# weleen/AGRL.pytorch

Hardware: AMD Instinct MI355X
Metric: frames/sec (fwd+GCN+distmat), MARS seq_len=8 (higher is better)
Workload: dtype fp16; 1 GPU; MARS seq_len=8 bs=32/GPU fp16 fwd+distmat (BASELINE configs[1]): 256x128 frames, VMGN ResNet50x2-branch + 2 graph layers, cosine distmat vs resident 12180 x 4096 gallery; global_batch=32, seq_len=8, gallery_rows_per_gpu=12180, parallelism=dp1, hip_graph=False, ranks=1, devices_visible=1, library=libagrl_hip.so, clip_batches_rotated=3, clip_bytes_rotated=301989888

## Files before the change

### agrl.pytorch_amd/csrc/bottleneck_block.hip

```cpp
#include "igemm_dev.h"

namespace {

struct BlockParams {
    const void* z;
    const void* w2;
    const float* b2;
    const void* w3;
    const float* b3;
    const void* res;
    const void* xs;
    const void* ws;
    const float* bs;
    void* out;
    const void* w1n;
    const float* b1n;
    void* zn;
    int F, H, W;
};

template <bool CAT, int CN>
__global__ __launch_bounds__(512) void bottleneck_block_kernel(const BlockParams p, int ntiles) {
    static_assert(CN == 64 || (CN == 128 && !CAT), "next conv1: 64 channels, or 128 with the identity shortcut");
    constexpr int NW = 8, PW = 10, PPIX = 100, PPIECES = 13, PATCH_BYTES = PPIECES * 1024, PJ = 2;
    constexpr int W_TAP = 64 * 128, W2_BYTES = 9 * W_TAP;
    constexpr int Y_BYTES = 64 * 128;
    constexpr int X_BYTES = CAT ? 64 * 128 : 0;
    constexpr int R_BYTES = 64 * 512;
    constexpr int NST = CN == 64 ? 5 : 6;
    constexpr int NA2 = CN / 64;
    __shared__ __attribute__((aligned(16))) unsigned char smem[W2_BYTES + 2 * PATCH_BYTES + Y_BYTES + X_BYTES + R_BYTES + 1024];
    unsigned char* s_w2 = smem;
    unsigned char* s_p = s_w2 + W2_BYTES;
    unsigned char* s_y = s_p + 2 * PATCH_BYTES;
    unsigned char* s_x = s_y + Y_BYTES;
    unsigned char* s_r = s_x + X_BYTES;
    unsigned char* s_dummy = s_r + R_BYTES;

    const int tid = threadIdx.x, lane = tid & 63;
    const int wave = __builtin_amdgcn_readfirstlane(tid >> 6);
    const int frow = lane & 15, fchunk = lane >> 4;
    const int lrow = lane >> 3, lchk = lane & 7;
    const int G = gridDim.x;
    const int tw = p.W >> 3, th = p.H >> 3;
    const unsigned char* zsrc = reinterpret_cast<const unsigned char*>(&g_zero16);
    const unsigned char* zg = reinterpret_cast<const unsigned char*>(p.z);
    const unsigned char* resg = reinterpret_cast<const unsigned char*>(p.res);
    const unsigned char* xsg = reinterpret_cast<const unsigned char*>(p.xs);

    {
        const int row = wave * 8 + lrow;
#pragma unroll
        for (int t = 0; t < 9; ++t)
            dma16(reinterpret_cast<const unsigned char*>(p.w2) + ((size_t)row * 576 + t * 64) * 2 + ((lchk ^ ((row >> 1) & 7)) << 4),
                  s_w2 + t * W_TAP + wave * 8 * 128);
    }
    const int wm2 = wave & 1, wn4 = wave >> 1;
    uint4 w3f[4][2], wsf[CAT ? 4 : 1][2], w1f[NA2][8];
#pragma unroll
    for (int a = 0; a < 4; ++a)
#pragma unroll
        for (int kk = 0; kk < 2; ++kk) {
            const size_t o = ((size_t)(wn4 * 64 + a * 16 + frow) * 64 + kk * 32 + fchunk * 8) * 2;
            w3f[a][kk] = *reinterpret_cast<const uint4*>(reinterpret_cast<const unsigned char*>(p.w3) + o);
            if constexpr (CAT) wsf[a][kk] = *reinterpret_cast<const uint4*>(reinterpret_cast<const unsigned char*>(p.ws) + o);
        }
#pragma unroll
    for (int a = 0; a < NA2; ++a)
#pragma unroll
        for (int ks = 0; ks < 8; ++ks)
            w1f[a][ks] = *reinterpret_cast<const uint4*>(reinterpret_cast<const unsigned char*>(p.w1n) +
                                                         ((size_t)(wn4 * (CN / 4) + a * 16 + frow) * 256 + ks * 32 + fchunk * 8) * 2);
    const int wm = wave & 3, wn = wave >> 2;
    float4 b2v[2], b3v[4], b1v[NA2];
#pragma unroll
    for (int a = 0; a < 2; ++a) b2v[a] = *reinterpret_cast<const float4*>(p.b2 + wn * 32 + a * 16 + fchunk * 4);
#pragma unroll
    for (int a = 0; a < 4; ++a) {
        b3v[a] = *reinterpret_cast<const float4*>(p.b3 + wn4 * 64 + a * 16 + fchunk * 4);
        if constexpr (CAT) {
            const float4 t = *reinterpret_cast<const float4*>(p.bs + wn4 * 64 + a * 16 + fchunk * 4);
            b3v[a].x += t.x; b3v[a].y += t.y; b3v[a].z += t.z; b3v[a].w += t.w;
        }
    }
#pragma unroll
    for (int a = 0; a < NA2; ++a) b1v[a] = *reinterpret_cast<const float4*>(p.b1n + wn4 * (CN / 4) + a * 16 + fchunk * 4);
#pragma unroll
    for (int a = 0; a < 4; ++a)
#pragma unroll
        for (int kk = 0; kk < 2; ++kk) {
            asm volatile("" : "+v"(w3f[a][kk].x), "+v"(w3f[a][kk].y), "+v"(w3f[a][kk].z), "+v"(w3f[a][kk].w));
            if constexpr (CAT) asm volatile("" : "+v"(wsf[a][kk].x), "+v"(wsf[a][kk].y), "+v"(wsf[a][kk].z), "+v"(wsf[a][kk].w));
        }
#pragma unroll
    for (int a = 0; a < NA2; ++a)
#pragma unroll
        for (int ks = 0; ks < 8; ++ks) asm volatile("" : "+v"(w1f[a][ks].x), "+v"(w1f[a][ks].y), "+v"(w1f[a][ks].z), "+v"(w1f[a][ks].w));
#pragma unroll
    for (int a = 0; a < 4; ++a) asm volatile("" : "+v"(b3v[a].x), "+v"(b3v[a].y), "+v"(b3v[a].z), "+v"(b3v[a].w));
#pragma unroll
    for (int a = 0; a < 2; ++a) asm volatile("" : "+v"(b2v[a].x), "+v"(b2v[a].y), "+v"(b2v[a].z), "+v"(b2v[a].w));
#pragma unroll
    for (int a = 0; a < NA2; ++a) asm volatile("" : "+v"(b1v[a].x), "+v"(b1v[a].y), "+v"(b1v[a].z), "+v"(b1v[a].w));

    unsigned res_lane[4], out_lane[CN == 64 ? 4 : 1];
#pragma unroll
    for (int j = 0; j < 4; ++j) {
        const int rrow = (wave * 4 + j) * 2 + (lane >> 5);
        res_lane[j] = (unsigned)(((rrow >> 3) * p.W + (rrow & 7)) * 512 + (((lane & 31) ^ (rrow & 31)) << 4));
        const int orow = (tid >> 5) + 16 * j;
        if constexpr (CN == 64) out_lane[j] = (unsigned)(((orow >> 3) * p.W + (orow & 7)) * 512 + (((tid & 31) ^ (orow & 31)) << 4));
    }

    auto tile_origin = [&](int T, int& img, int& oy0, int& ox0) {
        img = T / (tw * th);
        const int trem = T - img * (tw * th);
        oy0 = (trem / tw) << 3;
        ox0 = (trem % tw) << 3;
    };
    auto gpix = [&](int img, int oy0, int ox0, int q) { return ((size_t)img * p.H + oy0 + (q >> 3)) * p.W + ox0 + (q & 7); };

    auto stage_patch = [&](int T, int buf) {
        int img, oy0, ox0;
        tile_origin(T, img, oy0, ox0);
        int ln = lane;
        asm volatile("" : "+v"(ln));
#pragma unroll
        for (int i = 0; i < PJ; ++i) {
            const int piece = wave + NW * i;
            const int row = piece * 8 + (ln >> 3);
            const int py = row / PW, px = row - py * PW;
            const int iy = oy0 + py - 1, ix = ox0 + px - 1;
            const bool ok = piece < PPIECES && row < PPIX && (unsigned)iy < (unsigned)p.H && (unsigned)ix < (unsigned)p.W;
            dma16(ok ? zg + (((size_t)img * p.H + iy) * p.W + ix) * 128 + (((ln & 7) ^ patch_g(py, px)) << 4) : zsrc,
                  piece < PPIECES ? s_p + buf * PATCH_BYTES + piece * 1024 : s_dummy);
        }
    };
    auto stage_shortcut = [&](int T) {
        int img, oy0, ox0;
        tile_origin(T, img, oy0, ox0);
        int ln = lane;
        asm volatile("" : "+v"(ln));
        if constexpr (CAT) {
            const int row = wave * 8 + (ln >> 3);
            dma16(xsg + gpix(img, oy0, ox0, row) * 128 + (((ln & 7) ^ ((row >> 1) & 7)) << 4), s_x + wave * 1024);
        } else {
            const unsigned char* tbase = resg + gpix(img, oy0, ox0, 0) * 512;
#pragma unroll
            for (int j = 0; j < 4; ++j) dma16(tbase + res_lane[j], s_r + (wave * 4 + j) * 1024);
        }
    };

    int xoff[18], woff[2][2];
    {
        const int q = frag_px(frow);
        const int py0 = 2 * wm + (q >> 3), px0 = q & 7;
#pragma unroll
        for (int st = 0; st < 18; ++st) {
            const int t = st >> 1, kk = st & 1;
            xoff[st] = patch_off<PW>(py0 + t / 3, px0 + t % 3, kk * 4 + fchunk);
        }
#pragma unroll
        for (int kk = 0; kk < 2; ++kk)
#pragma unroll
            for (int a = 0; a < 2; ++a) woff[kk][a] = lds_off(wn * 32 + a * 16 + frow, kk * 4 + fchunk);
    }

    const int xcd = blockIdx.x & 7;
    const int xq = ntiles >> 3, xr = ntiles & 7;
    const int xbase = xcd < xr ? xcd * (xq + 1) : xr * (xq + 1) + (xcd - xr) * xq;
    const int tend = xbase + xq + (xcd < xr ? 1 : 0);
    const int tstep = (G >> 3) + (xcd < (G & 7) ? 1 : 0);
    int T = xbase + (int)(blockIdx.x >> 3);
    if (T < tend) stage_patch(T, 0);
    int buf = 0;
    bool first = true;
    for (; T < tend; T += tstep, buf ^= 1) {
        int img, oy0, ox0;
        tile_origin(T, img, oy0, ox0);
        const bool has_next = T + tstep < tend;
        if (first) wait_vmcnt<0>();
        else wait_vmcnt<NST>();
        first = false;
        wg_barrier();
        stage_shortcut(T);
        if (has_next) stage_patch(T + tstep, buf ^ 1);
        int fr = frow, fc = fchunk, td = tid;
        asm volatile("" : "+v"(fr), "+v"(fc), "+v"(td));

        {
            const unsigned char* sp = s_p + buf * PATCH_BYTES;
            const int q = frag_px(fr);
            f32x4_t acc0[2] = {f32x4_t{0.f, 0.f, 0.f, 0.f}, f32x4_t{0.f, 0.f, 0.f, 0.f}};
            uint4 xq[3], wq[3][2];
            auto ld0 = [&](int st, int slot) {
                const int t = st >> 1, kk = st & 1;
                xq[slot] = *reinterpret_cast<const uint4*>(sp + xoff[st]);
#pragma unroll
                for (int a = 0; a < 2; ++a) wq[slot][a] = *reinterpret_cast<const uint4*>(s_w2 + t * W_TAP + woff[kk][a]);
            };
            ld0(0, 0);
            ld0(1, 1);
#pragma unroll
            for (int st = 0; st < 18; ++st) {
                if (st + 2 < 18) ld0(st + 2, (st + 2) % 3);
#pragma unroll
                for (int a = 0; a < 2; ++a) acc0[a] = Frag<lp16_t>::mma(wq[st % 3][a], xq[st % 3], acc0[a]);
                __builtin_amdgcn_sched_barrier(0);
            }
            const int prow = wm * 16 + q;
#pragma unroll
            for (int a = 0; a < 2; ++a) {
                const int c = wn * 32 + a * 16 + fc * 4;
                float v[4] = {relu_nan(acc0[a][0] + b2v[a].x), relu_nan(acc0[a][1] + b2v[a].y),
                              relu_nan(acc0[a][2] + b2v[a].z), relu_nan(acc0[a][3] + b2v[a].w)};
                store4<lp16_t>(reinterpret_cast<lp16_t*>(s_y + prow * 128 + (((c >> 3) ^ ((prow >> 1) & 7)) << 4) + ((c & 4) << 1)), v);
            }
        }
        if constexpr (CAT) {
            if (has_next) wait_vmcnt<PJ>();
            else wait_vmcnt<0>();
        }
        wg_barrier();

        f32x4_t acc[4][2];
#pragma unroll
        for (int a = 0; a < 4; ++a)
#pragma unroll
            for (int b = 0; b < 2; ++b) acc[a][b] = f32x4_t{0.f, 0.f, 0.f, 0.f};
#pragma unroll
        for (int kk = 0; kk < 2; ++kk) {
            uint4 xf[2];
#pragma unroll
            for (int b = 0; b < 2; ++b) xf[b] = *reinterpret_cast<const uint4*>(s_y + lds_off(wm2 * 32 + b * 16 + fr, kk * 4 + fc));
#pragma unroll
            for (int a = 0; a < 4; ++a)
#pragma unroll
                for (int b = 0; b < 2; ++b) acc[a][b] = Frag<lp16_t>::mma(w3f[a][kk], xf[b], acc[a][b]);
        }
        if constexpr (CAT) {
#pragma unroll
            for (int kk = 0; kk < 2; ++kk) {
                uint4 xf[2];
#pragma unroll
                for (int b = 0; b < 2; ++b) xf[b] = *reinterpret_cast<const uint4*>(s_x + lds_off(wm2 * 32 + b * 16 + fr, kk * 4 + fc));
#pragma unroll
                for (int a = 0; a < 4; ++a)
#pragma unroll
                    for (int b = 0; b < 2; ++b) acc[a][b] = Frag<lp16_t>::mma(wsf[a][kk], xf[b], acc[a][b]);
            }
        } else {
            if (has_next) wait_vmcnt<PJ>();
            else wait_vmcnt<0>();
            wg_barrier();
        }
        uint2 rcell[2][4];
        if constexpr (!CAT) {
#pragma unroll
            for (int b = 0; b < 2; ++b) {
                const int px = wm2 * 32 + b * 16 + fr;
#pragma unroll
                for (int a = 0; a < 4; ++a) {
                    const int c = wn4 * 64 + a * 16 + fc * 4;
                    rcell[b][a] = *reinterpret_cast<const uint2*>(s_r + px * 512 + (((c >> 3) ^ (px & 31)) << 4) + ((c & 4) << 1));
                }
            }
        }
#pragma unroll
        for (int b = 0; b < 2; ++b) {
            const int px = wm2 * 32 + b * 16 + fr;
#pragma unroll
            for (int a = 0; a < 4; ++a) {
                const int c = wn4 * 64 + a * 16 + fc * 4;
                unsigned char* cell = s_r + px * 512 + (((c >> 3) ^ (px & 31)) << 4) + ((c & 4) << 1);
                float rr[4] = {0.f, 0.f, 0.f, 0.f};
                if constexpr (!CAT) {
                    unpack_lp16x2(rcell[b][a].x, rr[0], rr[1]);
                    unpack_lp16x2(rcell[b][a].y, rr[2], rr[3]);
                }
                float v[4];
                v[0] = relu_nan(acc[a][b][0] + b3v[a].x + rr[0]);
                v[1] = relu_nan(acc[a][b][1] + b3v[a].y + rr[1]);
                v[2] = relu_nan(acc[a][b][2] + b3v[a].z + rr[2]);
                v[3] = relu_nan(acc[a][b][3] + b3v[a].w + rr[3]);
                store4<lp16_t>(reinterpret_cast<lp16_t*>(cell), v);
            }
        }
        wg_barrier();
        {
            unsigned char* obase = reinterpret_cast<unsigned char*>(p.out) + gpix(img, oy0, ox0, 0) * 512;
#pragma unroll
            for (int i = 0; i < 4; ++i) {
                const int row = (td >> 5) + 16 * i;
                const int pch = td & 31;
                const uint4 v = *reinterpret_cast<const uint4*>(s_r + row * 512 + (pch << 4));
                if constexpr (CN == 64) *reinterpret_cast<uint4*>(obase + out_lane[i]) = v;
                else *reinterpret_cast<uint4*>(reinterpret_cast<unsigned char*>(p.out) + (gpix(img, oy0, ox0, row) * 256 + (pch ^ (row & 31)) * 8) * 2) = v;
            }
        }
        f32x4_t acc2[NA2][2];
#pragma unroll
        for (int a = 0; a < NA2; ++a)
#pragma unroll
            for (int b = 0; b < 2; ++b) acc2[a][b] = f32x4_t{0.f, 0.f, 0.f, 0.f};
        {
            uint4 x2[3][2];
            auto ld2 = [&](int ks, int slot) {
#pragma unroll
                for (int b = 0; b < 2; ++b) {
                    const int px = wm2 * 32 + b * 16 + fr;
                    x2[slot][b] = *reinterpret_cast<const uint4*>(s_r + px * 512 + (((ks * 4 + fc) ^ (px & 31)) << 4));
                }
            };
            ld2(0, 0);
            ld2(1, 1);
#pragma unroll
            for (int ks = 0; ks < 8; ++ks) {
                if (ks + 2 < 8) ld2(ks + 2, (ks + 2) % 3);
#pragma unroll
                for (int a = 0; a < NA2; ++a)
#pragma unroll
                    for (int b = 0; b < 2; ++b) acc2[a][b] = Frag<lp16_t>::mma(w1f[a][ks], x2[ks % 3][b], acc2[a][b]);
                __builtin_amdgcn_sched_barrier(0);
            }
        }
        unsigned char* sz = CN == 64 ? s_y : s_r;
        if constexpr (CN == 128) wg_barrier();
#pragma unroll
        for (int b = 0; b < 2; ++b) {
            const int px = wm2 * 32 + b * 16 + fr;
#pragma unroll
            for (int a = 0; a < NA2; ++a) {
                const int c = wn4 * (CN / 4) + a * 16 + fc * 4;
                float v[4];
                v[0] = relu_nan(acc2[a][b][0] + b1v[a].x);
                v[1] = relu_nan(acc2[a][b][1] + b1v[a].y);
                v[2] = relu_nan(acc2[a][b][2] + b1v[a].z);
                v[3] = relu_nan(acc2[a][b][3] + b1v[a].w);
                store4<lp16_t>(reinterpret_cast<lp16_t*>(sz + px * (CN * 2) + (((c >> 3) ^ (px & (CN / 8 - 1))) << 4) + ((c & 4) << 1)), v);
            }
        }
        wg_barrier();
#pragma unroll
        for (int i = 0; i < CN / 64; ++i) {
            const int row = td >> 3, pch = (td & 7) * (CN / 64) + i;
            const uint4 v = *reinterpret_cast<const uint4*>(sz + row * (CN * 2) + (pch << 4));
            *reinterpret_cast<uint4*>(reinterpret_cast<unsigned char*>(p.zn) + (gpix(img, oy0, ox0, row) * CN + (pch ^ (row & (CN / 8 - 1))) * 8) * 2) = v;
        }
    }
}

}

extern "C" int agrl_bottleneck_block(const void* z, const void* w2, const float* b2, const void* w3, const float* b3,
                                     const void* residual, const void* x_short, const void* w_short, const float* b_short,
                                     void* out, const void* w1_next, const float* b1_next, void* z_next, int F, int H, int W,
                                     int Cmid, int Cout, int Cnext, agrl_stream_t stream) {
    AGRL_CHECK_ARG(z && w2 && b2 && w3 && b3 && out && w1_next && b1_next && z_next, "agrl_bottleneck_block: null pointer");
    AGRL_CHECK_ARG((residual != nullptr) != (x_short != nullptr),
                   "agrl_bottleneck_block: pass either the residual map or the downsample conv's input, not both");
    AGRL_CHECK_ARG(!x_short || (w_short && b_short), "agrl_bottleneck_block: the downsample form needs its weights and bias");
    AGRL_CHECK_ARG(F > 0 && H > 0 && W > 0 && (H % 8) == 0 && (W % 8) == 0, "agrl_bottleneck_block: maps must be multiples of 8 x 8 (got %d x %d)", H, W);
    AGRL_CHECK_ARG(Cmid == 64 && Cout == 256 && (Cnext == 64 || (Cnext == 128 && !x_short)),
                   "agrl_bottleneck_block: built for Cmid=64, Cout=256, Cnext=64 (128 without downsample), got %d/%d/%d", Cmid, Cout, Cnext);
    AGRL_CHECK_ARG((size_t)F * H * W * 256 * 2 < (1ull << 40), "agrl_bottleneck_block: problem too large");
    const uintptr_t al = (uintptr_t)z | (uintptr_t)w2 | (uintptr_t)b2 | (uintptr_t)w3 | (uintptr_t)b3 | (uintptr_t)residual |
                         (uintptr_t)x_short | (uintptr_t)w_short | (uintptr_t)b_short | (uintptr_t)out | (uintptr_t)w1_next |
                         (uintptr_t)b1_next | (uintptr_t)z_next;
    AGRL_CHECK_ARG((al & 15) == 0, "agrl_bottleneck_block: pointers must be 16-byte aligned");
    BlockParams p;
    p.z = z; p.w2 = w2; p.b2 = b2; p.w3 = w3; p.b3 = b3; p.res = residual; p.xs = x_short; p.ws = w_short; p.bs = b_short;
    p.out = out; p.w1n = w1_next; p.b1n = b1_next; p.zn = z_next; p.F = F; p.H = H; p.W = W;
    const int ntiles = F * (H / 8) * (W / 8);
    const int grid = ntiles < 256 ? ntiles : 256;
    if (x_short) hipLaunchKernelGGL((bottleneck_block_kernel<true, 64>), dim3(grid), dim3(512), 0, (hipStream_t)stream, p, ntiles);
    else if (Cnext == 128) hipLaunchKernelGGL((bottleneck_block_kernel<false, 128>), dim3(grid), dim3(512), 0, (hipStream_t)stream, p, ntiles);
    else hipLaunchKernelGGL((bottleneck_block_kernel<false, 64>), dim3(grid), dim3(512), 0, (hipStream_t)stream, p, ntiles);
    AGRL_CHECK_LAUNCH("agrl_bottleneck_block");
    return 0;
}
```

### agrl.pytorch_amd/csrc/bottleneck_tail.hip

```cpp
#include "igemm_dev.h"

namespace {

struct TailParams {
    const void* y2;
    const void* w3;
    const float* b3;
    const void* res;
    void* out;
    const void* w1n;
    const float* b1n;
    void* z;
    const void* xs;
    const void* ws;
    const float* bs;
    int M;
};

constexpr int TBM = 64, TK1 = 64, TN1 = 256, TK2 = 256, TN2 = 64;

template <bool CAT>
__global__ __launch_bounds__(512) void bottleneck_tail_kernel(const TailParams p, int ntiles) {
    constexpr int NKT1 = CAT ? 2 : 1;
    constexpr int W3_BYTES = NKT1 * TN1 * 128;
// ... 207 lines not shown
            const int gch = (lane & 31) ^ (row & 31);
            dma16(gm < p.M ? resg + ((size_t)gm * TN1 + gch * 8) * 2 : zsrc, sr + piece * 1024);
        }
    };
    float4 b3v[4], b1v[2];
#pragma unroll
    for (int a = 0; a < 4; ++a) b3v[a] = *reinterpret_cast<const float4*>(p.b3 + wn4 * 64 + a * 16 + fchunk * 4);
#pragma unroll
    for (int a = 0; a < 2; ++a) b1v[a] = *reinterpret_cast<const float4*>(p.b1n + wn4 * 32 + a * 16 + fchunk * 4);

    int T = blockIdx.x;
    if (T < ntiles) stage_y2(T, 0);
    wait_vmcnt<0>();
    wg_barrier();
    int slot = 0;
    for (; T < ntiles; T += G, slot ^= 1) {
        const int m0 = T * TBM;
        const bool has_next = T + G < ntiles;
        stage_res(T);
        if (has_next) stage_y2(T + G, slot ^ 1);
        const unsigned char* sa = s_a + slot * A_BYTES;
        f32x4_t acc[4][2];
#pragma unroll
        for (int a = 0; a < 4; ++a)
#pragma unroll
            for (int b = 0; b < 2; ++b) acc[a][b] = f32x4_t{0.f, 0.f, 0.f, 0.f};
#pragma unroll
        for (int kk = 0; kk < 2; ++kk) {
            uint4 xf[2], wf[4];
#pragma unroll
            for (int b = 0; b < 2; ++b) xf[b] = *reinterpret_cast<const uint4*>(sa + lds_off(wm2 * 32 + b * 16 + frow, kk * 4 + fchunk));
#pragma unroll
            for (int a = 0; a < 4; ++a) wf[a] = *reinterpret_cast<const uint4*>(s_w3 + lds_off(wn4 * 64 + a * 16 + frow, kk * 4 + fchunk));
#pragma unroll
            for (int a = 0; a < 4; ++a)
#pragma unroll
                for (int b = 0; b < 2; ++b) acc[a][b] = Frag<lp16_t>::mma(wf[a], xf[b], acc[a][b]);
        }
        if (has_next) wait_vmcnt<1>();
        else wait_vmcnt<0>();
        wg_barrier();
#pragma unroll
        for (int b = 0; b < 2; ++b) {
            const int px = wm2 * 32 + b * 16 + frow;
#pragma unroll
            for (int a = 0; a < 4; ++a) {
                const int c = wn4 * 64 + a * 16 + fchunk * 4;
                unsigned char* cell = sr + px * 512 + (((c >> 3) ^ (px & 31)) << 4) + ((c & 4) << 1);
                float rr[4];
                load4<lp16_t>(reinterpret_cast<const lp16_t*>(cell), rr);
                float v[4];
                v[0] = relu_nan(acc[a][b][0] + b3v[a].x + rr[0]);
                v[1] = relu_nan(acc[a][b][1] + b3v[a].y + rr[1]);
                v[2] = relu_nan(acc[a][b][2] + b3v[a].z + rr[2]);
                v[3] = relu_nan(acc[a][b][3] + b3v[a].w + rr[3]);
                store4<lp16_t>(reinterpret_cast<lp16_t*>(cell), v);
            }
        }
        wg_barrier();
#pragma unroll
        for (int i = 0; i < 4; ++i) {
            const int row = (tid >> 5) + 16 * i;
            const int pch = tid & 31;
            const int gm = m0 + row;
            if (gm < p.M) {
                const uint4 v = *reinterpret_cast<const uint4*>(sr + row * 512 + (pch << 4));
                *reinterpret_cast<uint4*>(reinterpret_cast<unsigned char*>(p.out) + ((size_t)gm * TN1 + (pch ^ (row & 31)) * 8) * 2) = v;
            }
        }
        f32x4_t acc2[2][2];
#pragma unroll
        for (int a = 0; a < 2; ++a)
#pragma unroll
            for (int b = 0; b < 2; ++b) acc2[a][b] = f32x4_t{0.f, 0.f, 0.f, 0.f};
#pragma unroll
        for (int ks = 0; ks < TK2 / 32; ++ks) {
            uint4 wf[2], xf[2];
#pragma unroll
            for (int a = 0; a < 2; ++a)
                wf[a] = *reinterpret_cast<const uint4*>(s_w1 + (ks >> 1) * W1_KT + lds_off(wn4 * 32 + a * 16 + frow, (ks & 1) * 4 + fchunk));
#pragma unroll
            for (int b = 0; b < 2; ++b) {
                const int px = wm2 * 32 + b * 16 + frow;
                xf[b] = *reinterpret_cast<const uint4*>(sr + px * 512 + (((ks * 4 + fchunk) ^ (px & 31)) << 4));
            }
#pragma unroll
            for (int a = 0; a < 2; ++a)
#pragma unroll
                for (int b = 0; b < 2; ++b) acc2[a][b] = Frag<lp16_t>::mma(wf[a], xf[b], acc2[a][b]);
        }
        wg_barrier();
#pragma unroll
        for (int b = 0; b < 2; ++b) {
            const int px = wm2 * 32 + b * 16 + frow;
#pragma unroll
            for (int a = 0; a < 2; ++a) {
                const int c = wn4 * 32 + a * 16 + fchunk * 4;
                float v[4];
                v[0] = relu_nan(acc2[a][b][0] + b1v[a].x);
                v[1] = relu_nan(acc2[a][b][1] + b1v[a].y);
                v[2] = relu_nan(acc2[a][b][2] + b1v[a].z);
                v[3] = relu_nan(acc2[a][b][3] + b1v[a].w);
                store4<lp16_t>(reinterpret_cast<lp16_t*>(sr + px * 256 + (((c >> 3) ^ (px & 15)) << 4) + ((c & 4) << 1)), v);
            }
        }
        wg_barrier();
#pragma unroll
        for (int i = 0; i < 2; ++i) {
            const int row = tid >> 3, pch = (tid & 7) * 2 + i;
            const int gm = m0 + row;
            if (gm < p.M) {
                const uint4 v = *reinterpret_cast<const uint4*>(sr + row * 256 + (pch << 4));
                *reinterpret_cast<uint4*>(reinterpret_cast<unsigned char*>(p.z) + ((size_t)gm * CN + (pch ^ (row & 15)) * 8) * 2) = v;
            }
        }
        wait_vmcnt<6>();
        wg_barrier();
    }
}


constexpr int L2K1 = 128, L2N1 = 512, L2K2 = 512, L2N2 = 128;

__global__ __launch_bounds__(512) void bottleneck_tail_l2_kernel(const TailParams p, int ntiles) {
    constexpr int A_BYTES = 2 * TBM * 128;
    constexpr int R_BYTES = TBM * L2N1 * 2;
    __shared__ __attribute__((aligned(16))) unsigned char smem[2 * A_BYTES + 2 * R_BYTES];
    unsigned char* s_a = smem;
    unsigned char* s_r = smem + 2 * A_BYTES;

    const int tid = threadIdx.x, lane = tid & 63;
    const int wave = __builtin_amdgcn_readfirstlane(tid >> 6);
    const int frow = lane & 15, fchunk = lane >> 4;
    const int G = gridDim.x;
    const unsigned char* zsrc = reinterpret_cast<const unsigned char*>(&g_zero16);
    const unsigned char* y2g = reinterpret_cast<const unsigned char*>(p.y2);
    const unsigned char* resg = reinterpret_cast<const unsigned char*>(p.res);

    uint4 w3f[4][4], w1f[16];
#pragma unroll
    for (int a = 0; a < 4; ++a)
#pragma unroll
        for (int kk = 0; kk < 4; ++kk)
            w3f[a][kk] = *reinterpret_cast<const uint4*>(reinterpret_cast<const unsigned char*>(p.w3) +
                                                         ((size_t)(wave * 64 + a * 16 + frow) * L2K1 + kk * 32 + fchunk * 8) * 2);
#pragma unroll
    for (int ks = 0; ks < 16; ++ks)
        w1f[ks] = *reinterpret_cast<const uint4*>(reinterpret_cast<const unsigned char*>(p.w1n) +
                                                  ((size_t)(wave * 16 + frow) * L2K2 + ks * 32 + fchunk * 8) * 2);
    float b3l = p.b3[wave * 64 + lane];
    float b1l = p.b1n[wave * 16 + (lane & 15)];
    asm volatile("" : "+v"(b3l), "+v"(b1l));
    auto lane_bias = [&](float held, int src_lane) {
        return __int_as_float(__builtin_amdgcn_ds_bpermute(src_lane << 2, __float_as_int(held)));
    };
#pragma unroll
    for (int a = 0; a < 4; ++a)
#pragma unroll
        for (int kk = 0; kk < 4; ++kk)
            asm volatile("" : "+v"(w3f[a][kk].x), "+v"(w3f[a][kk].y), "+v"(w3f[a][kk].z), "+v"(w3f[a][kk].w));
#pragma unroll
    for (int ks = 0; ks < 16; ++ks) asm volatile("" : "+v"(w1f[ks].x), "+v"(w1f[ks].y), "+v"(w1f[ks].z), "+v"(w1f[ks].w));

    auto stage_tile = [&](int T, int slot) {
        const int m0 = T * TBM;
        int ln = lane;
        asm volatile("" : "+v"(ln));
        {
            const int row = wave * 8 + (ln >> 3);
            const int gm = m0 + row;
#pragma unroll
            for (int kt = 0; kt < 2; ++kt)
                dma16(gm < p.M ? y2g + (size_t)gm * (L2K1 * 2) + kt * 128 + (((ln & 7) ^ ((row >> 1) & 7)) << 4) : zsrc,
                      s_a + slot * A_BYTES + kt * (TBM * 128) + wave * 1024);
        }
#pragma unroll
        for (int j = 0; j < 8; ++j) {
            const int row = wave * 8 + j;
            const int gm = m0 + row;
            dma16(gm < p.M ? resg + (size_t)gm * (L2N1 * 2) + ((ln ^ (row & 31)) << 4) : zsrc, s_r + slot * R_BYTES + row * 1024);
        }
    };

    int T = blockIdx.x;
    if (T < ntiles) stage_tile(T, 0);
    wait_vmcnt<0>();
    wg_barrier();
    int slot = 0;
    for (; T < ntiles; T += G, slot ^= 1) {
        const int m0 = T * TBM;
        if (T + G < ntiles) stage_tile(T + G, slot ^ 1);
        const unsigned char* sa = s_a + slot * A_BYTES;
        unsigned char* sr = s_r + slot * R_BYTES;
#pragma unroll
        for (int ah = 0; ah < 2; ++ah) {
            f32x4_t acc[2][4];
#pragma unroll
            for (int a = 0; a < 2; ++a)
#pragma unroll
                for (int b = 0; b < 4; ++b) acc[a][b] = f32x4_t{0.f, 0.f, 0.f, 0.f};
            uint4 xp[2][4];
            auto ld1 = [&](int kk, int b) {
                return *reinterpret_cast<const uint4*>(sa + (kk >> 1) * (TBM * 128) + lds_off(b * 16 + frow, (kk & 1) * 4 + fchunk));
            };
#pragma unroll
            for (int b = 0; b < 4; ++b) xp[0][b] = ld1(0, b);
#pragma unroll
            for (int kk = 0; kk < 4; ++kk) {
                if (kk + 1 < 4) {
#pragma unroll
                    for (int b = 0; b < 4; ++b) xp[(kk + 1) & 1][b] = ld1(kk + 1, b);
                }
#pragma unroll
                for (int a = 0; a < 2; ++a)
#pragma unroll
                    for (int b = 0; b < 4; ++b) acc[a][b] = Frag<lp16_t>::mma(w3f[2 * ah + a][kk], xp[kk & 1][b], acc[a][b]);
                __builtin_amdgcn_sched_barrier(0);
            }
            float bv[2][4];
#pragma unroll
            for (int a = 0; a < 2; ++a)
#pragma unroll
                for (int r = 0; r < 4; ++r) bv[a][r] = lane_bias(b3l, (2 * ah + a) * 16 + fchunk * 4 + r);
            uint2 rcell[4][2];
#pragma unroll
            for (int b = 0; b < 4; ++b) {
                const int px = b * 16 + frow;
#pragma unroll
                for (int a = 0; a < 2; ++a) {
                    const int c = wave * 64 + (2 * ah + a) * 16 + fchunk * 4;
                    rcell[b][a] = *reinterpret_cast<const uint2*>(sr + px * 1024 + (((c >> 3) ^ (px & 31)) << 4) + ((c & 4) << 1));
                }
            }
#pragma unroll
            for (int b = 0; b < 4; ++b) {
                const int px = b * 16 + frow;
#pragma unroll
                for (int a = 0; a < 2; ++a) {
                    const int c = wave * 64 + (2 * ah + a) * 16 + fchunk * 4;
                    unsigned char* cell = sr + px * 1024 + (((c >> 3) ^ (px & 31)) << 4) + ((c & 4) << 1);
                    float rr[4];
                    unpack_lp16x2(rcell[b][a].x, rr[0], rr[1]);
                    unpack_lp16x2(rcell[b][a].y, rr[2], rr[3]);
                    float v[4];
#pragma unroll
                    for (int r = 0; r < 4; ++r) v[r] = relu_nan(acc[a][b][r] + bv[a][r] + rr[r]);
                    store4<lp16_t>(reinterpret_cast<lp16_t*>(cell), v);
                }
            }
        }
        wg_barrier();
        int ld = lane, td = tid;
        asm volatile("" : "+v"(ld), "+v"(td));
#pragma unroll
        for (int i = 0; i < 8; ++i) {
            const int row = wave + 8 * i;
            const int gm = m0 + row;
            if (gm < p.M) {
                const uint4 v = *reinterpret_cast<const uint4*>(sr + row * 1024 + (ld << 4));
                *reinterpret_cast<uint4*>(reinterpret_cast<unsigned char*>(p.out) + ((size_t)gm * L2N1 + (ld ^ (row & 31)) * 8) * 2) = v;
            }
        }
        f32x4_t acc2[4];
#pragma unroll
        for (int b = 0; b < 4; ++b) acc2[b] = f32x4_t{0.f, 0.f, 0.f, 0.f};
        uint4 xq[2][4];
        auto ld2 = [&](int ks, int b) {
            const int px = b * 16 + frow;
            return *reinterpret_cast<const uint4*>(sr + px * 1024 + (((ks * 4 + fchunk) ^ (px & 31)) << 4));
        };
#pragma unroll
        for (int b = 0; b < 4; ++b) xq[0][b] = ld2(0, b);
#pragma unroll
        for (int ks = 0; ks < 16; ++ks) {
            if (ks + 1 < 16) {
#pragma unroll
                for (int b = 0; b < 4; ++b) xq[(ks + 1) & 1][b] = ld2(ks + 1, b);
            }
#pragma unroll
            for (int b = 0; b < 4; ++b) acc2[b] = Frag<lp16_t>::mma(w1f[ks], xq[ks & 1][b], acc2[b]);
            __builtin_amdgcn_sched_barrier(0);
        }
        unsigned char* sz = s_a + slot * A_BYTES;
#pragma unroll
        for (int b = 0; b < 4; ++b) {
            const int px = b * 16 + frow;
            const int c = wave * 16 + fchunk * 4;
            float v[4];
#pragma unroll
            for (int r = 0; r < 4; ++r) v[r] = relu_nan(acc2[b][r] + lane_bias(b1l, fchunk * 4 + r));
            store4<lp16_t>(reinterpret_cast<lp16_t*>(sz + px * 256 + (((c >> 3) ^ (px & 15)) << 4) + ((c & 4) << 1)), v);
        }
        wg_barrier();
#pragma unroll
        for (int i = 0; i < 2; ++i) {
            const int row = (td >> 4) + 32 * i, pch = td & 15;
            const int gm = m0 + row;
            if (gm < p.M) {
                const uint4 v = *reinterpret_cast<const uint4*>(sz + row * 256 + (pch << 4));
                *reinterpret_cast<uint4*>(reinterpret_cast<unsigned char*>(p.z) + ((size_t)gm * L2N2 + (pch ^ (row & 15)) * 8) * 2) = v;
            }
        }
        wait_vmcnt<10>();
        wg_barrier();
    }
}

}

extern "C" int agrl_bottleneck_tail(const void* y2, const void* w3, const float* b3, const void* residual,
                                    const void* x_short, const void* w_short, const float* b_short, void* out,
                                    const void* w1_next, const float* b1_next, void* z, int M, int Cmid, int Cout,
                                    int Cnext, int Cshort, agrl_stream_t stream) {
    AGRL_CHECK_ARG(y2 && w3 && b3 && out && w1_next && b1_next && z, "agrl_bottleneck_tail: null pointer");
    AGRL_CHECK_ARG((residual != nullptr) != (x_short != nullptr),
                   "agrl_bottleneck_tail: pass either the residual map or the downsample conv's input, not both");
    AGRL_CHECK_ARG(!x_short || (w_short && b_short), "agrl_bottleneck_tail: the downsample form needs its weights and bias");
    AGRL_CHECK_ARG(M > 0, "agrl_bottleneck_tail: empty problem");
    const bool layer2 = Cmid == L2K1 && Cout == L2N1 && Cnext == L2N2 && !x_short;
    AGRL_CHECK_ARG(layer2 || (Cmid == TK1 && Cout == TN1 && (Cnext == TN2 || (Cnext == 128 && !x_short)) && (!x_short || Cshort == TK1)),
                   "agrl_bottleneck_tail: built for Cmid=64, Cout=256, Cnext=64 (128 without downsample), Cshort=64 "
                   "(layer 1) and Cmid=128, Cout=512, Cnext=128 without downsample (layer 2), got %d/%d/%d/%d", Cmid, Cout, Cnext, Cshort);
    const uintptr_t al = (uintptr_t)y2 | (uintptr_t)w3 | (uintptr_t)b3 | (uintptr_t)residual | (uintptr_t)out |
                         (uintptr_t)w1_next | (uintptr_t)b1_next | (uintptr_t)z | (uintptr_t)x_short | (uintptr_t)w_short |
                         (uintptr_t)b_short;
    AGRL_CHECK_ARG((al & 15) == 0, "agrl_bottleneck_tail: pointers must be 16-byte aligned");
    TailParams p;
    p.y2 = y2; p.w3 = w3; p.b3 = b3; p.res = residual; p.out = out; p.w1n = w1_next; p.b1n = b1_next; p.z = z; p.M = M;
    p.xs = x_short; p.ws = w_short; p.bs = b_short;
    const int ntiles = cdiv(M, TBM);
    const int grid = ntiles < 256 ? ntiles : 256;
    if (layer2) hipLaunchKernelGGL(bottleneck_tail_l2_kernel, dim3(grid), dim3(512), 0, (hipStream_t)stream, p, ntiles);
    else if (Cnext == 128) hipLaunchKernelGGL(bottleneck_tail128_kernel, dim3(grid), dim3(512), 0, (hipStream_t)stream, p, ntiles);
    else if (x_short) hipLaunchKernelGGL(bottleneck_tail_kernel<true>, dim3(grid), dim3(512), 0, (hipStream_t)stream, p, ntiles);
    else hipLaunchKernelGGL(bottleneck_tail_kernel<false>, dim3(grid), dim3(512), 0, (hipStream_t)stream, p, ntiles);
    AGRL_CHECK_LAUNCH("agrl_bottleneck_tail");
    return 0;
}
```

### agrl.pytorch_amd/torchreid/_hip.py

```python
from __future__ import annotations

import ctypes as C
import os
import threading

import torch

F32 = 0
LP16 = 1
F32X3 = 2
F32H3P = 4
F32H3 = 3
FRAMES_NCHW = 0
FRAMES_NHWC = 1
METRIC_EUCLIDEAN = 0
METRIC_COSINE = 1

LP_NAME = os.environ.get("AGRL_HIP_LP16")
if LP_NAME is None:
    LP_NAME = os.environ.get("AGRL_HIP_PRECISION") if os.environ.get("AGRL_HIP_PRECISION") in ("fp16", "bf16") else "fp16"
if LP_NAME not in ("fp16", "bf16"):
    raise ValueError("AGRL_HIP_LP16 must be fp16 or bf16, not %r" % LP_NAME)
LP_DTYPE = torch.float16 if LP_NAME == "fp16" else torch.bfloat16

_HERE = os.path.dirname(os.path.abspath(__file__))
LIB_PATH = os.environ.get(
    "AGRL_HIP_LIB", os.path.normpath(os.path.join(_HERE, "..", "lib", "libagrl_hip.so" if LP_NAME == "fp16" else "libagrl_hip_bf16.so"))
)


class HipLibraryError(RuntimeError):
    """libagrl_hip.so is missing or incomplete."""


class HipKernelError(RuntimeError):
    """An entry point of libagrl_hip.so returned a non-zero status."""


_p = C.c_void_p
_i = C.c_int
_f = C.c_float

SIGNATURES = {
    "agrl_stem_conv_bn_relu_maxpool": [_p, _p, _p, _p, _i, _i, _i, _i, _p],
    "agrl_stem_conv_bn_relu_maxpool_lp16": [_p, _p, _p, _p, _i, _i, _i, _p],
    "agrl_conv2d_bn_act": [_p, _p, _p, _p, _p, _i, _i, _i, _i, _i, _i, _i, _i, _i, _i, _i, _p],
    "agrl_conv1x1_dual_split16": [_p, _p, _p, _p, _p] + [_i] * 8 + [_f, _i, _i, _p],
    "agrl_stem_split16": [_p, _p, _p, _p, _p, _i, _i, _i, _f, _p],
    "agrl_stem_conv_bn_relu_maxpool_u8": [_p, _p, _i, _p, _p, _p, _i, _i, _i, _i, _p],
    "agrl_stem_conv_bn_relu_maxpool_lp16_u8": [_p, _p, _i, _p, _p, _p, _i, _i, _i, _p],
    "agrl_stem_split16_u8": [_p, _p, _i, _p, _p, _p, _p, _i, _i, _i, _f, _p],
    "agrl_frames_normalize_u8": [_p, _p, _i, _p, _i, _i, _i, _p],
    "agrl_split16_planes": [_p, _p, C.c_longlong, _i, _i, _p],
    "agrl_split16_weight_planes": [_p, _p, C.c_longlong, _i, _f, _p],
    "agrl_split16_weights_inloop": [_p, _p, C.c_longlong, _i, _p],
    "agrl_conv1x1_split16": [_p, _p, _p, _p, _p, _i, _i, _i, _i, _f, _i, _p],
    "agrl_conv1x1_split16_dual": [_p, _p, _p, _p, _p, _i, _i, _i, _i, _i, _f, _i, _p],
    "agrl_conv1x1_split16_pool": [_p, _p, _p, _p, _p, _i, _i, _i, _i, _i, _i, C.POINTER(_i), _i, _i, _f, _i, _p],
    "agrl_conv3x3_packed_split16": [_p, _p, _p, _p, _i, _i, _i, _i, _i, _i, _f, _p],
    "agrl_conv2d_bn_act_split16": [_p, _p, _p, _p, _p] + [_i] * 10 + [_f, _i, _i, _p],
    "agrl_bottleneck_tail": [_p, _p, _p, _p, _p, _p, _p, _p, _p, _p, _p, _i, _i, _i, _i, _i, _p],
    "agrl_bottleneck_seam_packed_bytes": [_i, _i, _i],
    "agrl_bottleneck_seam_pack": [_p, _p, _p, _i, _i, _i, _p],
    "agrl_bottleneck_seam": [_p, _p, _p, _p, _p, _p, _p, _i, _i, _i, _i, _p],
    "agrl_conv3x3_packed_bytes": [_i, _i],
    "agrl_conv1x1_packed_bytes": [_i, _i],
    "agrl_conv1x1_pack": [_p, _p, _i, _i, _p],
    "agrl_conv1x1_packed_bn_act": [_p, _p, _p, _p, _p, _i, _i, _i, _i, _i, _p],
    "agrl_conv1x1_packed_res_bn_act": [_p, _p, _p, _p, _p, _i, _i, _i, _i, _p],
    "agrl_conv1x1_packed_res_pool": [_p, _p, _p, _p, _p, _p, _i, _i, _i, _i, _i, _i, C.POINTER(_i), _i, _i, _p],
    "agrl_conv1x1_packed_dual_duo": [_p, _p, _p, _p, _p, _i, _i, _i, _i, _i, _p],
    "agrl_conv1x1_packed_dual_strided": [_p, _p, _p, _p, _p, _i, _i, _i, _i, _i, _i, _i, _i, _p],
    "agrl_conv3x3_pack": [_p, _p, _i, _i, _p],
    "agrl_conv3x3_packed_bn_act": [_p, _p, _p, _p, _i, _i, _i, _i, _i, _i, _p],
    "agrl_bottleneck_block": [_p, _p, _p, _p, _p, _p, _p, _p, _p, _p, _p, _p, _p, _i, _i, _i, _i, _i, _i, _p],
    "agrl_conv1x1_dual_bn_act": [_p, _p, _p, _p, _p, _i, _i, _i, _i, _i, _p],
    "agrl_conv1x1_bn_act_pool": [_p, _p, _p, _p, _p, _p, _p, _i, _i, _i, _i, _i, _i, C.POINTER(_i), _i, _i, _p],
    "agrl_linear_nobias": [_p, _p, _p, _i, _i, _i, _i, _p],
    "agrl_part_pool": [_p, _p, _p, _p, _p, _i, _i, _i, _i, C.POINTER(_i), _i, _i, _p],
    "agrl_clip_pool": [_p, _p, _i, _i, _i, _i, _p],
    "agrl_graph_gram": [_p, _p, _i, _i, _i, _i, _p],
    "agrl_graph_pair_product": [_p, _p, _p, _p, _i, _i, _i, _p],
    "agrl_graph_finalize": [_p, _i, _p, _p, _i, _i, _i, _i, _i, _p],
    "agrl_graph_propagate": [_p, _p, _p, _p, _p, _f, _f, _f, _p, _p, _i, _i, _i, _p],
    "agrl_pam_pool": [_p, _p, _p, _p, _i, _i, _i, _i, _i, C.POINTER(_i), _i, _i, _p],
    "agrl_pam_combine": [_p, _p, _p, _f, _p, _p, _i, _i, _p],
    "agrl_graph_apply": [_p, _p, _p, _i, _i, _i, _i, _p],
    "agrl_graph_tracklet_operand": [_p, _p, _i, _p, _p, _i, _i, _i, _i, _i, _i, _i, _p],
    "agrl_graph_finalize_bits": [_p, _i, _p, _p, _i, _i, _i, _i, _i, _p],
    "agrl_pose_adjacency_bits": [_p, _p, _p, _i, _i, _i, _i, C.c_float, C.c_float, _p],
    "agrl_adjacency_pack": [_p, _p, _i, _i, _p],
    "agrl_graph_linear_mix": [_p, _p, _p, _p, _p, _f, _f, _f, _p, _i, _i, _i, _i, _p],
    "agrl_row_sqnorm": [_p, _p, _i, _i, _i, _p],
    "agrl_attn_pool_bnneck": [_p, _p, _p, _p, _p, _p, _p, _p, _p, _p, _i, _i, _i, _i, _i, _p],
    "agrl_attn_tail": [_p, _p, _p, _p, _p, _p, _p, _p, _p, _p, _p, _p, _p, _i, _i, _i, _i, _i, _p],
    "agrl_row_l2_normalize": [_p, _p, _i, _i, _i, _i, _i, _p],
    "agrl_distmat_split16": [_p, _p, _p, _p, _p, _i, _i, _i, _i, _i, _f, _p, C.c_size_t, _p],
    "agrl_distmat": [_p, _p, _p, _p, _p, _i, _i, _i, _i, _i, _i, _p, C.c_size_t, _p],
    "agrl_pose_adjacency": [_p, _p, _p, _i, _i, _i, _i, C.c_float, C.c_float, _p],
    "agrl_re_ranking_workspace": [_i, _i, _i],
    "agrl_re_ranking": [_p, _p, _p, _i, _i, _i, _i, C.c_double, _p, _i, _p, C.c_size_t, _p],
    "agrl_rank_topk": [_p, _i, _i, _i, _i, _i, _p, _p, _p],
    "agrl_distmat_topk_workspace": [_i, _i],
    "agrl_distmat_topk": [_p, _p, _p, _p, _i, _i, _i, _i, _i, _i, _i, _p, _p, _p, C.c_size_t, _p, C.c_size_t, _p],
    "agrl_rank_argsort": [_p, _i, _i, _i, _p, _p],
    "agrl_rank_mars": [_p, _p, _p, _p, _p, _i, _i, _i, _p, _p, _p],
    "agrl_rank_market1501": [_p, _i, _i, _i, _p, _p, _p, _p, _i, _p, _p, _p, _p],
    "agrl_triplet_hard_mine": [_p, _p, _i, _i, _p, _p, _p, _p, _p],
    "agrl_axpby": [_p, _p, _f, _f, _p, C.c_size_t, _p],
    "agrl_part_pool_backward": [_p, _p, _p, _p, _i, _i, _i, _i, _i, C.POINTER(_i), _i, _p],
    "agrl_attn_pool_backward": [_p, _p, _p, _i, _i, _i, _i, _p],
    "agrl_graph_matrix_backward": [_p, _i, _p, _p, _i, _i, _i, _i, _p],
    "agrl_xent_label_smooth": [_p, _p, _i, _i, _f, _p, _p, _p, _p],
    "agrl_triplet_loss": [_p, _p, _i, _i, _f, _i, _p, _p, _p, _p, _p, _p, _p, _p],
    "agrl_bn_workspace": [_i, _i],
    "agrl_bn_stats": [_p, _p, _p, _i, _i, _p, C.c_size_t, _p],
    "agrl_conv2d_stats": [_p, _p, _p, _p, C.c_size_t] + [_i] * 10 + [_p],
    "agrl_bn_stats_from_partials": [_p, _i, _i, _i, _p, _p, _p, C.c_size_t, _p],
    "agrl_bn_fold_train": [_p, _p, _p, _p, _f, _f, C.c_longlong, _p, _p, _p, _p, _p, _p, _i, _p],
    "agrl_bn_apply": [_p, _p, _p, _p, _p, _p, _i, _i, _i, _f, _p],
    "agrl_bn_backward": [_p, _p, _p, _p, _p, _p, _p, _i, _f, _p, _p, _p, _p, _i, _i, _p, C.c_size_t, _p],
    "agrl_im2col_t": [_p, _p, _i, _i, _i, _i, _i, _i, _i, _i, _i, _p],
    "agrl_gemm_nt_splitk": [_p, _p, _p, _i, _i, _i, _i, _p, C.c_size_t, _p],
    "agrl_im2col_rows": [_p, _p] + [_i] * 10 + [_p],
    "agrl_conv_wgrad_workspace": [_i] * 9,
    "agrl_conv_wgrad_plan": [_i] * 10 + [C.POINTER(_i)],
    "agrl_conv_wgrad": [_p, _p, _p] + [_i] * 10 + [_p, C.c_size_t, _p],
    "agrl_maxpool3x3s2": [_p, _p, _p, _i, _i, _i, _i, _p],
    "agrl_maxpool3x3s2_backward": [_p, _p, _p, _i, _i, _i, _i, _p],
    "agrl_diag_read_stream": [_p, C.c_size_t, _p, _i, _p],
    "agrl_optim_geometry": [C.POINTER(_i), C.POINTER(_i), C.POINTER(_i)],
    "agrl_adam_step": [_p, _i, _p, _i] + [_f] * 7 + [_i, _i, _p],
    "agrl_sgd_step": [_p, _i, _p, _i, _f, _f, _f, _i, _i, _i, _i, _p],
}

_lock = threading.Lock()
_lib = None


def lib():
    global _lib
    if _lib is not None:
        return _lib
    with _lock:
        if _lib is not None:
            return _lib
        if not os.path.exists(LIB_PATH):
            raise HipLibraryError(
                "libagrl_hip.so not found at %s -- build it with `python __graft_entry__.py` "
                "(or `make -C agrl.pytorch_amd/csrc`); the HIP path has no fallback" % LIB_PATH
            )
        try:
            h = C.CDLL(LIB_PATH)
        except OSError as e:
            raise HipLibraryError("cannot load %s: %s" % (LIB_PATH, e))
        for name, argtypes in SIGNATURES.items():
            try:
                fn = getattr(h, name)
            except AttributeError:
                raise HipLibraryError("%s does not export %s" % (LIB_PATH, name))
            fn.argtypes = argtypes
            fn.restype = _i
        h.agrl_re_ranking_workspace.restype = C.c_size_t
        h.agrl_bn_workspace.restype = C.c_size_t
        h.agrl_conv_wgrad_workspace.restype = C.c_size_t
        h.agrl_distmat_topk_workspace.restype = C.c_size_t
        h.agrl_bottleneck_seam_packed_bytes.restype = C.c_longlong
        h.agrl_conv3x3_packed_bytes.restype = C.c_longlong
        h.agrl_conv1x1_packed_bytes.restype = C.c_longlong
        for name in ("agrl_reload_options", "agrl_built_with_ablation", "agrl_lp16_is_f16"):
            getattr(h, name).argtypes = []
            getattr(h, name).restype = _i
        h.agrl_version.restype = _i
        h.agrl_last_error.restype = C.c_char_p
        if bool(h.agrl_lp16_is_f16()) != (LP_NAME == "fp16"):
            raise HipLibraryError("%s stores 16-bit data as %s but AGRL_HIP_LP16 asks for %s" % (
                LIB_PATH, "fp16" if h.agrl_lp16_is_f16() else "bf16", LP_NAME))
        _lib = h
    return _lib


RELOAD_HOOKS = []


def reload_options():
    lib().agrl_reload_options()
    for hook in RELOAD_HOOKS:
        hook()


def available() -> bool:
    try:
        lib()
        return True
    except HipLibraryError:
        return False


def _check(name, status):
    if status != 0:
        msg = lib().agrl_last_error()
        raise HipKernelError("%s failed (%d): %s" % (name, status, msg.decode() if msg else "?"))


def stream_ptr(device=None):
    return torch.cuda.current_stream(device).cuda_stream


def ptr(t):
    if t is None:
        return None
    assert t.is_cuda, "HIP entry points take device tensors"
    assert t.is_contiguous(), "HIP entry points take contiguous tensors"
    return t.data_ptr()


def dtype_code(dt):
    if dt == torch.float32:
        return F32
    if dt == LP_DTYPE:
        return LP16
    raise TypeError("unsupported dtype %s (float32 / %s only: the loaded library's 16-bit type is %s)" % (dt, LP_DTYPE, LP_NAME))


PROFILE = None
PROFILE_TAG = None


def call(name, *args):
    fn = getattr(lib(), name)
    if PROFILE is None:
        _check(name, fn(*args))
        return
    stream = torch.cuda.ExternalStream(args[-1]) if args[-1] else torch.cuda.current_stream()
    start, end = torch.cuda.Event(enable_timing=True), torch.cuda.Event(enable_timing=True)
    start.record(stream)
    _check(name, fn(*args))
    end.record(stream)
    global PROFILE_TAG
    PROFILE.append((name, start, end, PROFILE_TAG))
    PROFILE_TAG = None
```

### agrl.pytorch_amd/torchreid/hip_ops.py

```python
from __future__ import annotations

import ctypes as C
import os

import torch

from . import _hip
from ._hip import F32, LP16, LP_DTYPE, LP_NAME, METRIC_COSINE, METRIC_EUCLIDEAN, call, dtype_code, ptr


import contextlib
import threading
import weakref

_MODE = threading.local()


@contextlib.contextmanager
def f32_split(on=True):
    prev = getattr(_MODE, 'split', False)
    _MODE.split = bool(on)
    try:
        yield
    finally:
# ... 308 lines not shown
    Cc = x.shape[-1]
    out = torch.empty(tuple(x.shape[:-1]) + (nplanes * Cc,), dtype=torch.float16, device=x.device)
    with _dev(x):
        call("agrl_split16_planes", ptr(x), ptr(out), x.numel() // Cc, Cc, nplanes, _stream(x))
    return out


def to_split16_weight_planes(x, scale):
    assert x.dtype == torch.float32 and x.is_contiguous() and x.dim() == 2 and x.shape[1] % 4 == 0
    out = torch.empty((x.shape[0], 3 * x.shape[1]), dtype=torch.float16, device=x.device)
    with _dev(x):
        call("agrl_split16_weight_planes", ptr(x), ptr(out), x.shape[0], x.shape[1], float(scale), _stream(x))
    return out


def distmat_split16(q3, g3, metric, g_unscale, qn=None, gn=None, out=None):
    m, D3 = q3.shape
    n = g3.shape[0]
    assert g3.shape[1] == D3 and q3.dtype == torch.float16 and g3.dtype == torch.float16
    if out is None:
        out = torch.empty((m, n), dtype=torch.float32, device=q3.device)
    code = METRIC_EUCLIDEAN if metric == "euclidean" else METRIC_COSINE
    if _hip.PROFILE is not None:
        _hip.PROFILE_TAG = {"flops": 2.0 * m * n * D3 / 3, "mfma_flops": 2.0 * m * n * D3, "bytes": 2.0 * (m + n) * D3 + 4.0 * m * n}
    ws = None
    if (-(-m // 64)) * (-(-n // 128)) < 256:
        ws = torch.empty((8 * m * n,), dtype=torch.float32, device=q3.device)
    with _dev(q3):
        call("agrl_distmat_split16", ptr(q3), ptr(g3), ptr(qn), ptr(gn), out.data_ptr(), m, n, D3, out.stride(0), code, float(g_unscale),
             ptr(ws), 0 if ws is None else ws.numel() * 4, _stream(q3))
    return out


def from_split16_planes(x3, nplanes=3):
    Cc = x3.shape[-1] // nplanes
    return x3[..., :Cc].float() + x3[..., Cc:2 * Cc].float() * (2.0 ** -11)


def conv1x1_split16(x3, packed, unscale, bias, Cout, residual3=None, relu=True, x2=None, layout=0):
    N, H, W, Kx = x3.shape
    K3 = Kx // 2 * 3 if layout & 1 else Kx
    K23 = 0 if x2 is None else x2.shape[3]
    M = N * H * W
    no = 2 if layout & 2 else 3
    assert x3.dtype == torch.float16 and x3.is_contiguous() and packed.numel() == 2 * (K3 + K23) * Cout
    assert residual3 is None or (residual3.dtype == torch.float16 and residual3.is_contiguous() and tuple(residual3.shape) == (N, H, W, no * Cout))
    out = torch.empty((N, H, W, no * Cout), dtype=torch.float16, device=x3.device)
    if _hip.PROFILE is not None:
        _hip.PROFILE_TAG = {"flops": 2.0 * M * Cout * (K3 + K23) / 3, "mfma_flops": 2.0 * M * Cout * (K3 + K23),
                            "bytes": 2.0 * (x3.numel() + (0 if x2 is None else x2.numel()) + out.numel() + (0 if residual3 is None else residual3.numel() * 2 // no)) + packed.numel()}
    with _dev(x3):
        if x2 is None:
            call("agrl_conv1x1_split16", ptr(x3), ptr(packed), ptr(bias), ptr(residual3), ptr(out), M, K3, Cout, 1 if relu else 0,
                 float(unscale), int(layout), _stream(x3))
        else:
            assert residual3 is None and x2.dtype == torch.float16 and x2.is_contiguous() and tuple(x2.shape[:3]) == (N, H, W)
            call("agrl_conv1x1_split16_dual", ptr(x3), ptr(x2), ptr(packed), ptr(bias), ptr(out), M, K3, K23, Cout, 1 if relu else 0,
                 float(unscale), int(layout), _stream(x3))
    return out


def conv1x1_split16_pool(x3, packed, unscale, bias, Cout, residual3, splits, mean, relu=True, layout=0):
    N, H, W, K3 = x3.shape
    assert x3.dtype == torch.float16 and x3.is_contiguous() and (H, W) == (16, 8) and packed.numel() == 2 * K3 * Cout
    assert not (layout & 1), "the pooled conv's input is conv2's output: a triple"
    assert residual3 is None or (residual3.dtype == torch.float16 and residual3.is_contiguous()
                                 and tuple(residual3.shape) == (N, H, W, (2 if layout & 2 else 3) * Cout))
    P = int(sum(splits))
    pooled = torch.empty((N, P, Cout), dtype=torch.float32, device=x3.device)
    arr = (C.c_int * len(splits))(*[int(s_) for s_ in splits])
    if _hip.PROFILE is not None:
        _hip.PROFILE_TAG = {"flops": 2.0 * N * H * W * Cout * K3 / 3, "mfma_flops": 2.0 * N * H * W * Cout * K3,
                            "bytes": 2.0 * (x3.numel() + (residual3.numel() if residual3 is not None else 0)) + packed.numel() + 4.0 * pooled.numel()}
    with _dev(x3):
        call("agrl_conv1x1_split16_pool", ptr(x3), ptr(packed), ptr(bias), ptr(residual3), ptr(pooled), N, H, W, K3, Cout,
             1 if relu else 0, arr, len(splits), 1 if mean else 0, float(unscale), int(layout), _stream(x3))
    return pooled


def conv3x3_split16(x3, packed, unscale, bias, Cout, relu=True):
    N, H, W, Cin3 = x3.shape
    assert x3.dtype == torch.float16 and x3.is_contiguous() and packed.numel() == 2 * 9 * Cin3 * Cout
    out = torch.empty((N, H, W, 3 * Cout), dtype=torch.float16, device=x3.device)
    if _hip.PROFILE is not None:
        _hip.PROFILE_TAG = {"flops": 2.0 * N * H * W * Cout * 9 * Cin3 / 3, "mfma_flops": 2.0 * N * H * W * Cout * 9 * Cin3,
                            "bytes": 2.0 * (x3.numel() + out.numel()) + packed.numel()}
    with _dev(x3):
        call("agrl_conv3x3_packed_split16", ptr(x3), ptr(packed), ptr(bias), ptr(out), N, H, W, Cin3, Cout, 1 if relu else 0,
             float(unscale), _stream(x3))
    return out


def conv1x1_dual_supported(x1, x2, w_cat):
    K1, K2 = x1.shape[-1], x2.shape[-1]
    return (x1.dtype == LP_DTYPE and x2.dtype == LP_DTYPE and K1 == 2 * K2 and K1 % 64 == 0
            and w_cat.shape[0] % 256 == 0 and x1.shape[:-1] == x2.shape[:-1])


def conv1x1_dual(x1, x2, w_cat, bias, relu=True):
    N, H, W, K1 = x1.shape
    K2 = x2.shape[-1]
    Cout = w_cat.shape[0]
    assert tuple(w_cat.shape) == (Cout, K1 + K2) and w_cat.dtype == x1.dtype
    out = torch.empty((N, H, W, Cout), dtype=x1.dtype, device=x1.device)
    M = N * H * W
    if _hip.PROFILE is not None:
        _hip.PROFILE_TAG = {"flops": 2.0 * M * Cout * (K1 + K2), "bytes": 2.0 * (x1.numel() + x2.numel() + w_cat.numel() + out.numel()),
                            "conv": (1, 1, K1 + K2, Cout, H, W)}
    with _dev(x1):
        call("agrl_conv1x1_dual_bn_act", ptr(x1), ptr(x2), ptr(w_cat), ptr(bias), ptr(out), M, K1, K2, Cout, 1 if relu else 0,
             _stream(x1))
    return out


def conv1x1_bn_act_pool(x, w_ohwi, bias, residual, splits, mean, want_lp, relu=True):
    N, H, W, Cin = x.shape
    Cout = w_ohwi.shape[0]
    assert x.dtype == LP_DTYPE and tuple(w_ohwi.shape[1:3]) == (1, 1) and H * W == 128
    P = int(sum(splits))
    pooled = torch.empty((N, P, Cout), dtype=torch.float32, device=x.device)
    pooled_lp = torch.empty((N, P, Cout), dtype=LP_DTYPE, device=x.device) if want_lp else None
    arr = (C.c_int * len(splits))(*[int(s) for s in splits])
    if _hip.PROFILE is not None:
        _hip.PROFILE_TAG = {"flops": 2.0 * N * H * W * Cout * Cin,
                            "bytes": 2.0 * (x.numel() + w_ohwi.numel() + (residual.numel() if residual is not None else 0)) + 4.0 * pooled.numel()}
    with _dev(x):
        call("agrl_conv1x1_bn_act_pool", ptr(x), ptr(w_ohwi), ptr(bias), ptr(residual), None, ptr(pooled), ptr(pooled_lp),
             N, H, W, Cin, Cout, 1 if relu else 0, arr, len(splits), 1 if mean else 0, _stream(x))
    return pooled, pooled_lp


SEAM_SHAPES = ((256, 1024, 256), (512, 2048, 512), (256, 1024, 512))


def bottleneck_seam_supported(w3, w1_next, pixels=None):
    return (w3.dtype == LP_DTYPE and w1_next.dtype == LP_DTYPE and w3.dim() == 4 and tuple(w3.shape[1:3]) == (1, 1)
            and (w3.shape[3], w3.shape[0], w1_next.shape[0]) in SEAM_SHAPES and tuple(w1_next.shape[1:]) == (1, 1, w3.shape[0])
            and (pixels is None or pixels % 128 == 0))


def bottleneck_seam_pack(w3, w1_next):
    assert bottleneck_seam_supported(w3, w1_next)
    Cout, Cmid, Cnext = w3.shape[0], w3.shape[3], w1_next.shape[0]
    w3, w1_next = w3.contiguous(), w1_next.contiguous()
    nbytes = int(_hip.lib().agrl_bottleneck_seam_packed_bytes(Cmid, Cout, Cnext))
    assert nbytes == 2 * (w3.numel() + w1_next.numel())
    packed = torch.empty((nbytes,), dtype=torch.uint8, device=w3.device)
    with _dev(w3):
        call("agrl_bottleneck_seam_pack", ptr(w3), ptr(w1_next), ptr(packed), Cmid, Cout, Cnext, _stream(w3))
    return packed


def bottleneck_seam(y2, packed, b3, residual, b1_next, dims):
    Cmid, Cout, Cnext = dims
    N, H, W, C = y2.shape
    M = N * H * W
    assert y2.dtype == LP_DTYPE and C == Cmid and residual.shape == (N, H, W, Cout) and residual.dtype == y2.dtype and M % 128 == 0
    assert y2.is_contiguous() and residual.is_contiguous()
    out = torch.empty((N, H, W, Cout), dtype=y2.dtype, device=y2.device)
    z = torch.empty((N, H, W, Cnext), dtype=y2.dtype, device=y2.device)
    if _hip.PROFILE is not None:
        _hip.PROFILE_TAG = {"flops": 2.0 * M * (Cmid * Cout + Cout * Cnext),
                            "bytes": 2.0 * (y2.numel() + residual.numel() + out.numel() + z.numel()) + packed.numel(),
                            "conv": (1, 1, Cmid, Cout, H, W)}
    with _dev(y2):
        call("agrl_bottleneck_seam", ptr(y2), ptr(packed), ptr(b3), ptr(residual), ptr(out), ptr(b1_next), ptr(z), M, Cmid, Cout,
             Cnext, _stream(y2))
    return out, z


def conv3x3_packed_enabled():
    return True


def conv3x3_packed_supported(w_ohwi, H=None, W=None):
    return (w_ohwi.dtype == LP_DTYPE and w_ohwi.dim() == 4 and tuple(w_ohwi.shape[1:3]) == (3, 3) and w_ohwi.shape[3] % 64 == 0
            and w_ohwi.shape[3] >= 128 and (w_ohwi.shape[0] % 256 == 0 or w_ohwi.shape[0] == 128) and (H is None or (H % 16 == 0 and W % 8 == 0)))


def conv3x3_pack(w_ohwi):
    assert conv3x3_packed_supported(w_ohwi)
    Cout, Cin = w_ohwi.shape[0], w_ohwi.shape[3]
    if Cout == 128:
        w_ohwi = torch.cat([w_ohwi, torch.zeros_like(w_ohwi)], dim=0)
        Cout = 256
    w_ohwi = w_ohwi.contiguous()
    nbytes = int(_hip.lib().agrl_conv3x3_packed_bytes(Cin, Cout))
    assert nbytes == 2 * w_ohwi.numel()
    packed = torch.empty((nbytes,), dtype=torch.uint8, device=w_ohwi.device)
    with _dev(w_ohwi):
        call("agrl_conv3x3_pack", ptr(w_ohwi), ptr(packed), Cin, Cout, _stream(w_ohwi))
    return packed


def conv3x3_packed(x, packed, bias, Cout, relu=True):
    N, H, W, Cin = x.shape
    assert x.dtype == LP_DTYPE and x.is_contiguous() and packed.numel() == 2 * 9 * Cin * max(Cout, 256)
    out = torch.empty((N, H, W, Cout), dtype=x.dtype, device=x.device)
    if _hip.PROFILE is not None:
        _hip.PROFILE_TAG = {"flops": 2.0 * N * H * W * 9 * Cin * Cout, "bytes": 2.0 * (x.numel() + out.numel()) + 2.0 * 9 * Cin * Cout,
                            "conv": (3, 1, Cin, Cout, H, W)}
    with _dev(x):
        call("agrl_conv3x3_packed_bn_act", ptr(x), ptr(packed), ptr(bias), ptr(out), N, H, W, Cin, Cout, 1 if relu else 0, _stream(x))
    return out


def conv1x1_packed_supported(w):
    w2 = w.reshape(w.shape[0], -1) if w.dim() == 4 and tuple(w.shape[1:3]) == (1, 1) else w
    return w2.dtype == LP_DTYPE and w2.dim() == 2 and w2.shape[1] % 128 == 0 and w2.shape[0] % 256 == 0


def conv1x1_pack(w):
    assert conv1x1_packed_supported(w)
    w = w.reshape(w.shape[0], -1).contiguous()
    Cout, K = w.shape
    nbytes = int(_hip.lib().agrl_conv1x1_packed_bytes(K, Cout))
    assert nbytes == 2 * w.numel()
    packed = torch.empty((nbytes,), dtype=torch.uint8, device=w.device)
    with _dev(w):
        call("agrl_conv1x1_pack", ptr(w), ptr(packed), K, Cout, _stream(w))
    return packed


def conv1x1_packed(x, packed, bias, Cout, relu=True, x2=None, duo=False):
    N, H, W, K1 = x.shape
    K2 = 0 if x2 is None else x2.shape[3]
    M = N * H * W
    assert x.dtype == LP_DTYPE and x.is_contiguous() and packed.numel() == 2 * (K1 + K2) * Cout
    assert x2 is None or (x2.dtype == x.dtype and x2.is_contiguous() and tuple(x2.shape[:3]) == (N, H, W))
    out = torch.empty((N, H, W, Cout), dtype=x.dtype, device=x.device)
    if _hip.PROFILE is not None:
        _hip.PROFILE_TAG = {"flops": 2.0 * M * (K1 + K2) * Cout,
                            "bytes": 2.0 * (x.numel() + (0 if x2 is None else x2.numel()) + out.numel()) + packed.numel(),
                            "conv": (1, 1, K1 + K2, Cout, H, W)}
    with _dev(x):
        if duo and x2 is not None:
            call("agrl_conv1x1_packed_dual_duo", ptr(x), ptr(x2), ptr(packed), ptr(bias), ptr(out), M, K1, K2, Cout, 1 if relu else 0, _stream(x))
        else:
            call("agrl_conv1x1_packed_bn_act", ptr(x), ptr(x2), ptr(packed), ptr(bias), ptr(out), M, K1, K2, Cout, 1 if relu else 0, _stream(x))
    return out


def conv1x1_packed_dual_strided(x, x2, packed, bias, Cout, stride, relu=True):
    N, Hi, Wi, K1 = x.shape
    Ho, Wo = (Hi - 1) // stride + 1, (Wi - 1) // stride + 1
    K2 = x2.shape[3]
    assert x.dtype == LP_DTYPE and x2.dtype == LP_DTYPE and x.is_contiguous() and x2.is_contiguous()
    assert tuple(x2.shape[:3]) == (N, Ho, Wo) and packed.numel() == 2 * (K1 + K2) * Cout
    out = torch.empty((N, Ho, Wo, Cout), dtype=x.dtype, device=x.device)
    M = N * Ho * Wo
    if _hip.PROFILE is not None:
        _hip.PROFILE_TAG = {"flops": 2.0 * M * (K1 + K2) * Cout, "bytes": 2.0 * (M * K1 + x2.numel() + out.numel()) + packed.numel(),
                            "conv": (1, 1, K1 + K2, Cout, Ho, Wo)}
    with _dev(x):
        call("agrl_conv1x1_packed_dual_strided", ptr(x), ptr(x2), ptr(packed), ptr(bias), ptr(out), N, Hi, Wi, stride, K1, K2, Cout,
             1 if relu else 0, _stream(x))
    return out


def conv1x1_packed_res(x, packed, bias, Cout, residual, relu=True):
    N, H, W, K = x.shape
    M = N * H * W
    assert x.dtype == LP_DTYPE and x.is_contiguous() and packed.numel() == 2 * K * Cout
    assert residual is None or (residual.dtype == x.dtype and residual.is_contiguous() and tuple(residual.shape) == (N, H, W, Cout))
    out = torch.empty((N, H, W, Cout), dtype=x.dtype, device=x.device)
    if _hip.PROFILE is not None:
        _hip.PROFILE_TAG = {"flops": 2.0 * M * K * Cout,
                            "bytes": 2.0 * (x.numel() + out.numel() * (2 if residual is not None else 1)) + packed.numel(),
                            "conv": (1, 1, K, Cout, H, W)}
    with _dev(x):
        call("agrl_conv1x1_packed_res_bn_act", ptr(x), ptr(packed), ptr(bias), ptr(residual), ptr(out), M, K, Cout, 1 if relu else 0,
             _stream(x))
    return out


def conv1x1_packed_res_pool(x, packed, bias, Cout, residual, splits, mean, want_lp, relu=True):
    N, H, W, K = x.shape
    assert x.dtype == LP_DTYPE and x.is_contiguous() and (H, W) == (16, 8) and packed.numel() == 2 * K * Cout
    assert residual is None or (residual.dtype == x.dtype and residual.is_contiguous() and tuple(residual.shape) == (N, H, W, Cout))
    P = int(sum(splits))
    pooled = torch.empty((N, P, Cout), dtype=torch.float32, device=x.device)
    pooled_lp = torch.empty((N, P, Cout), dtype=LP_DTYPE, device=x.device) if want_lp else None
    arr = (C.c_int * len(splits))(*[int(s) for s in splits])
    if _hip.PROFILE is not None:
        _hip.PROFILE_TAG = {"flops": 2.0 * N * H * W * Cout * K,
                            "bytes": 2.0 * (x.numel() + (residual.numel() if residual is not None else 0)) + packed.numel() + 4.0 * pooled.numel()}
    with _dev(x):
        call("agrl_conv1x1_packed_res_pool", ptr(x), ptr(packed), ptr(bias), ptr(residual), ptr(pooled), ptr(pooled_lp),
             N, H, W, K, Cout, 1 if relu else 0, arr, len(splits), 1 if mean else 0, _stream(x))
    return pooled, pooled_lp


def bottleneck_tail_supported(y2, w3, w1_next, shortcut_conv=None):
    if (y2.dtype == LP_DTYPE and tuple(w3.shape) == (512, 1, 1, 128) and tuple(w1_next.shape) == (128, 1, 1, 512)
            and shortcut_conv is None):
        return True
    ok = (y2.dtype == LP_DTYPE and tuple(w3.shape) == (256, 1, 1, 64)
          and tuple(w1_next.shape) in ((64, 1, 1, 256), (128, 1, 1, 256)))
    if shortcut_conv is not None:
        ok = ok and tuple(shortcut_conv[0].shape) == (256, 1, 1, 64) and shortcut_conv[1] == 1 and w1_next.shape[0] == 64
    return ok


def bottleneck_tail(y2, w3, b3, residual, w1_next, b1_next, shortcut=None):
    N, H, W, Cmid = y2.shape
    Cout, Cnext = w3.shape[0], w1_next.shape[0]
    assert y2.dtype == LP_DTYPE and (residual is None) != (shortcut is None)
    xs = ws = bs = None
    Cshort = 0
    if shortcut is not None:
        xs, ws, bs = shortcut
        assert xs.shape[:3] == y2.shape[:3] and xs.dtype == y2.dtype
        Cshort = xs.shape[3]
    else:
        assert residual.shape == (N, H, W, Cout) and residual.dtype == y2.dtype
    out = torch.empty((N, H, W, Cout), dtype=y2.dtype, device=y2.device)
    z = torch.empty((N, H, W, Cnext), dtype=y2.dtype, device=y2.device)
    M = N * H * W
    if _hip.PROFILE is not None:
        rd = (residual.numel() if residual is not None else xs.numel() + ws.numel())
        _hip.PROFILE_TAG = {"flops": 2.0 * M * ((Cmid + Cshort) * Cout + Cout * Cnext),
                            "bytes": 2.0 * (y2.numel() + rd + out.numel() + z.numel() + w3.numel() + w1_next.numel())}
    with _dev(y2):
        call("agrl_bottleneck_tail", ptr(y2), ptr(w3), ptr(b3), ptr(residual), ptr(xs), ptr(ws), ptr(bs), ptr(out),
             ptr(w1_next), ptr(b1_next), ptr(z), M, Cmid, Cout, Cnext, Cshort, _stream(y2))
    return out, z


def bottleneck_block_supported(z, w2, stride, w3, w1_next, shortcut_conv=None):
    ok = (z.dtype == LP_DTYPE and stride == 1 and tuple(w2.shape) == (64, 3, 3, 64) and tuple(w3.shape) == (256, 1, 1, 64)
          and tuple(w1_next.shape) in ((64, 1, 1, 256), (128, 1, 1, 256)) and z.shape[1] % 8 == 0 and z.shape[2] % 8 == 0)
    if shortcut_conv is not None:
        ok = ok and tuple(shortcut_conv[0].shape) == (256, 1, 1, 64) and shortcut_conv[1] == 1 and w1_next.shape[0] == 64
    return ok


def bottleneck_block(z, w2, b2, w3, b3, residual, w1_next, b1_next, shortcut=None):
    N, H, W, Cmid = z.shape
    Cout, Cnext = w3.shape[0], w1_next.shape[0]
    assert z.dtype == LP_DTYPE and (residual is None) != (shortcut is None)
    xs = ws = bs = None
    if shortcut is not None:
        xs, ws, bs = shortcut
        assert tuple(xs.shape) == (N, H, W, 64) and xs.dtype == z.dtype
    else:
        assert tuple(residual.shape) == (N, H, W, Cout) and residual.dtype == z.dtype
    out = torch.empty((N, H, W, Cout), dtype=z.dtype, device=z.device)
    zn = torch.empty((N, H, W, Cnext), dtype=z.dtype, device=z.device)
    M = N * H * W
    if _hip.PROFILE is not None:
        rd = residual.numel() if residual is not None else xs.numel() + ws.numel()
        _hip.PROFILE_TAG = {"flops": 2.0 * M * (9 * Cmid * Cmid + (Cmid + (64 if shortcut is not None else 0)) * Cout + Cout * Cnext),
                            "bytes": 2.0 * (z.numel() + rd + out.numel() + zn.numel() + w2.numel() + w3.numel() + w1_next.numel())}
    with _dev(z):
        call("agrl_bottleneck_block", ptr(z), ptr(w2), ptr(b2), ptr(w3), ptr(b3), ptr(residual), ptr(xs), ptr(ws), ptr(bs),
             ptr(out), ptr(w1_next), ptr(b1_next), ptr(zn), N, H, W, Cmid, Cout, Cnext, _stream(z))
    return out, zn


def linear_nobias(x, w):
    M, K = x.shape
    Nout, K2 = w.shape
    assert K == K2 and x.dtype == w.dtype
    y = torch.empty((M, Nout), dtype=torch.float32, device=x.device)
    if _hip.PROFILE is not None:
        _hip.PROFILE_TAG = {"flops": 2.0 * M * K * Nout, "bytes": x.element_size() * (x.numel() + w.numel()) + 4 * y.numel()}
    with _dev(x):
        call("agrl_linear_nobias", ptr(x), ptr(w), ptr(y), M, K, Nout, _gemm_code(x.dtype), _stream(x))
    return y


def part_pool(x4_1, x4_2, splits, want_lp):
    F_, h, w, Cc = x4_1.shape
    assert x4_2.shape == x4_1.shape and x4_1.dtype == x4_2.dtype
    P = int(sum(splits))
    gsum = torch.empty((F_, Cc), dtype=torch.float32, device=x4_1.device)
    nodes = torch.empty((F_, P, Cc), dtype=torch.float32, device=x4_1.device)
    nodes_lp = torch.empty((F_, P, Cc), dtype=LP_DTYPE, device=x4_1.device) if want_lp else None
    arr = (C.c_int * len(splits))(*[int(s) for s in splits])
    with _dev(x4_1):
        call("agrl_part_pool", ptr(x4_1), ptr(x4_2), ptr(gsum), ptr(nodes), ptr(nodes_lp), F_, h, w, Cc, arr,
             len(splits), dtype_code(x4_1.dtype), _stream(x4_1))
    return gsum, nodes, nodes_lp


GRAM_CSLICE = 128


def graph_matrix(f, adj, use_pose, learn_graph, mask_diag=False):
    B, V, Cc = f.shape
    G = torch.empty((B, V, V), dtype=torch.float32, device=f.device)
    gram = None
    nz = 0
    with _dev(f):
        if learn_graph:
            nz = Cc // GRAM_CSLICE
            gram = torch.empty((B, nz, V, V), dtype=torch.float32, device=f.device)
            call("agrl_graph_gram", ptr(f), ptr(gram), B, V, Cc, GRAM_CSLICE, _stream(f))
        if use_pose and adjacency_is_packed(adj):
            assert tuple(adj.shape) == (B, V, (V + 31) // 32)
            call("agrl_graph_finalize_bits", ptr(gram), nz, ptr(adj.contiguous()), ptr(G), B, V, 1, 1 if learn_graph else 0,
                 1 if mask_diag else 0, _stream(f))
            return G
        if use_pose:
            assert adj is not None and tuple(adj.shape) == (B, V, V) and adj.dtype == torch.float32
            adj = adj.contiguous()
        call("agrl_graph_finalize", ptr(gram), nz, ptr(adj) if use_pose else None, ptr(G), B, V,
             1 if use_pose else 0, 1 if learn_graph else 0, 1 if mask_diag else 0, _stream(f))
    return G


def adjacency_is_packed(adj):
    return adj is not None and adj.dtype == torch.int32


def adjacency_pack(adj):
    B, V, V2 = adj.shape
    assert V == V2 and adj.dtype == torch.float32
    bits = torch.empty((B, V, (V + 31) // 32), dtype=torch.int32, device=adj.device)
    with _dev(adj):
        call("agrl_adjacency_pack", ptr(adj.contiguous()), ptr(bits), B, V, _stream(adj))
    return bits


def adjacency_pack_host(adj):
    import numpy as np
    a = np.asarray(adj.detach().cpu() if hasattr(adj, "detach") else adj) != 0
    B, V, _ = a.shape
    W = (V + 31) // 32
    pad = np.zeros((B, V, W * 32), dtype=bool)
    pad[:, :, :V] = a
    words = (pad.reshape(B, V, W, 32).astype(np.uint64) << np.arange(32, dtype=np.uint64)).sum(axis=3).astype(np.uint32)
    return torch.from_numpy(words.view(np.int32).copy())


def graph_propagate(f, h, G, bn_scale, bn_shift, gamma, slope, want_lp, keep=None):
    if keep is None:
        keep = 1.0 - float(gamma)
    B, V, Cc = f.shape
    out = torch.empty_like(f)
    out_lp = torch.empty((B, V, Cc), dtype=LP_DTYPE, device=f.device) if want_lp else None
    if _hip.PROFILE is not None:
        _hip.PROFILE_TAG = {"flops": 2.0 * B * V * V * Cc, "bytes": 4.0 * (3 * B * V * Cc + B * V * V)}
    with _dev(f):
        call("agrl_graph_propagate", ptr(f), ptr(h), ptr(G), ptr(bn_scale), ptr(bn_shift), float(keep), float(gamma),
             float(slope), ptr(out), ptr(out_lp), B, V, Cc, _stream(f))
    return out, out_lp


def graph_apply_presplit_supported(f):
    B, V, Cc = f.shape
    return V <= 64 and V % 4 == 0 and Cc % 128 == 0


def graph_apply_operand(G, f, out_dtype, presplit=False):
    B, V, Cc = f.shape
    assert f.dtype == torch.float32 and G.dtype == torch.float32 and tuple(G.shape) == (B, V, V)
    assert not presplit or (out_dtype == torch.float32 and graph_apply_presplit_supported(f))
    if V <= 64 and V % 4 == 0 and Cc % 128 == 0:
        out = torch.empty((B, V, Cc), dtype=out_dtype, device=f.device)
        if _hip.PROFILE is not None:
            _hip.PROFILE_TAG = {"flops": 2.0 * B * V * V * Cc, "bytes": 4.0 * (B * V * Cc + B * V * V) + out.element_size() * B * V * Cc}
        with _dev(f):
            call("agrl_graph_apply", ptr(G.contiguous()), ptr(f.contiguous()), ptr(out), _hip.F32H3P if presplit else dtype_code(out_dtype), B, V, Cc,
                 _stream(f))
        return out
    key = (f.device, Cc)
    if key not in _UNIT:
        _UNIT[key] = (torch.ones((Cc,), dtype=torch.float32, device=f.device), torch.zeros((Cc,), dtype=torch.float32, device=f.device))
    one, zero = _UNIT[key]
    out, out_lp = graph_propagate(f, f, G, one, zero, 1.0, 1.0, want_lp=out_dtype == LP_DTYPE, keep=0.0)
    return out_lp if out_dtype == LP_DTYPE else out


TRACKLET_FORM_MIN_B = 224


def graph_tracklet_operand_supported(f):
    B, V, Cc = f.shape
    return B >= TRACKLET_FORM_MIN_B and V <= 64 and V % 4 == 0 and Cc % 512 == 0


def graph_tracklet_operand(f, adj, use_pose, learn_graph, out_dtype, want_graph=False, mask_diag=False):
    B, V, Cc = f.shape
    assert f.dtype == torch.float32
    P = torch.empty((B, V, Cc), dtype=out_dtype, device=f.device)
    G = torch.empty((B, V, V), dtype=torch.float32, device=f.device) if want_graph else None
    packed = use_pose and adjacency_is_packed(adj)
    if use_pose:
        assert adj is not None and (tuple(adj.shape) == (B, V, (V + 31) // 32) if packed else (tuple(adj.shape) == (B, V, V) and adj.dtype == torch.float32))
        adj = adj.contiguous()
    if _hip.PROFILE is not None:
        _hip.PROFILE_TAG = {"flops": 4.0 * B * V * V * Cc, "bytes": 4.0 * (B * V * Cc + B * V * V) + P.element_size() * B * V * Cc}
    with _dev(f):
        call("agrl_graph_tracklet_operand", ptr(f.contiguous()), ptr(adj) if use_pose else None, 1 if packed else 0, ptr(G), ptr(P),
             dtype_code(out_dtype), B, V, Cc, 1 if use_pose else 0, 1 if learn_graph else 0, 1 if mask_diag else 0, _stream(f))
    return P, G


def graph_linear_mix(p_op, w, f, bn_scale, bn_shift, gamma, slope, keep=None, p_presplit=False):
    if keep is None:
        keep = 1.0 - float(gamma)
    B, V, K = p_op.shape
    Nout = w.shape[0]
    assert w.shape[1] == K and p_op.dtype == w.dtype and f.dtype == torch.float32 and tuple(f.shape) == (B, V, Nout)
    out = torch.empty_like(f)
    if _hip.PROFILE is not None:
        _hip.PROFILE_TAG = {"flops": 2.0 * B * V * K * Nout, "bytes": p_op.element_size() * (p_op.numel() + w.numel()) + 8.0 * f.numel()}
    code = _gemm_code(p_op.dtype)
    unscale = getattr(w, 'agrl_unscale', None)
    if unscale is not None:
        assert p_op.dtype == torch.float32 and getattr(bn_scale, 'agrl_folded_unscale', None) == unscale and getattr(w, 'agrl_presplit', False)
        code = _hip.F32H3P if p_presplit else _hip.F32H3
    else:
        assert not p_presplit
    with _dev(f):
        call("agrl_graph_linear_mix", ptr(p_op.contiguous()), ptr(w), ptr(f.contiguous()), ptr(bn_scale), ptr(bn_shift), float(keep), float(gamma),
             float(slope), ptr(out), B * V, K, Nout, code, _stream(f))
    return out


def pam_pool(x, qk, splits):
    F_, h, w, Cc = x.shape
    P = int(sum(splits))
    xmean = torch.empty((F_, P, Cc), dtype=torch.float32, device=x.device)
    xbar = None
    Cq = 0
    if qk is not None:
        assert qk.dtype == x.dtype and tuple(qk.shape[:3]) == (F_, h, w) and qk.shape[3] % 2 == 0
        Cq = qk.shape[3] // 2
        xbar = torch.empty((F_, P, Cc), dtype=torch.float32, device=x.device)
    arr = (C.c_int * len(splits))(*[int(s) for s in splits])
    with _dev(x):
        call("agrl_pam_pool", ptr(x), ptr(qk), ptr(xbar), ptr(xmean), F_, h, w, Cc, Cq, arr, len(splits), dtype_code(x.dtype),
             _stream(x))
    return xbar, xmean


def pam_combine(y, bv, xmean, gamma, want_lp):
    nodes = torch.empty_like(xmean)
    nodes_lp = torch.empty(xmean.shape, dtype=LP_DTYPE, device=xmean.device) if want_lp else None
    rows, Cc = xmean.numel() // xmean.shape[-1], xmean.shape[-1]
    with _dev(xmean):
        call("agrl_pam_combine", ptr(y), ptr(bv), ptr(xmean), float(gamma), ptr(nodes), ptr(nodes_lp), rows, Cc, _stream(xmean))
    return nodes, nodes_lp


def clip_pool(feats, num_clips, mode="avg"):
    assert feats.dtype == torch.float32 and feats.dim() == 2 and feats.size(0) % num_clips == 0 and mode in ("avg", "max")
    feats = feats.contiguous()
    T, D = feats.size(0) // num_clips, feats.size(1)
    out = torch.empty((T, D), dtype=torch.float32, device=feats.device)
    with _dev(feats):
        call("agrl_clip_pool", ptr(feats), ptr(out), T, num_clips, D, 0 if mode == "avg" else 1, _stream(feats))
    return out


def row_sqnorm(x):
    R, Cc = x.shape
    out = torch.empty((R,), dtype=torch.float32, device=x.device)
    with _dev(x):
        call("agrl_row_sqnorm", ptr(x), ptr(out), R, Cc, dtype_code(x.dtype), _stream(x))
    return out


def attn_pool_bnneck(nodes, sqn, gsum, g_scale, g_shift, a_scale, a_shift, B, S, P, hw, want_feats=False):
    Cc = nodes.shape[-1]
    out = torch.empty((B, 2 * Cc), dtype=torch.float32, device=nodes.device)
    g_f = torch.empty((B, Cc), dtype=torch.float32, device=nodes.device) if want_feats else None
    att_f = torch.empty((B, Cc), dtype=torch.float32, device=nodes.device) if want_feats else None
    with _dev(nodes):
        call("agrl_attn_pool_bnneck", ptr(nodes), ptr(sqn), ptr(gsum), ptr(g_scale), ptr(g_shift), ptr(a_scale),
             ptr(a_shift), ptr(out), ptr(g_f), ptr(att_f), B, S, P, Cc, hw, _stream(nodes))
    if want_feats:
        return out, g_f, att_f
    return out


def attn_tail_supported(S, P, Cc, B=None):
    ok = Cc % 4 == 0 and (((S * P + 3) & ~3) + 2 * Cc + 4) * 4 <= 64 * 1024
    if B is None or not ok:
        return ok
    force = switch('AGRL_HIP_FUSE_ATTN_TAIL', '')
    if force != '':
        return force != '0'
    return B >= int(switch('AGRL_HIP_ATTN_TAIL_MIN_B', '224'))


def attn_tail(nodes, gsum, g_scale, g_shift, a_scale, a_shift, B, S, P, hw, want_feats=False, query_dtype=None, want_node_sqn=False):
    Cc = nodes.shape[-1]
    dev = nodes.device
    out = torch.empty((B, 2 * Cc), dtype=torch.float32, device=dev)
    g_f = torch.empty((B, Cc), dtype=torch.float32, device=dev) if want_feats else None
    att_f = torch.empty((B, Cc), dtype=torch.float32, device=dev) if want_feats else None
    node_sqn = torch.empty((B * S * P,), dtype=torch.float32, device=dev) if want_node_sqn else None
    q_lp = q_f32 = out_sqn = None
    if query_dtype is not None:
        out_sqn = torch.empty((B,), dtype=torch.float32, device=dev)
        if query_dtype == LP_DTYPE:
            q_lp = torch.empty((B, 2 * Cc), dtype=LP_DTYPE, device=dev)
        else:
            q_f32 = torch.empty((B, 2 * Cc), dtype=torch.float32, device=dev)
    with _dev(nodes):
        call("agrl_attn_tail", ptr(nodes), ptr(gsum), ptr(g_scale), ptr(g_shift), ptr(a_scale), ptr(a_shift), ptr(out), ptr(g_f),
             ptr(att_f), ptr(node_sqn), ptr(out_sqn), ptr(q_lp), ptr(q_f32), B, S, P, Cc, hw, _stream(nodes))
    query = None if query_dtype is None else {'sqn': out_sqn, 'normalized': q_lp if q_lp is not None else q_f32}
    return out, ((g_f, att_f) if want_feats else None), query, node_sqn


class QueryOperandCache:

    def __init__(self, emb, query):
        self.ref = weakref.ref(emb)
        self.version = emb._version
        self.query = query

    def lookup(self, emb, dtype):
        if self.ref() is not emb or self.version != emb._version or self.query['normalized'].dtype != dtype:
            return None
        return self.query


def query_operands(model, emb, metric, dtype):
    cache = getattr(model, '_hip_query', None)
    q = cache.lookup(emb, dtype) if cache is not None else None
    if metric == 'cosine':
        return (q['normalized'] if q is not None else row_l2_normalize(emb, True, dtype)), None
    qn = q['sqn'] if q is not None else row_sqnorm(emb)
    return (row_l2_normalize(emb, False, dtype) if dtype != torch.float32 else emb), qn


def k_multiple(dtype):
    return 64 if dtype == LP_DTYPE else 32


def row_l2_normalize(x, normalize, out_dtype, pad_to=1):
    R, Cc = x.shape
    assert x.dtype == torch.float32
    ld = -(-Cc // pad_to) * pad_to
    y = torch.empty((R, ld), dtype=out_dtype, device=x.device)
    with _dev(x):
        call("agrl_row_l2_normalize", ptr(x), ptr(y), R, Cc, ld, 1 if normalize else 0, dtype_code(out_dtype),
             _stream(x))
    return y


def distmat(q, g, metric, qn=None, gn=None, out=None):
    m, D = q.shape
    n, D2 = g.shape
    assert D == D2 and q.dtype == g.dtype
    if out is None:
        out = torch.empty((m, n), dtype=torch.float32, device=q.device)
    assert out.stride(1) == 1 and out.dtype == torch.float32
    code = METRIC_EUCLIDEAN if metric == "euclidean" else METRIC_COSINE
    if _hip.PROFILE is not None:
        _hip.PROFILE_TAG = {"flops": 2.0 * m * n * D, "bytes": q.element_size() * (m + n) * D + 4.0 * m * n}
    ws = None
    if (-(-m // 64)) * (-(-n // 128)) < 256:
        ws = torch.empty((8 * m * n,), dtype=torch.float32, device=q.device)
# ... 409 lines not shown
```

### agrl.pytorch_amd/torchreid/models/_ganet_hip.py

```python
from __future__ import annotations

import torch

from torchreid import hip_ops as ops
from torchreid import _hip
from torchreid.models._vmgn_hip import (_PRECISIONS, eval_frames, run_stem, _fingerprint, _fold_bn1d, _fold_conv_bn, _pack_stage, _run_block, _run_trunk,
                                         check_packed_range)


def pack_weights(model, device, precision):
    ops.check_precision(precision)
    key = (device.index if device.index is not None else torch.cuda.current_device(), precision)
    cached = model._hip_packs.get(key)
    if cached is not None and (model.hip_static_weights or cached['fingerprint'] == _fingerprint(model)):
        return cached
    first = next(model.parameters())
    if first.device != device:
        raise RuntimeError('model parameters live on {} but the input is on {}'.format(first.device, device))
    dtype = _PRECISIONS[precision]
    s16 = precision == 'fp16x3'
    pam = model.pam_layer
    with torch.no_grad():
        stem_w, stem_b = _fold_conv_bn(model.conv1, model.bn1, torch.float32)
        cq = pam.query_conv.weight.shape[0]
        pack = {
            'dtype': dtype,
            'stem': (stem_w, stem_b),
            'stem_lp': ops.pack_stem_weights_lp16(stem_w) if dtype == ops.LP_DTYPE else None,
            'stem_s16': ops.pack_stem_weights_split16(stem_w) if s16 else None,
            'trunk': (_pack_stage(model.layer1, dtype, split16=s16) + _pack_stage(model.layer2, dtype, split16=s16)
                      + _pack_stage(model.layer3, dtype, seam=True, split16=s16)),
            'l4': _pack_stage(model.layer4, dtype, split16=s16),
            'qk_w': torch.cat([pam.query_conv.weight, pam.key_conv.weight], 0).detach().float().permute(0, 2, 3, 1).contiguous().to(dtype),
            'qk_b': torch.cat([pam.query_conv.bias, pam.key_conv.bias], 0).detach().float().contiguous(),
            'cq': cq,
            'v_w': pam.value_conv.weight.detach().float().view(pam.value_conv.weight.shape[0], -1).contiguous().to(dtype),
            'v_b': pam.value_conv.bias.detach().float().contiguous(),
            'pam_gamma': float(pam.gamma.detach()),
            'bn': _fold_bn1d(model.bottleneck),
            'graph': [],
        }
        for layer in model.graph_layers:
            scale, shift = _fold_bn1d(layer.bn)
            pack['graph'].append({'w': layer.linear.weight.detach().to(dtype).contiguous(), 'scale': scale, 'shift': shift,
                                  'slope': float(layer.relu.negative_slope), 'use_pose': bool(layer.use_pose),
                                  'learn_graph': bool(layer.learn_graph)})
    if dtype == ops.LP_DTYPE:
        check_packed_range(pack, 'ganet')
    pack['fingerprint'] = _fingerprint(model)
    model._hip_packs[key] = pack
    return pack


def hip_forward_ganet(model, x, adj, stages=None):
    _hip.lib()
    frames, B, S, norm = eval_frames(model, x)
    P = model.total_split
    V = S * P
    if tuple(adj.shape) != (B, V, V):
        raise ValueError('adj must be {} for S={} and {} parts, got {}'.format((B, V, V), S, P, tuple(adj.shape)))
    pack = pack_weights(model, x.device, model.hip_precision)
    lp = pack['dtype'] == ops.LP_DTYPE
    splits = list(model.total_split_list)
    with torch.no_grad(), ops.f32_split(model.hip_precision == 'bf16x3'):
        a = run_stem(frames, pack, norm)
        a = _run_trunk(a, pack['trunk'])
        for blk in pack['l4']:
            a = _run_block(a, blk)
        C = a.shape[-1]
        gamma_p = pack['pam_gamma']
        if gamma_p != 0.0:
            qk = ops.conv_bn_act(a, pack['qk_w'], pack['qk_b'], 1, 0, False)
            xbar, xmean = ops.pam_pool(a, qk, splits)
            operand = xbar.to(pack['dtype']) if lp else xbar
            y = ops.linear_nobias(operand.view(B * V, C), pack['v_w'])
            nodes, nodes_lp = ops.pam_combine(y, pack['v_b'], xmean, gamma_p, want_lp=lp)
        else:
            _, xmean = ops.pam_pool(a, None, splits)
            nodes, nodes_lp = ops.pam_combine(None, None, xmean, 0.0, want_lp=lp)
        del a
        nodes = nodes.view(B, V, C)
        if nodes_lp is not None:
            nodes_lp = nodes_lp.view(B, V, C)
        adj32 = adj.detach().to(torch.float32).contiguous()
        outs = [nodes]
        for g, layer in zip(pack['graph'], model.graph_layers):
            gamma_g = float(layer.gamma)
            cur = outs[-1]
            if gamma_g == 0.0:
                outs.append(cur)
                continue
            operand = nodes_lp if lp else cur
            h = ops.linear_nobias(operand.view(B * V, C), g['w']).view(B, V, C)
            G = ops.graph_matrix(cur, adj32, g['use_pose'], g['learn_graph'], mask_diag=True)
            if stages is not None:
                stages.setdefault('G', []).append(G)
            nxt, nodes_lp = ops.graph_propagate(cur, h, G, g['scale'], g['shift'], gamma_g, g['slope'], want_lp=lp, keep=1.0)
            outs.append(nxt)
        cat = torch.cat(outs, dim=2).contiguous()
        Ct = cat.shape[-1]
        if stages is not None:
            stages.update(nodes=nodes, cat=cat)
        sqn = ops.row_sqnorm(cat.view(B * V, Ct))
        gsum = torch.zeros((B * S, Ct), dtype=torch.float32, device=x.device)
        ident = (torch.ones_like(pack['bn'][0]), torch.zeros_like(pack['bn'][1]))
        out = ops.attn_pool_bnneck(cat, sqn, gsum, ident[0], ident[1], pack['bn'][0], pack['bn'][1], B, S, P, 1)
        return out[:, Ct:].contiguous()
```

### agrl.pytorch_amd/torchreid/models/_vmgn_hip.py

```python
from __future__ import annotations

import os

import torch

from torchreid import hip_ops as ops
from torchreid import _hip

_PRECISIONS = {'fp32': torch.float32, ops.LP_NAME: ops.LP_DTYPE, 'bf16x3': torch.float32, 'fp16x3': torch.float32}


def _fold_conv_bn(conv, bn, dtype, split16=False):
    w = conv.weight.detach().float()
    scale = bn.weight.detach().float() / torch.sqrt(bn.running_var.detach().float() + bn.eps)
    shift = bn.bias.detach().float() - bn.running_mean.detach().float() * scale
    w = (w * scale.view(-1, 1, 1, 1)).permute(0, 2, 3, 1).contiguous()
    if split16:
        assert dtype == torch.float32
        return ops.split16_inloop_weights(w), shift.contiguous()
    return w.to(dtype).contiguous(), shift.contiguous()


def check_packed_range(pack, where="vmgn"):
    def walk(obj, path):
        if torch.is_tensor(obj):
            if obj.dtype == ops.LP_DTYPE and obj.numel() and not bool(torch.isfinite(obj).all()):
                raise FloatingPointError("%s: the BatchNorm-folded weights of %s overflow %s (abs-max of the fp32 fold is beyond its "
                                         "range): load the bf16 build (AGRL_HIP_LP16=bf16) or use hip_precision='fp32'" % (where, path, ops.LP_NAME))
        elif isinstance(obj, dict):
            for k, v in obj.items():
                walk(v, "%s.%s" % (path, k))
        elif isinstance(obj, (list, tuple)):
            for i, v in enumerate(obj):
                walk(v, "%s[%d]" % (path, i))
    walk({k: v for k, v in pack.items() if k != 'fingerprint'}, "pack")


def _fold_bn1d(bn):
    scale = bn.weight.detach().float() / torch.sqrt(bn.running_var.detach().float() + bn.eps)
    shift = bn.bias.detach().float() - bn.running_mean.detach().float() * scale
    return scale.contiguous(), shift.contiguous()


def _pack_stage(stage, dtype, seam=False, split16=False):
    blocks = []
    for unit in stage:
        blk = {
            'c1': _fold_conv_bn(unit.conv1, unit.bn1, dtype, split16),
            'c2': _fold_conv_bn(unit.conv2, unit.bn2, dtype, split16),
            'c3': _fold_conv_bn(unit.conv3, unit.bn3, dtype, split16),
            'stride': unit.conv2.stride[0],
            'ds': None,
        }
        if unit.downsample is not None:
            blk['ds'] = _fold_conv_bn(unit.downsample[0], unit.downsample[1], dtype, split16)
            blk['ds_stride'] = unit.downsample[0].stride[0]
            if split16 and blk['ds_stride'] == blk['stride'] and blk['ds'][0].shape[3] % 32 == 0 and blk['c3'][0].shape[3] % 32 == 0:
                cout = blk['c3'][0].shape[0]
                wd = ops.split16_true_weights(blk['ds'][0])
                w3 = ops.split16_true_weights(blk['c3'][0])
                blk['dual16'] = (ops.split16_inloop_weights(torch.cat([wd.view(cout, -1), w3.view(cout, -1)], dim=1).contiguous()),
                                 (blk['ds'][1] + blk['c3'][1]).contiguous())
            if dtype == ops.LP_DTYPE and blk['ds_stride'] == 1 and blk['stride'] == 1:
                cout = blk['c3'][0].shape[0]
                blk['dual'] = (torch.cat([blk['ds'][0].view(cout, -1), blk['c3'][0].view(cout, -1)], dim=1).contiguous(),
                               (blk['ds'][1] + blk['c3'][1]).contiguous())
                if (ops.conv1x1_packed_supported(blk['dual'][0]) and blk['dual'][0].shape[1] >= 1536
                        and blk['ds'][0].shape[3] % 128 == 0 and blk['c3'][0].shape[3] % 128 == 0):
                    blk['dualp'] = ops.conv1x1_pack(blk['dual'][0])
            if dtype == ops.LP_DTYPE and blk['ds_stride'] > 1 and blk['ds_stride'] == blk['stride']:
                cout = blk['c3'][0].shape[0]
                dual_w = torch.cat([blk['ds'][0].view(cout, -1), blk['c3'][0].view(cout, -1)], dim=1).contiguous()
                if (ops.conv1x1_packed_supported(dual_w) and blk['ds'][0].shape[3] % 128 == 0 and blk['c3'][0].shape[3] % 128 == 0):
                    blk['dualps'] = ops.conv1x1_pack(dual_w)
                    blk['dualps_bias'] = (blk['ds'][1] + blk['c3'][1]).contiguous()
        if dtype == ops.LP_DTYPE and ops.conv1x1_packed_supported(blk['c1'][0]) and blk['c1'][0].shape[3] >= 1024:
            blk['c1p'] = ops.conv1x1_pack(blk['c1'][0])
        if (dtype == ops.LP_DTYPE and blk['ds'] is None and ops.conv1x1_packed_supported(blk['c3'][0])
                and blk['c3'][0].shape[0] >= 2048):
            blk['c3p'] = ops.conv1x1_pack(blk['c3'][0])
        if dtype == ops.LP_DTYPE and blk['stride'] == 1 and ops.conv3x3_packed_supported(blk['c2'][0]):
            blk['c2p'] = ops.conv3x3_pack(blk['c2'][0])
        blocks.append(blk)
    if seam and dtype == ops.LP_DTYPE:
        for blk, nxt in zip(blocks[:-1], blocks[1:]):
            if ops.bottleneck_seam_supported(blk['c3'][0], nxt['c1'][0]):
                blk['seam'] = ops.bottleneck_seam_pack(blk['c3'][0], nxt['c1'][0])
                blk['seam_dims'] = (blk['c3'][0].shape[3], blk['c3'][0].shape[0], nxt['c1'][0].shape[0])
    return blocks


def K_OK(w):
    return w.dim() == 2 and w.shape[1] % 32 == 0


def _fingerprint(model):
    return tuple((t.data_ptr(), t._version) for t in list(model.parameters()) + list(model.buffers()))


def pack_weights(model, device, precision):
    ops.check_precision(precision)
    key = (device.index if device.index is not None else torch.cuda.current_device(), precision)
    cached = model._hip_packs.get(key)
    if cached is not None and (model.hip_static_weights or cached['fingerprint'] == _fingerprint(model)):
        return cached
    first = next(model.parameters())
    if first.device != device:
        raise RuntimeError('model parameters live on {} but the input is on {}'.format(first.device, device))
    dtype = _PRECISIONS[precision]
    s16 = precision == 'fp16x3'
    with torch.no_grad():
        stem_w, stem_b = _fold_conv_bn(model.conv1, model.bn1, torch.float32)
        pack = {
            'dtype': dtype,
            'stem': (stem_w, stem_b),
            'stem_lp': ops.pack_stem_weights_lp16(stem_w) if dtype == ops.LP_DTYPE else None,
            'stem_s16': ops.pack_stem_weights_split16(stem_w) if s16 else None,
            'trunk': _pack_stage(model.layer1, dtype, split16=s16) + _pack_stage(model.layer2, dtype, split16=s16) + _pack_stage(model.layer3, dtype, seam=True, split16=s16),
            'graph': [],
        }
        if hasattr(model, 'layer4_1'):
            pack['l4_1'] = _pack_stage(model.layer4_1, dtype, split16=s16)
            pack['l4_2'] = _pack_stage(model.layer4_2, dtype, split16=s16)
            pack['g_bn'] = _fold_bn1d(model.global_bottleneck)
            pack['a_bn'] = _fold_bn1d(model.att_bottleneck)
        else:
            pack['l4'] = _pack_stage(model.layer4, dtype, split16=s16)
            pack['a_bn'] = _fold_bn1d(model.bottleneck)
            pack['g_bn'] = (torch.ones_like(pack['a_bn'][0]), torch.zeros_like(pack['a_bn'][1]))
        for layer in model.graph_layers:
            scale, shift = _fold_bn1d(layer.bn)
            gw = layer.linear.weight.detach().to(dtype).contiguous()
            if s16 and K_OK(gw):
                gw = ops.split16_inloop_weights(gw)
                scale = (scale * gw.agrl_unscale).contiguous()
                scale.agrl_folded_unscale = gw.agrl_unscale
            pack['graph'].append({
                'w': gw,
                'scale': scale, 'shift': shift,
                'gamma': float(layer.gamma), 'slope': float(layer.relu.negative_slope),
                'use_pose': bool(layer.use_pose), 'learn_graph': bool(layer.learn_graph),
            })
    if s16:
        stages = pack['trunk'] + pack.get('l4_1', []) + pack.get('l4_2', []) + pack.get('l4', [])
        for blk in stages:
            for name in ('c1', 'c2', 'c3', 'ds'):
                if blk.get(name) is not None and not (hasattr(blk[name][0], 'agrl_unscale') and getattr(blk[name][0], 'agrl_presplit', False)):
                    raise RuntimeError("fp16x3 pack: %s lost its pre-scale attributes" % name)
    if s16 and ops.split16_planes_available() and hasattr(model, 'layer4_1'):
        first = len(model.layer1) + len(model.layer2) + 1
        with torch.no_grad():
            ok = all(_pack_planes(blk) for blk in pack['trunk'][first:] + pack['l4_1'] + pack['l4_2'])
        pack['planes_from'] = first if ok else None
    if s16:
        for blk in stages:
            for name in ('c1', 'c2', 'c3', 'ds', 'dual16'):
                if blk.get(name) is not None and hasattr(blk[name][0], 'agrl_scaled'):
                    del blk[name][0].agrl_scaled
    if dtype == ops.LP_DTYPE:
        check_packed_range(pack)
    pack['fingerprint'] = _fingerprint(model)
    model._hip_packs[key] = pack
    return pack


def _pack_planes(blk):
    def true_w(pair):
        return ops.split16_true_weights(pair[0])

    w1, w2, w3 = true_w(blk['c1']), true_w(blk['c2']), true_w(blk['c3'])
    K1, K3c, mid, cout = w1.shape[3], w3.shape[3], w1.shape[0], w3.shape[0]
    if blk['stride'] != 1 or mid % 256 or cout % 256 or K1 % 128 or K3c % 128 or tuple(w2.shape[1:3]) != (3, 3) or w2.shape[3] % 64:
        return False
    p3 = {}
    t, u = ops.split16_plane_weights(w1.view(mid, K1), pair_first=True)
    p3['c1'] = (ops.conv1x1_pack(t), u, blk['c1'][1], mid)
    t, u = ops.split16_plane_weights(w2)
    p3['c2'] = (ops.conv3x3_pack(t), u, blk['c2'][1], w2.shape[0])
    if blk['ds'] is not None:
        if blk['ds_stride'] != 1:
            return False
        wd = true_w(blk['ds'])
        Kd = wd.shape[3]
        if Kd % 128:
            return False
        t, u = ops.split16_plane_weights(torch.cat([wd.view(cout, Kd), w3.view(cout, K3c)], dim=1), segments=[Kd, K3c], pair_first=True)
        p3['dual'] = (ops.conv1x1_pack(t), u, (blk['ds'][1] + blk['c3'][1]).contiguous(), cout)
    else:
        t, u = ops.split16_plane_weights(w3.view(cout, K3c))
        p3['c3'] = (ops.conv1x1_pack(t), u, blk['c3'][1], cout)
    blk['p3'] = p3
    return True


def _run_block_planes(x3, blk, pool=None):
    p3 = blk['p3']
    xp, rop = 1, 2
    y = ops.conv1x1_split16(x3, p3['c1'][0], p3['c1'][1], p3['c1'][2], p3['c1'][3], layout=xp)
    y = ops.conv3x3_split16(y, p3['c2'][0], p3['c2'][1], p3['c2'][2], p3['c2'][3])
    if 'dual' in p3:
        assert pool is None
        d = p3['dual']
        return ops.conv1x1_split16(x3, d[0], d[1], d[2], d[3], x2=y, layout=xp | rop)
    c = p3['c3']
    if pool is not None:
        return ops.conv1x1_split16_pool(y, c[0], c[1], c[2], c[3], x3, pool[0], pool[1], layout=rop)
    return ops.conv1x1_split16(y, c[0], c[1], c[2], c[3], residual3=x3, layout=rop)


def _conv2(y, blk):
    if 'c2p' in blk and y.shape[1] % 16 == 0 and y.shape[2] % 8 == 0:
        return ops.conv3x3_packed(y, blk['c2p'], blk['c2'][1], blk['c2'][0].shape[0], True)
    return ops.conv_bn_act(y, blk['c2'][0], blk['c2'][1], blk['stride'], 1, True)


def _conv1(x, blk):
    if 'c1p' in blk and x.is_contiguous():
        return ops.conv1x1_packed_res(x, blk['c1p'], blk['c1'][1], blk['c1'][0].shape[0], None, True)
    return ops.conv_bn_act(x, blk['c1'][0], blk['c1'][1], 1, 0, True)


def _run_block_inloop(x, blk, out_planes=0):
    y = ops.conv_bn_act(x, blk['c1'][0], blk['c1'][1], 1, 0, True, out_presplit=True)
    y = ops.conv_bn_act(y, blk['c2'][0], blk['c2'][1], blk['stride'], 1, True, x_presplit=True, out_presplit=True)
    if 'dual16' in blk and x.is_contiguous():
        return ops.conv1x1_dual_split16(x, y, blk['dual16'][0], blk['dual16'][1], blk['stride'], True, x2_presplit=True, out_planes=out_planes)
    shortcut = x if blk['ds'] is None else ops.conv_bn_act(x, blk['ds'][0], blk['ds'][1], blk['ds_stride'], 0, False)
    out = ops.conv_bn_act(y, blk['c3'][0], blk['c3'][1], 1, 0, True, residual=shortcut, x_presplit=True)
    return ops.to_split16_planes(out, out_planes) if out_planes else out


def _is_inloop(blk):
    return getattr(blk['c1'][0], 'agrl_presplit', False)


def _run_trunk(a, blocks):
    z = None
    for i, blk in enumerate(blocks):
        if _is_inloop(blk):
            a = _run_block_inloop(a, blk)
            continue
        nxt = blocks[i + 1] if i + 1 < len(blocks) else None
        y = z if z is not None else ops.conv_bn_act(a, blk['c1'][0], blk['c1'][1], 1, 0, True)
        if nxt is not None:
            ds = None if blk['ds'] is None else (blk['ds'][0], blk['ds_stride'])
            if ops.bottleneck_block_supported(y, blk['c2'][0], blk['stride'], blk['c3'][0], nxt['c1'][0], ds) and (
                    ds is None or a.shape[3] == 64):
                if ds is None:
                    a, z = ops.bottleneck_block(y, blk['c2'][0], blk['c2'][1], blk['c3'][0], blk['c3'][1], a,
                                                nxt['c1'][0], nxt['c1'][1])
                else:
                    a, z = ops.bottleneck_block(y, blk['c2'][0], blk['c2'][1], blk['c3'][0], blk['c3'][1], None,
                                                nxt['c1'][0], nxt['c1'][1], shortcut=(a, blk['ds'][0], blk['ds'][1]))
                continue
        y = _conv2(y, blk)
        fusable = nxt is not None and ops.bottleneck_tail_supported(y, blk['c3'][0], nxt['c1'][0])
        if fusable and blk['ds'] is not None and ops.bottleneck_tail_supported(
                y, blk['c3'][0], nxt['c1'][0], (blk['ds'][0], blk['ds_stride'])) and a.shape[3] == 64:
            a, z = ops.bottleneck_tail(y, blk['c3'][0], blk['c3'][1], None, nxt['c1'][0], nxt['c1'][1],
                                       shortcut=(a, blk['ds'][0], blk['ds'][1]))
            continue
        if ('dualps' in blk and a.is_contiguous() and y.is_contiguous() and a.dtype == y.dtype and a.shape[0] == y.shape[0]
                and tuple(y.shape[1:3]) == tuple((d - 1) // blk['stride'] + 1 for d in a.shape[1:3])):
            a = ops.conv1x1_packed_dual_strided(a, y, blk['dualps'], blk['dualps_bias'], blk['c3'][0].shape[0], blk['stride'], True)
            z = None
            continue
        shortcut = a if blk['ds'] is None else ops.conv_bn_act(a, blk['ds'][0], blk['ds'][1], blk['ds_stride'], 0, False)
        if nxt is not None and 'seam' in blk and (y.numel() // y.shape[-1]) % 128 == 0:
            a, z = ops.bottleneck_seam(y, blk['seam'], blk['c3'][1], shortcut, nxt['c1'][1], blk['seam_dims'])
            continue
        if fusable:
            a, z = ops.bottleneck_tail(y, blk['c3'][0], blk['c3'][1], shortcut, nxt['c1'][0], nxt['c1'][1])
        else:
            a = ops.conv_bn_act(y, blk['c3'][0], blk['c3'][1], 1, 0, True, residual=shortcut)
            z = None
    return a


def _run_block(x, blk, pool=None):
    if _is_inloop(blk):
        assert pool is None
        return _run_block_inloop(x, blk)
    y = _conv1(x, blk)
    y = _conv2(y, blk)
    if (pool is None and 'dualp' in blk
            and x.shape[:3] == y.shape[:3] and x.dtype == y.dtype and x.is_contiguous() and y.is_contiguous()):
        return ops.conv1x1_packed(x, blk['dualp'], blk['dual'][1], blk['dual'][0].shape[0], True, x2=y, duo=True)
    if pool is None and 'dual' in blk and ops.conv1x1_dual_supported(x, y, blk['dual'][0]):
        return ops.conv1x1_dual(x, y, blk['dual'][0], blk['dual'][1], True)
    shortcut = x if blk['ds'] is None else ops.conv_bn_act(x, blk['ds'][0], blk['ds'][1], blk['ds_stride'], 0, False)
    duo = 'c3p' in blk and blk['ds'] is None and shortcut.is_contiguous() and y.is_contiguous()
    if pool is not None:
        if duo and tuple(y.shape[1:3]) == (16, 8):
            return ops.conv1x1_packed_res_pool(y, blk['c3p'], blk['c3'][1], blk['c3'][0].shape[0], shortcut, pool[0], pool[1], False)[0]
        return ops.conv1x1_bn_act_pool(y, blk['c3'][0], blk['c3'][1], shortcut, pool[0], pool[1], False)[0]
    if duo:
        return ops.conv1x1_packed_res(y, blk['c3p'], blk['c3'][1], blk['c3'][0].shape[0], shortcut)
    return ops.conv_bn_act(y, blk['c3'][0], blk['c3'][1], 1, 0, True, residual=shortcut)


def run_stem(frames, pack, norm=None):
    mean, std = norm if norm is not None else (ops.PIXEL_MEAN, ops.PIXEL_STD)
    if pack['stem_lp'] is not None:
        return ops.stem_lp16(frames, pack['stem_lp'], pack['stem'][1], mean, std)
    if pack.get('stem_s16') is not None:
        return ops.stem_split16(frames, pack['stem_s16'][0], pack['stem_s16'][1], pack['stem_s16'][2], pack['stem'][1], mean, std)
    return ops.stem(frames, pack['stem'][0], pack['stem'][1], pack['dtype'], mean, std)


def eval_frames(model, x):
    if x.dtype == torch.uint8:
        _, B, S, _, _ = ops.clip_frames(x)
        norm = (getattr(model, 'pixel_mean', ops.PIXEL_MEAN), getattr(model, 'pixel_std', ops.PIXEL_STD))
        return x.reshape((B * S,) + tuple(x.shape[2:])), B, S, norm
    if x.dtype != torch.float32:
        raise TypeError('frames must be float32, got {}'.format(x.dtype))
    B, S, Cc, H, W = x.shape
    return x.reshape(B * S, Cc, H, W), B, S, None


def _frame_size(frames):
    if frames.dtype == torch.uint8 and ops.frames_layout(frames.shape) == 'nhwc':
        return frames.shape[1], frames.shape[2]
    return frames.shape[2], frames.shape[3]


def hip_featuremaps(frames, pack, norm=None):
    a = run_stem(frames, pack, norm)
    a = _run_trunk(a, pack['trunk'])
    x4_1 = a
    for blk in pack['l4_1']:
        x4_1 = _run_block(x4_1, blk)
    x4_2 = a
    for blk in pack['l4_2']:
        x4_2 = _run_block(x4_2, blk)
    return x4_1, x4_2


def hip_features_pooled(frames, pack, splits, norm=None):
    first = pack.get('planes_from')
    if (pack['dtype'] != ops.LP_DTYPE and first is None) or pack['l4_1'][0]['stride'] != 1:
        return None
    H, W = _frame_size(frames)
    h4, w4 = H, W
    for _ in range(4):
        h4, w4 = (h4 + 1) // 2, (w4 + 1) // 2
    if (h4, w4) != (16, 8):
        return None
    a = run_stem(frames, pack, norm)
    if first is None:
        run_block = _run_block
        a = _run_trunk(a, pack['trunk'])
    else:
        run_block = _run_block_planes
        a = _run_trunk(a, pack['trunk'][:first - 1])
        a = _run_block_inloop(a, pack['trunk'][first - 1], out_planes=2)
        for blk in pack['trunk'][first:]:
            a = run_block(a, blk)
    assert a.shape[1] == 16 and a.shape[2] == 8
    splits = list(splits)
    x4_1 = a
    for blk in pack['l4_1'][:-1]:
        x4_1 = run_block(x4_1, blk)
    gsum = run_block(x4_1, pack['l4_1'][-1], pool=([1], False))
    x4_2 = a
    for blk in pack['l4_2'][:-1]:
        x4_2 = run_block(x4_2, blk)
    nodes = run_block(x4_2, pack['l4_2'][-1], pool=(splits, True))
    return gsum.view(gsum.shape[0], gsum.shape[2]), nodes


def gcn_commute_enabled(model=None):
    return True


def hip_graph_layers(nodes, nodes_lp, adj, pack, stages=None, commute=True):
    if not commute:
        raise ValueError("hip_graph_layers runs the commuted GraphLayer only ((G f) W^T): the Linear -> message pass form is retired")
    for i, g in enumerate(pack['graph']):
        pre = False
        if ops.graph_tracklet_operand_supported(nodes):
            P, G = ops.graph_tracklet_operand(nodes, adj, g['use_pose'], g['learn_graph'], pack['dtype'], want_graph=stages is not None)
        else:
            G = ops.graph_matrix(nodes, adj, g['use_pose'], g['learn_graph'])
            pre = getattr(g['w'], 'agrl_presplit', False) and ops.graph_apply_presplit_supported(nodes)
            P = ops.graph_apply_operand(G, nodes, pack['dtype'], presplit=pre)
        if stages is not None:
            stages['G%d' % i] = G
        nodes = ops.graph_linear_mix(P, g['w'], nodes, g['scale'], g['shift'], g['gamma'], g['slope'], p_presplit=pre)
    return nodes


def hip_forward(model, x, adj, return_feats=False, stages=None):
    _hip.lib()
    frames, B, S, norm = eval_frames(model, x)
    P = model.total_split
    V = S * P
    packed_adj = ops.adjacency_is_packed(adj)
    if tuple(adj.shape) != ((B, V, (V + 31) // 32) if packed_adj else (B, V, V)):
        raise ValueError('adj must be {} (fp32) or {} (bit-packed int32) for S={} and {} parts, got {}'.format(
            (B, V, V), (B, V, (V + 31) // 32), S, P, tuple(adj.shape)))
    pack = pack_weights(model, x.device, model.hip_precision)
    lp = pack['dtype'] == ops.LP_DTYPE
    with torch.no_grad(), ops.f32_split(model.hip_precision == 'bf16x3'):
        fused = hip_features_pooled(frames, pack, model.total_split_list, norm)
        if fused is not None:
            gsum, nodes = fused
            hw = 128
        else:
            x4_1, x4_2 = hip_featuremaps(frames, pack, norm)
            hw = x4_1.shape[1] * x4_1.shape[2]
            gsum, nodes, _ = ops.part_pool(x4_1, x4_2, model.total_split_list, want_lp=False)
            del x4_1, x4_2
        C = nodes.shape[-1]
        nodes = nodes.view(B, V, C)
        adj32 = adj.detach().contiguous() if packed_adj else adj.detach().to(torch.float32).contiguous()
        if stages is not None:
            stages.update(gsum=gsum, hw=hw, nodes=nodes)
        nodes = hip_graph_layers(nodes, None, adj32, pack, stages)
        model._hip_query = None
        if ops.attn_tail_supported(S, P, C, B):
            want = return_feats or stages is not None
            out, feats, query, _ = ops.attn_tail(nodes, gsum, pack['g_bn'][0], pack['g_bn'][1], pack['a_bn'][0], pack['a_bn'][1],
                                                 B, S, P, hw, want_feats=want, query_dtype=ops.LP_DTYPE if lp else torch.float32)
            model._hip_query = ops.QueryOperandCache(out, query)
            res = (out, feats[0], feats[1]) if want else out
        else:
            sqn = ops.row_sqnorm(nodes.view(B * V, C))
            res = ops.attn_pool_bnneck(nodes, sqn, gsum, pack['g_bn'][0], pack['g_bn'][1], pack['a_bn'][0],
                                       pack['a_bn'][1], B, S, P, hw, want_feats=return_feats or stages is not None)
        if stages is not None:
            stages.update(nodes_out=nodes, out=res[0], g_f=res[1], att_f=res[2])
            return res if return_feats else res[0]
        return res


def hip_forward_gsta(model, x, adj):
    _hip.lib()
    frames, B, S, norm = eval_frames(model, x)
    P = model.total_split
    V = S * P
    if tuple(adj.shape) != (B, V, V):
        raise ValueError('adj must be {} for S={} and {} parts, got {}'.format((B, V, V), S, P, tuple(adj.shape)))
    pack = pack_weights(model, x.device, model.hip_precision)
    lp = pack['dtype'] == ops.LP_DTYPE
    splits = list(model.total_split_list)
    with torch.no_grad(), ops.f32_split(model.hip_precision == 'bf16x3'):
        a = run_stem(frames, pack, norm)
        a = _run_trunk(a, pack['trunk'])
        if lp and a.shape[1] * a.shape[2] == 128 and pack['l4'][0]['stride'] == 1:
            for blk in pack['l4'][:-1]:
                a = _run_block(a, blk)
            nodes = _run_block(a, pack['l4'][-1], pool=(splits, True))
            hw = 128
        else:
            for blk in pack['l4']:
                a = _run_block(a, blk)
            hw = a.shape[1] * a.shape[2]
            _, nodes, _ = ops.part_pool(a, a, splits, want_lp=False)
        C = nodes.shape[-1]
        nodes = nodes.view(B, V, C)
        nodes = hip_graph_layers(nodes, None, adj.detach().to(torch.float32).contiguous(), pack)
        sqn = ops.row_sqnorm(nodes.view(B * V, C))
        gsum = torch.zeros((B * S, C), dtype=torch.float32, device=x.device)
        out = ops.attn_pool_bnneck(nodes, sqn, gsum, pack['g_bn'][0], pack['g_bn'][1], pack['a_bn'][0], pack['a_bn'][1], B, S, P, hw)
        return out[:, C:].contiguous()
```

### agrl.pytorch_amd/torchreid/models/ganet.py

```python
from __future__ import absolute_import
from __future__ import division

__all__ = ['ganet']

import os

import numpy as np
import torch
from torch import nn
from torch.nn import functional as F

from torchreid.utils.reidtools import calc_splits
from .vmgn import Bottleneck, RESNET50_STAGES, _make_stage


class PAM_Module(nn.Module):

    def __init__(self, in_dim):
        super(PAM_Module, self).__init__()
        self.channel_in = in_dim
        self.query_conv = nn.Conv2d(in_dim, in_dim // 8, kernel_size=1)
        self.key_conv = nn.Conv2d(in_dim, in_dim // 8, kernel_size=1)
        self.value_conv = nn.Conv2d(in_dim, in_dim, kernel_size=1)
        self.gamma = nn.Parameter(torch.zeros(1))
        self.softmax = nn.Softmax(dim=-1)

    def forward(self, x):
        n, c, h, w = x.size()
        query = self.query_conv(x).view(n, -1, h * w).permute(0, 2, 1)
        key = self.key_conv(x).view(n, -1, h * w)
        attention = self.softmax(torch.bmm(query, key))
        value = self.value_conv(x).view(n, -1, h * w)
        attended = torch.bmm(value, attention.permute(0, 2, 1)).view(n, c, h, w)
        return self.gamma * attended + x, attended


class CAM_Module(nn.Module):

    def __init__(self, in_dim):
        super(CAM_Module, self).__init__()
        self.channel_in = in_dim
        self.gamma = nn.Parameter(torch.zeros(1))
        self.softmax = nn.Softmax(dim=-1)

    def forward(self, x):
        n, c, h, w = x.size()
        flat = x.view(n, c, -1)
        energy = torch.bmm(flat, flat.permute(0, 2, 1))
        energy = torch.max(energy, -1, keepdim=True)[0].expand_as(energy) - energy
        out = torch.bmm(self.softmax(energy), flat).view(n, c, h, w)
        return self.gamma * out + x


class MaskedGraphLayer(nn.Module):

    def __init__(self, in_features, out_features, learn_graph=True, use_pose=True, dist_method='l2', gamma=0, k=4, **kwargs):
        super(MaskedGraphLayer, self).__init__()
        assert use_pose or learn_graph
        if dist_method != 'l2':
            raise NotImplementedError("dist_method={!r}: only 'l2' is on the ganet path".format(dist_method))
        self.in_features = in_features
        self.out_features = out_features
        self.learn_graph = learn_graph
        self.use_pose = use_pose
        self.dist_method = dist_method
        self.gamma = gamma
        self.linear = nn.Linear(in_features, out_features, bias=False)
        self.bn = nn.BatchNorm1d(out_features)
        self.relu = nn.LeakyReLU(0.1)
        nn.init.normal_(self.linear.weight, 0, 0.01)
        nn.init.constant_(self.bn.weight, 1)
        nn.init.constant_(self.bn.bias, 0)

    def get_sim_matrix(self, v_feats):
        sq = v_feats.pow(2).sum(dim=2)
        d2 = sq.unsqueeze(1) + sq.unsqueeze(2) - 2 * torch.bmm(v_feats, v_feats.transpose(1, 2))
        return 2 / (d2.clamp(1e-12).sqrt().exp() + 1)

    def forward(self, input, adj):
        h = self.linear(input)
        n, v, _ = h.size()
        mask = 1 - torch.eye(v, dtype=h.dtype, device=h.device).unsqueeze(0)
        graph = None
        if self.use_pose:
            graph = F.normalize(mask * adj, p=1, dim=2)
        if self.learn_graph:
            learned = F.normalize(mask * self.get_sim_matrix(input), p=1, dim=2)
            graph = learned if graph is None else (graph + learned) / 2
        msg = torch.bmm(graph, h)
        msg = self.relu(self.bn(msg.view(n * v, -1)).view(n, v, -1))
        return input + self.gamma * msg


class GANet(nn.Module):

    def __init__(self, num_classes, loss, block, layers, num_split, pyramid_part, num_gb, use_pose, learn_graph,
                 consistent_loss, nonlinear='relu', **kwargs):
        super(GANet, self).__init__()
        assert block is Bottleneck
        self.loss = loss
        self.feature_dim = 512 * block.expansion
        self.conv1 = nn.Conv2d(3, 64, kernel_size=7, stride=2, padding=3, bias=False)
        self.bn1 = nn.BatchNorm2d(64)
        self.relu = nn.ReLU(inplace=True)
        self.maxpool = nn.MaxPool2d(kernel_size=3, stride=2, padding=1)
        ch = 64
        self.layer1, ch = _make_stage(ch, 64, layers[0], 1)
        self.layer2, ch = _make_stage(ch, 128, layers[1], 2)
        self.layer3, ch = _make_stage(ch, 256, layers[2], 2)
        self.layer4, ch = _make_stage(ch, 512, layers[3], 1)

        self.num_split = num_split
        self.total_split_list = calc_splits(num_split) if pyramid_part else [num_split]
        self.total_split = sum(self.total_split_list)
        self.pam_layer = PAM_Module(self.feature_dim)
        self.cam_layer = CAM_Module(self.feature_dim)
        self.avgpool = nn.AdaptiveAvgPool2d(1)
        self.num_gb = num_gb
        self.graph_layers = nn.ModuleList(
            MaskedGraphLayer(in_features=self.feature_dim, out_features=self.feature_dim, use_pose=use_pose, learn_graph=learn_graph)
            for _ in range(num_gb))
        self.consistent_loss = consistent_loss
        self.bottleneck = nn.BatchNorm1d((num_gb + 1) * self.feature_dim)
        self.bottleneck.bias.requires_grad_(False)
        self.classifier = nn.Linear((num_gb + 1) * self.feature_dim, num_classes, bias=False)
        self._init_params()

        self.hip_precision = os.environ.get('AGRL_HIP_PRECISION', 'fp32')
        from torchreid import hip_ops as _ops
        _ops.check_precision(self.hip_precision)
        self.hip_static_weights = False
        self._hip_packs = {}
        self.pixel_mean = (0.485, 0.456, 0.406)
        self.pixel_std = (0.229, 0.224, 0.225)

    def _init_params(self):
        for m in self.modules():
            if isinstance(m, nn.Conv2d):
                nn.init.kaiming_normal_(m.weight, mode='fan_out', nonlinearity='relu')
                if m.bias is not None:
                    nn.init.constant_(m.bias, 0)
            elif isinstance(m, (nn.BatchNorm2d, nn.BatchNorm1d)):
                nn.init.constant_(m.weight, 1)
                nn.init.constant_(m.bias, 0)
            elif isinstance(m, nn.Linear):
                nn.init.normal_(m.weight, 0, 0.01)
                if m.bias is not None:
                    nn.init.constant_(m.bias, 0)

    def featuremaps(self, x):
        x = self.maxpool(self.relu(self.bn1(self.conv1(x))))
        return self.layer4(self.layer3(self.layer2(self.layer1(x))))

    def _attention_op(self, feat):
        att = F.normalize(feat.norm(p=2, dim=3, keepdim=True), p=1, dim=1)
        return (feat * att).sum(dim=1)

    def forward(self, x, adj, *args):
        if x.is_cuda and not self.training:
            from torchreid.models._ganet_hip import hip_forward_ganet
            return hip_forward_ganet(self, x, adj)
        if x.dtype == torch.uint8:
            from torchreid import hip_ops as _ops
            x = _ops.clips_to_float(x, self.pixel_mean, self.pixel_std)
        B, S, C, H, W = x.size()
        fm = self.featuremaps(x.view(B * S, C, H, W))
        _, c, h, w = fm.shape
        nodes = []
        for n in self.total_split_list:
            step = h // n
            for i in range(n):
                piece = fm[:, :, step * i: step * (i + 1)]
                pam_f, _ = self.pam_layer(piece)
                nodes.append(self.avgpool(pam_f + piece).view(B * S, c))
        f = torch.stack(nodes, dim=2).transpose(1, 2).contiguous().view(B, S * self.total_split, c)
        outs = [f]
        for layer in self.graph_layers:
            outs.append(layer(outs[-1], adj))
        f = torch.cat(outs, dim=2).view(B, S, self.total_split, (self.num_gb + 1) * c)
        f_g = self._attention_op(f).mean(dim=1).view(B, -1)
        bn = self.bottleneck(f_g)
        if self.consistent_loss and self.training:
            keep = []
            for _ in range(B):
                idx = list(range(S))
                idx.remove(np.random.randint(S))
                keep.append(idx)
            keep = torch.LongTensor(keep).to(f.device)
            sf = torch.gather(f, dim=1, index=keep.view(B, S - 1, 1, 1).repeat(1, 1, f.size(2), f.size(3)))
            sf_g = self._attention_op(sf).mean(dim=1).view(B, -1)
            sy = self.classifier(self.bottleneck(sf_g))
        if not self.training:
            return bn
        y = self.classifier(bn)
        if self.loss == {'xent'}:
            return [y, sy] if self.consistent_loss else y
        elif self.loss == {'xent', 'htri'}:
            return ([y, sy], [f_g, sf_g]) if self.consistent_loss else (y, f_g)
        raise KeyError('Unsupported loss: {}'.format(self.loss))

    def invalidate_hip_cache(self):
        self._hip_packs.clear()


def ganet(num_classes, loss, last_stride, num_split, num_gb, num_scale, knn, pyramid_part, use_pose, learn_graph,
          pretrained=True, consistent_loss=False, **kwargs):
    model = GANet(num_classes=num_classes, loss=loss, block=Bottleneck, layers=list(RESNET50_STAGES), last_stride=last_stride,
                  num_split=num_split, pyramid_part=pyramid_part, num_gb=num_gb, use_pose=use_pose, learn_graph=learn_graph,
                  consistent_loss=consistent_loss, nonlinear='relu', **kwargs)
    path = os.environ.get('AGRL_PRETRAINED_RESNET50', '')
    if pretrained and path and os.path.isfile(path):
        own = model.state_dict()
        picked = {k: v for k, v in torch.load(path, map_location='cpu').items() if k in own and own[k].size() == v.size()}
        own.update(picked)
        model.load_state_dict(own)
    return model
```

### agrl.pytorch_amd/torchreid/models/gsta.py

```python
from __future__ import absolute_import
from __future__ import division

__all__ = ['gsta']

import os

import numpy as np
import torch
from torch import nn
from torch.nn import functional as F

from torchreid.utils.reidtools import calc_splits
from .vmgn import Bottleneck, GraphLayer, RESNET50_STAGES, _make_stage


class GSTASingle(nn.Module):

    def __init__(self, num_classes, loss, block, layers, num_split, pyramid_part, num_gb, use_pose, learn_graph,
                 consistent_loss, nonlinear='relu', **kwargs):
        super(GSTASingle, self).__init__()
        assert block is Bottleneck
        self.loss = loss
        self.feature_dim = 512 * block.expansion
        self.conv1 = nn.Conv2d(3, 64, kernel_size=7, stride=2, padding=3, bias=False)
        self.bn1 = nn.BatchNorm2d(64)
        self.relu = nn.ReLU(inplace=True)
        self.maxpool = nn.MaxPool2d(kernel_size=3, stride=2, padding=1)
        ch = 64
        self.layer1, ch = _make_stage(ch, 64, layers[0], 1)
        self.layer2, ch = _make_stage(ch, 128, layers[1], 2)
        self.layer3, ch = _make_stage(ch, 256, layers[2], 2)
        self.layer4, ch = _make_stage(ch, 512, layers[3], 1)

        self.num_split = num_split
        self.total_split_list = calc_splits(num_split) if pyramid_part else [num_split]
        self.total_split = sum(self.total_split_list)
        self.parts_avgpool = nn.ModuleList(nn.AdaptiveAvgPool2d((n, 1)) for n in self.total_split_list)
        self.num_gb = num_gb
        self.graph_layers = nn.ModuleList(
            GraphLayer(in_features=self.feature_dim, out_features=self.feature_dim, use_pose=use_pose, learn_graph=learn_graph)
            for _ in range(num_gb))
        self.consistent_loss = consistent_loss
        self.bottleneck = nn.BatchNorm1d(self.feature_dim)
        self.bottleneck.bias.requires_grad_(False)
        self.classifier = nn.Linear(self.feature_dim, num_classes, bias=False)
        self._init_params()

        self.hip_precision = os.environ.get('AGRL_HIP_PRECISION', 'fp32')
        from torchreid import hip_ops as _ops
        _ops.check_precision(self.hip_precision)
        self.hip_static_weights = False
        self.hip_train = os.environ.get('AGRL_HIP_TRAIN', '1') != '0'
        self.hip_train_precision = os.environ.get('AGRL_HIP_TRAIN_PRECISION', 'fp32')
        self._hip_packs = {}
        self.pixel_mean = (0.485, 0.456, 0.406)
        self.pixel_std = (0.229, 0.224, 0.225)

    def _init_params(self):
        for m in self.modules():
            if isinstance(m, nn.Conv2d):
                nn.init.kaiming_normal_(m.weight, mode='fan_out', nonlinearity='relu')
            elif isinstance(m, (nn.BatchNorm2d, nn.BatchNorm1d)):
                nn.init.constant_(m.weight, 1)
                nn.init.constant_(m.bias, 0)
            elif isinstance(m, nn.Linear):
                nn.init.normal_(m.weight, 0, 0.01)

    def featuremaps(self, x):
        x = self.maxpool(self.relu(self.bn1(self.conv1(x))))
        return self.layer4(self.layer3(self.layer2(self.layer1(x))))

    def _attention_op(self, feat):
        att = F.normalize(feat.norm(p=2, dim=3, keepdim=True), p=1, dim=1)
        return (feat * att).sum(dim=1)

    def forward(self, x, adj, *args):
        if x.is_cuda and not self.training:
            from torchreid.models._vmgn_hip import hip_forward_gsta
            return hip_forward_gsta(self, x, adj)
        if x.dtype == torch.uint8:
            from torchreid import hip_ops as _ops
            x = _ops.clips_to_float(x, self.pixel_mean, self.pixel_std)
        if x.is_cuda and self.training and self.hip_train:
            if x.dtype != torch.float32:
                raise TypeError('the native train step takes float32 frames, got {}; set model.hip_train = False for the '
                                'stock-torch module tree'.format(x.dtype))
            from torchreid.models._train_hip import forward_train_gsta
            return forward_train_gsta(self, x, adj)
        B, S, C, H, W = x.size()
        fm = self.featuremaps(x.view(B * S, C, H, W))
        c = fm.size(1)
        parts = [pool(fm).view(B, S, c, n) for pool, n in zip(self.parts_avgpool, self.total_split_list)]
        f = torch.cat(parts, dim=3).transpose(2, 3).contiguous().view(B, S * self.total_split, c)
        for layer in self.graph_layers:
            f = layer(f, adj)
        f = f.view(B, S, self.total_split, c)
        f_g = self._attention_op(f).mean(dim=1).view(B, -1)
        bn = self.bottleneck(f_g)
        if self.consistent_loss and self.training:
            keep = []
            for _ in range(B):
                idx = list(range(S))
                idx.remove(np.random.randint(S))
                keep.append(idx)
            keep = torch.LongTensor(keep).to(f.device)
            sf = torch.gather(f, dim=1, index=keep.view(B, S - 1, 1, 1).repeat(1, 1, f.size(2), f.size(3)))
            sf_g = self._attention_op(sf).mean(dim=1).view(B, -1)
            sy = self.classifier(self.bottleneck(sf_g))
        if not self.training:
            return bn
        y = self.classifier(bn)
        if self.loss == {'xent'}:
            return [y, sy] if self.consistent_loss else y
        elif self.loss == {'xent', 'htri'}:
            return ([y, sy], [f_g, sf_g]) if self.consistent_loss else (y, f_g)
        raise KeyError('Unsupported loss: {}'.format(self.loss))

    def invalidate_hip_cache(self):
        self._hip_packs.clear()


def gsta(num_classes, loss, last_stride, num_split, num_gb, num_scale, pyramid_part, use_pose, learn_graph,
         pretrained=True, consistent_loss=False, **kwargs):
    model = GSTASingle(num_classes=num_classes, loss=loss, block=Bottleneck, layers=list(RESNET50_STAGES), last_stride=last_stride,
                       num_split=num_split, pyramid_part=pyramid_part, num_gb=num_gb, use_pose=use_pose, learn_graph=learn_graph,
                       consistent_loss=consistent_loss, nonlinear='relu', **kwargs)
    path = os.environ.get('AGRL_PRETRAINED_RESNET50', '')
    if pretrained and path and os.path.isfile(path):
        own = model.state_dict()
        picked = {k: v for k, v in torch.load(path, map_location='cpu').items() if k in own and own[k].size() == v.size()}
        own.update(picked)
        model.load_state_dict(own)
    return model
```

### agrl.pytorch_amd/torchreid/models/vmgn.py

```python
from __future__ import absolute_import
from __future__ import division

__all__ = ['vmgn']

import copy
import os

import torch
from torch import nn
from torch.nn import functional as F

from torchreid.utils.reidtools import calc_splits
from torchreid.utils.torchtools import weights_init_kaiming, weights_init_classifier

FEATURE_DIM = 2048
RESNET50_STAGES = (3, 4, 6, 3)


class Bottleneck(nn.Module):
    expansion = 4

    def __init__(self, inplanes, planes, stride=1, downsample=None):
        super(Bottleneck, self).__init__()
        width_out = planes * self.expansion
        self.conv1 = nn.Conv2d(inplanes, planes, kernel_size=1, bias=False)
        self.bn1 = nn.BatchNorm2d(planes)
        self.conv2 = nn.Conv2d(planes, planes, kernel_size=3, stride=stride, padding=1, bias=False)
        self.bn2 = nn.BatchNorm2d(planes)
        self.conv3 = nn.Conv2d(planes, width_out, kernel_size=1, bias=False)
        self.bn3 = nn.BatchNorm2d(width_out)
        self.relu = nn.ReLU(inplace=True)
        self.downsample = downsample
        self.stride = stride

    def forward(self, x):
        shortcut = x if self.downsample is None else self.downsample(x)
        y = self.relu(self.bn1(self.conv1(x)))
        y = self.relu(self.bn2(self.conv2(y)))
        y = self.bn3(self.conv3(y))
        y += shortcut
        return self.relu(y)


def _make_stage(inplanes, planes, blocks, stride):
    out_ch = planes * Bottleneck.expansion
    downsample = None
    if stride != 1 or inplanes != out_ch:
        downsample = nn.Sequential(
            nn.Conv2d(inplanes, out_ch, kernel_size=1, stride=stride, bias=False),
            nn.BatchNorm2d(out_ch),
        )
    units = [Bottleneck(inplanes, planes, stride, downsample)]
    units.extend(Bottleneck(out_ch, planes) for _ in range(1, blocks))
    return nn.Sequential(*units), out_ch


class GraphLayer(nn.Module):

    def __init__(self, in_features, out_features, learn_graph=True, use_pose=True,
                 dist_method='l2', gamma=0.1, k=4, **kwargs):
        super(GraphLayer, self).__init__()
        assert use_pose or learn_graph
        if dist_method != 'l2':
            raise NotImplementedError("dist_method={!r}: only 'l2' is on the vmgn path".format(dist_method))
        self.in_features = in_features
        self.out_features = out_features
        self.learn_graph = learn_graph
        self.use_pose = use_pose
        self.dist_method = dist_method
        self.gamma = gamma
        self.linear = nn.Linear(in_features, out_features, bias=False)
        self.bn = nn.BatchNorm1d(out_features)
        self.relu = nn.LeakyReLU(0.1)
        nn.init.normal_(self.linear.weight, 0, 0.01)
        nn.init.constant_(self.bn.weight, 1)
        nn.init.constant_(self.bn.bias, 0)

    def get_sim_matrix(self, v_feats):
        sq = v_feats.pow(2).sum(dim=2)
        d2 = sq.unsqueeze(1) + sq.unsqueeze(2)
        d2 = d2 - 2 * torch.bmm(v_feats, v_feats.transpose(1, 2))
        dist = d2.clamp(1e-12).sqrt()
        return 2 / (dist.exp() + 1)

    def forward(self, input, adj):
        h = self.linear(input)
        n, v, _ = h.size()
        graph = None
        if self.use_pose:
            graph = F.normalize(adj, p=1, dim=2)
        if self.learn_graph:
            learned = F.normalize(self.get_sim_matrix(input), p=1, dim=2)
            graph = learned if graph is None else (graph + learned) / 2
        msg = torch.bmm(graph, h)
        msg = self.relu(self.bn(msg.view(n * v, -1)).view(n, v, -1))
        return (1 - self.gamma) * input + self.gamma * msg


class GSTA(nn.Module):

    def __init__(self, num_classes, loss, block, layers, num_split, pyramid_part, num_gb, use_pose,
                 learn_graph, consistent_loss, nonlinear='relu', **kwargs):
        super(GSTA, self).__init__()
        assert block is Bottleneck
        self.loss = loss
        self.feature_dim = 512 * block.expansion

        self.conv1 = nn.Conv2d(3, 64, kernel_size=7, stride=2, padding=3, bias=False)
        self.bn1 = nn.BatchNorm2d(64)
        self.relu = nn.ReLU(inplace=True)
        self.maxpool = nn.MaxPool2d(kernel_size=3, stride=2, padding=1)
        ch = 64
        self.layer1, ch = _make_stage(ch, 64, layers[0], 1)
        self.layer2, ch = _make_stage(ch, 128, layers[1], 2)
        self.layer3, ch = _make_stage(ch, 256, layers[2], 2)
        self.layer4_1, ch = _make_stage(ch, 512, layers[3], 1)
        _load_local_pretrained(self)
        self.layer4_2 = copy.deepcopy(self.layer4_1)

        self.global_avg_pool = nn.AdaptiveAvgPool3d(1)
        self.global_bottleneck = nn.BatchNorm1d(self.feature_dim)
        self.global_bottleneck.bias.requires_grad_(False)
        self.global_classifier = nn.Linear(self.feature_dim, num_classes, bias=False)
        weights_init_kaiming(self.global_bottleneck)
        weights_init_classifier(self.global_classifier)

        self.num_split = num_split
        self.total_split_list = calc_splits(num_split) if pyramid_part else [num_split]
        self.total_split = sum(self.total_split_list)
        self.parts_avgpool = nn.ModuleList(nn.AdaptiveAvgPool2d((n, 1)) for n in self.total_split_list)
        self.num_gb = num_gb
        self.graph_layers = nn.ModuleList(
            GraphLayer(in_features=self.feature_dim, out_features=self.feature_dim,
                       use_pose=use_pose, learn_graph=learn_graph)
            for _ in range(num_gb))
        self.consistent_loss = consistent_loss
        self.att_bottleneck = nn.BatchNorm1d(self.feature_dim)
        self.att_bottleneck.bias.requires_grad_(False)
        self.att_classifier = nn.Linear(self.feature_dim, num_classes, bias=False)
        weights_init_kaiming(self.att_bottleneck)
        weights_init_classifier(self.att_classifier)

        self.hip_precision = os.environ.get('AGRL_HIP_PRECISION', 'fp32')
        from torchreid import hip_ops as _ops
        _ops.check_precision(self.hip_precision)
        self.hip_static_weights = False
        self.hip_train = os.environ.get('AGRL_HIP_TRAIN', '1') != '0'
        self.hip_train_precision = os.environ.get('AGRL_HIP_TRAIN_PRECISION', 'fp32')
        self.hip_train_tail = os.environ.get('AGRL_HIP_TRAIN_TAIL', '1') != '0'
        self._hip_packs = {}
        self.pixel_mean = (0.485, 0.456, 0.406)
        self.pixel_std = (0.229, 0.224, 0.225)

    def _attention_op(self, feat):
        att = F.normalize(feat.norm(p=2, dim=3, keepdim=True), p=1, dim=1)
        return (feat * att).sum(dim=1)

    def featuremaps(self, x):
        x = self.maxpool(self.relu(self.bn1(self.conv1(x))))
        x = self.layer3(self.layer2(self.layer1(x)))
        return self.layer4_1(x), self.layer4_2(x)

    def _pooled_nodes(self, x4_1, x4_2, B, S):
        _, c, h, w = x4_1.shape
        g_f = self.global_avg_pool(x4_1.view(B, S, c, h, w).transpose(1, 2).contiguous()).view(B, -1)
        parts = [pool(x4_2).view(B, S, c, n) for pool, n in zip(self.parts_avgpool, self.total_split_list)]
        f = torch.cat(parts, dim=3).transpose(2, 3).contiguous().view(B, S * self.total_split, c)
        return g_f, f

    def forward(self, x, adj, *args):
        if x.is_cuda and not self.training:
            from torchreid.models._vmgn_hip import hip_forward
            return hip_forward(self, x, adj)

        if x.dtype == torch.uint8:
            from torchreid import hip_ops as _ops
            x = _ops.clips_to_float(x, self.pixel_mean, self.pixel_std)
        B, S, C, H, W = x.size()
        if x.is_cuda and self.training and self.hip_train and x.dtype != torch.float32:
            raise TypeError('the native train step takes float32 frames (the reference trains in fp32), got {}; '
                            'set model.hip_train = False for the stock-torch module tree'.format(x.dtype))
        if x.is_cuda and self.training and self.hip_train and self.hip_train_tail:
            from torchreid.models._train_hip import forward_train
            out_list, f_list = forward_train(self, x, adj)
            if self.loss == {'xent'}:
                return out_list
            elif self.loss == {'xent', 'htri'}:
                return out_list, f_list
            raise KeyError('Unsupported loss: {}'.format(self.loss))
        if x.is_cuda and self.training and self.hip_train:
            from torchreid.models._train_hip import featuremaps_train
            x4_1, x4_2 = [t.contiguous() for t in featuremaps_train(self, x.view(B * S, C, H, W))]
        else:
            x4_1, x4_2 = self.featuremaps(x.view(B * S, C, H, W))
        c = x4_1.size(1)
        g_f, f = self._pooled_nodes(x4_1, x4_2, B, S)
        g_bn = self.global_bottleneck(g_f)
        for layer in self.graph_layers:
            f = layer(f, adj)
        f = f.view(B, S, self.total_split, c)
        att_f = self._attention_op(f).mean(dim=1).view(B, -1)
        att_bn = self.att_bottleneck(att_f)

        if not self.training:
            return torch.cat([g_bn, att_bn], dim=1)

        out_list = [self.global_classifier(g_bn), self.att_classifier(att_bn)]
        f_list = [g_f, att_f]
        if self.consistent_loss:
            assert S >= 5
            for num_frame in [S - 3, S - 2, S - 1]:
                pick = torch.sort(torch.randperm(S)[:num_frame])[0].long().to(f.device)
                sub = torch.gather(f, dim=1, index=pick.view(1, num_frame, 1, 1).repeat(B, 1, self.total_split, c))
                satt_f = self._attention_op(sub).mean(dim=1).view(B, -1)
                out_list.append(self.att_classifier(self.att_bottleneck(satt_f)))
                f_list.append(satt_f)

        if self.loss == {'xent'}:
            return out_list
        elif self.loss == {'xent', 'htri'}:
            return out_list, f_list
        raise KeyError('Unsupported loss: {}'.format(self.loss))

    def invalidate_hip_cache(self):
        self._hip_packs.clear()


def _load_local_pretrained(model):
    path = os.environ.get('AGRL_PRETRAINED_RESNET50', '')
    if not path or not os.path.isfile(path):
        return False
    pretrained = torch.load(path, map_location='cpu')
    own = model.state_dict()
    picked = {}
    for key, value in pretrained.items():
        target = key.replace('layer4.', 'layer4_1.', 1) if key.startswith('layer4.') else key
        if target in own and own[target].size() == value.size():
            picked[target] = value
    own.update(picked)
    model.load_state_dict(own)
    print('Initialized model with pretrained weights from {}'.format(path))
    return True


def vmgn(num_classes, loss, last_stride, num_split, num_gb, num_scale,
         pyramid_part, use_pose, learn_graph, consistent_loss=False, **kwargs):
    return GSTA(
        num_classes=num_classes,
        loss=loss,
        block=Bottleneck,
        layers=list(RESNET50_STAGES),
        last_stride=last_stride,
        num_split=num_split,
        pyramid_part=pyramid_part,
        num_gb=num_gb,
        use_pose=use_pose,
        learn_graph=learn_graph,
        consistent_loss=consistent_loss,
        nonlinear='relu',
        **kwargs
    )
```

### include/agrl_hip.h

```cpp
#ifndef AGRL_HIP_H
#define AGRL_HIP_H

#include <stddef.h>
#include <stdint.h>

#ifdef __cplusplus
extern "C" {
#endif

#define AGRL_F32 0
#define AGRL_LP16 1
#define AGRL_BF16 AGRL_LP16
#define AGRL_F32X3 2
#define AGRL_F32H3 3
#define AGRL_F32H3P 4

#define AGRL_METRIC_EUCLIDEAN 0
#define AGRL_METRIC_COSINE 1

typedef void* agrl_stream_t;

int agrl_version(void);
const char* agrl_last_error(void);

int agrl_lp16_is_f16(void);

int agrl_reload_options(void);
int agrl_built_with_ablation(void);


int agrl_stem_conv_bn_relu_maxpool(const float* x, const float* w, const float* bias, void* out,
                                   int N, int H, int W, int out_dtype, agrl_stream_t stream);

int agrl_stem_conv_bn_relu_maxpool_lp16(const float* x, const void* w_packed, const float* bias,
                                        void* out, int N, int H, int W, agrl_stream_t stream);

int agrl_stem_split16(const float* x, const void* wh_packed, const void* wl_packed, const float* bias, float* out, int N, int H,
                      int W, float w_unscale, agrl_stream_t stream);

#define AGRL_FRAMES_NCHW 0
#define AGRL_FRAMES_NHWC 1
int agrl_stem_conv_bn_relu_maxpool_u8(const unsigned char* x, const float* table, int layout, const float* w, const float* bias,
                                      void* out, int N, int H, int W, int out_dtype, agrl_stream_t stream);
int agrl_stem_conv_bn_relu_maxpool_lp16_u8(const unsigned char* x, const float* table, int layout, const void* w_packed,
                                           const float* bias, void* out, int N, int H, int W, agrl_stream_t stream);
int agrl_stem_split16_u8(const unsigned char* x, const float* table, int layout, const void* wh_packed, const void* wl_packed,
                         const float* bias, float* out, int N, int H, int W, float w_unscale, agrl_stream_t stream);

int agrl_frames_normalize_u8(const unsigned char* x, const float* table, int layout, float* out, int N, int H, int W,
                             agrl_stream_t stream);

int agrl_conv2d_bn_act(const void* x, const void* w, const float* bias, const void* residual,
                       void* out, int N, int H, int W, int Cin, int Cout, int R, int S, int stride,
                       int pad, int relu, int dtype, agrl_stream_t stream);

int agrl_conv2d_bn_act_split16(const void* x, const void* w_scaled, const float* bias, const void* residual, void* out, int N,
                               int H, int W, int Cin, int Cout, int R, int S, int stride, int pad, int relu, float w_unscale,
                               int x_presplit, int out_presplit, agrl_stream_t stream);

int agrl_split16_weights_inloop(const float* w_scaled, void* out, long long rows, int K, agrl_stream_t stream);

int agrl_conv1x1_dual_split16(const void* x, const void* x2, const void* w_scaled, const float* bias, void* out, int N, int H, int W,
                              int stride, int K1, int K2, int Cout, int relu, float w_unscale, int x2_presplit, int out_planes,
                              agrl_stream_t stream);

int agrl_split16_planes(const float* x, void* out, long long rows, int C, int nplanes, agrl_stream_t stream);
int agrl_split16_weight_planes(const float* x, void* out, long long rows, int C, float scale, agrl_stream_t stream);
int agrl_conv1x1_split16(const void* x, const void* packed, const float* bias, const void* residual, void* out, int M, int K3,
                         int Cout, int relu, float w_unscale, int layout, agrl_stream_t stream);
int agrl_conv1x1_split16_dual(const void* x, const void* x2, const void* packed, const float* bias, void* out, int M, int K1_3,
                              int K2_3, int Cout, int relu, float w_unscale, int layout, agrl_stream_t stream);
int agrl_conv1x1_split16_pool(const void* x, const void* packed, const float* bias, const void* residual, float* pool_out, int N,
                              int H, int W, int K3, int Cout, int relu, const int* splits, int n_splits, int mean, float w_unscale,
                              int layout, agrl_stream_t stream);
int agrl_conv3x3_packed_split16(const void* x, const void* packed, const float* bias, void* out, int N, int H, int W, int Cin3,
                                int Cout, int relu, float w_unscale, agrl_stream_t stream);

int agrl_conv1x1_dual_bn_act(const void* x1, const void* x2, const void* w, const float* bias, void* out, int M,
                             int K1, int K2, int Cout, int relu, agrl_stream_t stream);

int agrl_conv1x1_bn_act_pool(const void* x, const void* w, const float* bias, const void* residual,
                             void* out, float* pool_out, void* pool_out_lp, int N, int H, int W,
                             int Cin, int Cout, int relu, const int* splits, int n_splits, int mean,
                             agrl_stream_t stream);

int agrl_bottleneck_tail(const void* y2, const void* w3, const float* b3, const void* residual,
                         const void* x_short, const void* w_short, const float* b_short, void* out,
                         const void* w1_next, const float* b1_next, void* z, int M, int Cmid, int Cout,
                         int Cnext, int Cshort, agrl_stream_t stream);

long long agrl_bottleneck_seam_packed_bytes(int Cmid, int Cout, int Cnext);
int agrl_bottleneck_seam_pack(const void* w3, const void* w1_next, void* packed, int Cmid, int Cout, int Cnext,
                              agrl_stream_t stream);
int agrl_bottleneck_seam(const void* y2, const void* packed, const float* b3, const void* residual, void* out,
                         const float* b1_next, void* z, int M, int Cmid, int Cout, int Cnext, agrl_stream_t stream);

long long agrl_conv3x3_packed_bytes(int Cin, int Cout);
int agrl_conv3x3_pack(const void* w_ohwi, void* packed, int Cin, int Cout, agrl_stream_t stream);
int agrl_conv3x3_packed_bn_act(const void* x, const void* packed, const float* bias, void* out, int N, int H, int W, int Cin,
                               int Cout, int relu, agrl_stream_t stream);

long long agrl_conv1x1_packed_bytes(int K, int Cout);
int agrl_conv1x1_pack(const void* w, void* packed, int K, int Cout, agrl_stream_t stream);
int agrl_conv1x1_packed_bn_act(const void* x, const void* x2, const void* packed, const float* bias, void* out, int M, int K1,
                               int K2, int Cout, int relu, agrl_stream_t stream);

int agrl_conv1x1_packed_res_bn_act(const void* x, const void* packed, const float* bias, const void* residual, void* out, int M,
                                   int K, int Cout, int relu, agrl_stream_t stream);
int agrl_conv1x1_packed_res_pool(const void* x, const void* packed, const float* bias, const void* residual, float* pool_out,
                                 void* pool_out_lp, int N, int H, int W, int K, int Cout, int relu, const int* splits,
                                 int n_splits, int mean, agrl_stream_t stream);
int agrl_conv1x1_packed_dual_duo(const void* x, const void* x2, const void* packed, const float* bias, void* out, int M, int K1,
                                 int K2, int Cout, int relu, agrl_stream_t stream);
int agrl_conv1x1_packed_dual_strided(const void* x, const void* x2, const void* packed, const float* bias, void* out, int N, int Hi,
                                     int Wi, int stride, int K1, int K2, int Cout, int relu, agrl_stream_t stream);

int agrl_bottleneck_block(const void* z, const void* w2, const float* b2, const void* w3, const float* b3,
                          const void* residual, const void* x_short, const void* w_short, const float* b_short,
                          void* out, const void* w1_next, const float* b1_next, void* z_next, int F, int H, int W,
                          int Cmid, int Cout, int Cnext, agrl_stream_t stream);

int agrl_linear_nobias(const void* x, const void* w, float* y, int M, int K, int Nout,
                       int in_dtype, agrl_stream_t stream);


int agrl_pose_adjacency(const float* poses, const unsigned char* detected, float* adj, int B, int S,
                        int num_split, int pyramid_part, float height, float threshold, agrl_stream_t stream);
int agrl_pose_adjacency_bits(const float* poses, const unsigned char* detected, uint32_t* adj_bits, int B, int S, int num_split,
                             int pyramid_part, float height, float threshold, agrl_stream_t stream);
int agrl_adjacency_pack(const float* adj, uint32_t* adj_bits, int B, int V, agrl_stream_t stream);


int agrl_part_pool(const void* x4_1, const void* x4_2, float* gsum, float* nodes, void* nodes_lp,
                   int F, int h, int w, int C, const int* splits, int n_splits, int dtype,
                   agrl_stream_t stream);


int agrl_graph_gram(const float* f, float* gram_part, int B, int V, int C, int cslice,
                    agrl_stream_t stream);

int agrl_graph_finalize(const float* gram_part, int nz, const float* adj, float* G, int B, int V,
                        int use_pose, int learn_graph, int mask_diag, agrl_stream_t stream);
int agrl_graph_finalize_bits(const float* gram_part, int nz, const uint32_t* adj_bits, float* G, int B, int V, int use_pose,
                             int learn_graph, int mask_diag, agrl_stream_t stream);

int agrl_graph_apply(const float* G, const float* f, void* out, int out_dtype, int B, int V, int C, agrl_stream_t stream);
int agrl_graph_tracklet_operand(const float* f, const void* adj, int adj_packed, float* G_out, void* out, int out_dtype, int B,
                                int V, int C, int use_pose, int learn_graph, int mask_diag, agrl_stream_t stream);
int agrl_graph_linear_mix(const void* p_op, const void* w, const float* f, const float* bn_scale, const float* bn_shift,
                          float keep, float gamma, float slope, float* out, int M, int K, int Nout, int in_dtype,
                          agrl_stream_t stream);

int agrl_graph_propagate(const float* f, const float* h, const float* G, const float* bn_scale,
                         const float* bn_shift, float keep, float gamma, float slope, float* out, void* out_lp,
                         int B, int V, int C, agrl_stream_t stream);


int agrl_pam_pool(const void* x, const void* qk, float* xbar, float* xmean, int F, int h, int w, int C, int Cq,
                  const int* splits, int n_splits, int dtype, agrl_stream_t stream);

int agrl_pam_combine(const float* y, const float* bv, const float* xmean, float gamma, float* nodes, void* nodes_lp,
                     int rows, int C, agrl_stream_t stream);


int agrl_row_sqnorm(const void* x, float* sqn, int R, int C, int dtype, agrl_stream_t stream);

int agrl_attn_pool_bnneck(const float* nodes, const float* sqn, const float* gsum,
                          const float* g_scale, const float* g_shift, const float* a_scale,
                          const float* a_shift, float* out, float* g_f, float* att_f, int B, int S,
                          int P, int C, int hw, agrl_stream_t stream);

int agrl_attn_tail(const float* nodes, const float* gsum, const float* g_scale, const float* g_shift, const float* a_scale,
                   const float* a_shift, float* out, float* g_f, float* att_f, float* node_sqn, float* out_sqn, void* q_lp,
                   float* q_f32, int B, int S, int P, int C, int hw, agrl_stream_t stream);

int agrl_clip_pool(const float* feats, float* out, int T, int n, int D, int mode, agrl_stream_t stream);


int agrl_row_l2_normalize(const float* x, void* y, int R, int C, int ldy, int normalize, int out_dtype,
                          agrl_stream_t stream);

int agrl_distmat(const void* q, const void* g, const float* qn, const float* gn, float* dist,
                 int m, int n, int D, int ldd, int metric, int dtype, void* workspace,
                 size_t workspace_bytes, agrl_stream_t stream);

int agrl_distmat_split16(const void* q3, const void* g3, const float* qn, const float* gn, float* dist, int m, int n, int D3,
                         int ldd, int metric, float g_unscale, void* workspace, size_t workspace_bytes, agrl_stream_t stream);

int agrl_rank_topk(const float* dist, int m, int n, int ldd, int k, int idx_offset, int32_t* idx,
                   float* val, agrl_stream_t stream);

size_t agrl_distmat_topk_workspace(int m, int n);
int agrl_distmat_topk(const void* q, const void* g, const float* qn, const float* gn, int m, int n, int D, int metric,
                      int dtype, int k, int idx_offset, int32_t* idx, float* val, void* workspace,
                      size_t workspace_bytes, void* gemm_workspace, size_t gemm_workspace_bytes, agrl_stream_t stream);

int agrl_rank_argsort(const float* dist, int m, int n, int ldd, int32_t* idx, agrl_stream_t stream);

int agrl_rank_mars(const int32_t* topk_idx, const int32_t* q_pids, const int32_t* q_camids,
                   const int32_t* g_pids, const int32_t* g_camids, int m, int n, int k, double* ap,
                   float* cmc, agrl_stream_t stream);

int agrl_rank_market1501(const float* dist, int m, int n, int ldd, const int32_t* q_pids,
                         const int32_t* q_camids, const int32_t* g_pids, const int32_t* g_camids,
                         int max_rank, double* ap, float* cmc, int32_t* valid, agrl_stream_t stream);

size_t agrl_re_ranking_workspace(int m, int n, int k1);
int agrl_re_ranking(const float* q_g, const float* q_q, const float* g_g, int m, int n, int k1, int k2,
                    double lambda_value, float* final_dist, int ldf, void* workspace, size_t workspace_bytes,
                    agrl_stream_t stream);


size_t agrl_bn_workspace(int M, int C);

int agrl_bn_stats(const float* y, float* mean, float* var, int M, int C, void* workspace, size_t workspace_bytes,
                  agrl_stream_t stream);

int agrl_conv2d_stats(const float* x, const float* w, float* out, float* partial, size_t partial_bytes, int N, int H, int W, int Cin,
                      int Cout, int R, int S, int stride, int pad, int dtype, agrl_stream_t stream);
int agrl_bn_stats_from_partials(const float* partial, int rows, int C, int M, float* mean, float* var, void* workspace,
                                size_t workspace_bytes , agrl_stream_t stream);

int agrl_bn_fold_train(const float* mean, const float* var, const float* gamma, const float* beta, float eps, float momentum,
                       long long n, float* running_mean, float* running_var, long long* num_batches_tracked, float* scale,
                       float* shift, float* invstd, int C, agrl_stream_t stream);

int agrl_bn_apply(const float* y, const float* scale, const float* shift, const float* residual, float* out, unsigned char* mask,
                  int M, int C, int relu, float slope, agrl_stream_t stream);

int agrl_bn_backward(const float* dout, const float* out, const unsigned char* mask, const float* y, const float* mean,
                     const float* invstd, const float* gamma, int relu, float slope, float* dy, float* dz, float* dgamma,
                     float* dbeta, int M, int C, void* workspace, size_t workspace_bytes, agrl_stream_t stream);

int agrl_im2col_t(const float* x, float* T, int ldT, int F, int H, int W, int C, int R, int S, int stride, int pad,
                  agrl_stream_t stream);

int agrl_im2col_rows(const float* x, float* P, int ldP, int F, int H, int W, int C, int R, int S, int stride, int pad, int nchw,
                     agrl_stream_t stream);

int agrl_gemm_nt_splitk(const void* x, const void* w, float* y, int M, int K, int Nout, int in_dtype, void* workspace,
                        size_t workspace_bytes, agrl_stream_t stream);

size_t agrl_conv_wgrad_workspace(int F, int H, int W, int Cin, int Cout, int R, int S, int stride, int pad);
int agrl_conv_wgrad_plan(int F, int H, int W, int Cin, int Cout, int R, int S, int stride, int pad, int dtype, int* plan);
int agrl_conv_wgrad(const float* x, const float* dy, float* dw, int F, int H, int W, int Cin, int Cout, int R, int S, int stride,
                    int pad, int dtype, void* workspace, size_t workspace_bytes, agrl_stream_t stream);

int agrl_maxpool3x3s2(const float* x, float* out, unsigned char* idx, int F, int H, int W, int C, agrl_stream_t stream);
int agrl_maxpool3x3s2_backward(const float* dout, const unsigned char* idx, float* dx, int F, int H, int W, int C,
                               agrl_stream_t stream);


int agrl_axpby(const float* x, const float* y, float a, float b, float* out, size_t total, agrl_stream_t stream);

int agrl_part_pool_backward(const float* dg, const float* dnodes, float* dx1, float* dx2, int F, int S, int h, int w, int C,
                            const int* splits, int n_splits, agrl_stream_t stream);

int agrl_attn_pool_backward(const float* nodes, const float* datt, float* dnodes, int B, int S, int P, int C,
                            agrl_stream_t stream);

int agrl_graph_matrix_backward(const float* gram_part, int nz, const float* dG, float* M, int B, int V, int use_pose,
                               int mask_diag, agrl_stream_t stream);

int agrl_graph_pair_product(const float* a, const float* b, float* part, float* out, int B, int V, int C, agrl_stream_t stream);

int agrl_xent_label_smooth(const float* logits, const int32_t* targets, int n, int K, float eps, float* loss, float* dlogits,
                           float* row_loss, agrl_stream_t stream);


int agrl_triplet_hard_mine(const float* x, const int32_t* pids, int n, int d, float* dist_ap,
                           float* dist_an, int32_t* idx_ap, int32_t* idx_an, agrl_stream_t stream);


int agrl_diag_read_stream(const void* src, size_t bytes, float* sink, int workgroups, agrl_stream_t stream);

int agrl_triplet_loss(const float* x, const int32_t* pids, int n, int d, float margin, int soft, float* loss, float* grad,
                      float* dist_ap, float* dist_an, int32_t* idx_ap, int32_t* idx_an, float* coeff, agrl_stream_t stream);

int agrl_optim_geometry(int* chunk_elems, int* max_workgroups, int* descriptor_words);

int agrl_adam_step(const void* tensors, int n_tensors, const void* chunks, int n_chunks, float weight_decay,
                   float one_minus_beta1, float beta2, float one_minus_beta2, float step_size, float inv_sqrt_bc2, float eps,
                   int amsgrad, int zero_grad, agrl_stream_t stream);

int agrl_sgd_step(const void* tensors, int n_tensors, const void* chunks, int n_chunks, float weight_decay, float momentum,
                  float lr, int has_momentum, int first_step, int nesterov, int zero_grad, agrl_stream_t stream);

#ifdef __cplusplus
}
#endif
#endif
```

Before: 73940 frames/s.

## Write stride-2 subsampled block outputs at layer exits feeding strided downsample blocks

```diff
diff --git a/agrl.pytorch_amd/csrc/bottleneck_block.hip b/agrl.pytorch_amd/csrc/bottleneck_block.hip
--- a/agrl.pytorch_amd/csrc/bottleneck_block.hip
+++ b/agrl.pytorch_amd/csrc/bottleneck_block.hip
@@ -19,15 +19,16 @@
     int F, H, W;
 };
 
-template <bool CAT, int CN>
+template <bool CAT, int CN, int NST = 4 + CN / 64>
 __global__ __launch_bounds__(512) void bottleneck_block_kernel(const BlockParams p, int ntiles) {
     static_assert(CN == 64 || (CN == 128 && !CAT), "next conv1: 64 channels, or 128 with the identity shortcut");
+    static_assert(NST == 4 + CN / 64 || (NST == 1 + CN / 64 && CN == 128 && !CAT), "4 out stores per thread, or 1 (out at stride 2)");
+    constexpr bool SOUT = NST != 4 + CN / 64;
     constexpr int NW = 8, PW = 10, PPIX = 100, PPIECES = 13, PATCH_BYTES = PPIECES * 1024, PJ = 2;
     constexpr int W_TAP = 64 * 128, W2_BYTES = 9 * W_TAP;
     constexpr int Y_BYTES = 64 * 128;
     constexpr int X_BYTES = CAT ? 64 * 128 : 0;
     constexpr int R_BYTES = 64 * 512;
-    constexpr int NST = CN == 64 ? 5 : 6;
     constexpr int NA2 = CN / 64;
     __shared__ __attribute__((aligned(16))) unsigned char smem[W2_BYTES + 2 * PATCH_BYTES + Y_BYTES + X_BYTES + R_BYTES + 1024];
     unsigned char* s_w2 = smem;
@@ -287,7 +288,13 @@
             }
         }
         wg_barrier();
-        {
+        if constexpr (SOUT) {
+            const int k = td >> 5, pch = td & 31;
+            const int row = ((k >> 2) << 4) + ((k & 3) << 1);
+            const size_t opix = ((size_t)img * (p.H >> 1) + (oy0 >> 1) + (k >> 2)) * (p.W >> 1) + (ox0 >> 1) + (k & 3);
+            const uint4 v = *reinterpret_cast<const uint4*>(s_r + row * 512 + (pch << 4));
+            *reinterpret_cast<uint4*>(reinterpret_cast<unsigned char*>(p.out) + (opix * 256 + (pch ^ (row & 31)) * 8) * 2) = v;
+        } else {
             unsigned char* obase = reinterpret_cast<unsigned char*>(p.out) + gpix(img, oy0, ox0, 0) * 512;
 #pragma unroll
             for (int i = 0; i < 4; ++i) {
@@ -379,3 +386,32 @@
     AGRL_CHECK_LAUNCH("agrl_bottleneck_block");
     return 0;
 }
+
+extern "C" int agrl_bottleneck_block_strided_out(const void* z, const void* w2, const float* b2, const void* w3, const float* b3,
+                                                 const void* residual, const void* x_short, const void* w_short,
+                                                 const float* b_short, void* out, const void* w1_next, const float* b1_next,
+                                                 void* z_next, int F, int H, int W, int Cmid, int Cout, int Cnext, int out_stride,
+                                                 agrl_stream_t stream) {
+    AGRL_CHECK_ARG(z && w2 && b2 && w3 && b3 && residual && out && w1_next && b1_next && z_next,
+                   "agrl_bottleneck_block_strided_out: null pointer");
+    AGRL_CHECK_ARG(!x_short && !w_short && !b_short,
+                   "agrl_bottleneck_block_strided_out: built for the identity shortcut only (no downsample conv)");
+    AGRL_CHECK_ARG(out_stride == 2, "agrl_bottleneck_block_strided_out: built for out_stride=2 (got %d)", out_stride);
+    AGRL_CHECK_ARG(F > 0 && H > 0 && W > 0 && (H % 8) == 0 && (W % 8) == 0,
+                   "agrl_bottleneck_block_strided_out: maps must be multiples of 8 x 8 (got %d x %d)", H, W);
+    AGRL_CHECK_ARG(Cmid == 64 && Cout == 256 && Cnext == 128,
+                   "agrl_bottleneck_block_strided_out: built for Cmid=64, Cout=256, Cnext=128 with the identity shortcut, got %d/%d/%d",
+                   Cmid, Cout, Cnext);
+    AGRL_CHECK_ARG((size_t)F * H * W * 256 * 2 < (1ull << 40), "agrl_bottleneck_block_strided_out: problem too large");
+    const uintptr_t al = (uintptr_t)z | (uintptr_t)w2 | (uintptr_t)b2 | (uintptr_t)w3 | (uintptr_t)b3 | (uintptr_t)residual |
+                         (uintptr_t)out | (uintptr_t)w1_next | (uintptr_t)b1_next | (uintptr_t)z_next;
+    AGRL_CHECK_ARG((al & 15) == 0, "agrl_bottleneck_block_strided_out: pointers must be 16-byte aligned");
+    BlockParams p;
+    p.z = z; p.w2 = w2; p.b2 = b2; p.w3 = w3; p.b3 = b3; p.res = residual; p.xs = nullptr; p.ws = nullptr; p.bs = nullptr;
+    p.out = out; p.w1n = w1_next; p.b1n = b1_next; p.zn = z_next; p.F = F; p.H = H; p.W = W;
+    const int ntiles = F * (H / 8) * (W / 8);
+    const int grid = ntiles < 256 ? ntiles : 256;
+    hipLaunchKernelGGL((bottleneck_block_kernel<false, 128, 3>), dim3(grid), dim3(512), 0, (hipStream_t)stream, p, ntiles);
+    AGRL_CHECK_LAUNCH("agrl_bottleneck_block_strided_out");
+    return 0;
+}
diff --git a/agrl.pytorch_amd/csrc/bottleneck_tail.hip b/agrl.pytorch_amd/csrc/bottleneck_tail.hip
--- a/agrl.pytorch_amd/csrc/bottleneck_tail.hip
+++ b/agrl.pytorch_amd/csrc/bottleneck_tail.hip
@@ -533,6 +533,211 @@
             }
         }
         wait_vmcnt<10>();
+        wg_barrier();
+    }
+}
+
+
+constexpr int L2XN2 = 256;
+
+__global__ __launch_bounds__(512) void bottleneck_tail_l2_exit_kernel(const TailParams p, int ntiles, int H, int W) {
+    constexpr int A_BYTES = 2 * TBM * 128;
+    constexpr int R_BYTES = TBM * L2N1 * 2;
+    __shared__ __attribute__((aligned(16))) unsigned char smem[2 * A_BYTES + 2 * R_BYTES];
+    unsigned char* s_a = smem;
+    unsigned char* s_r = smem + 2 * A_BYTES;
+
+    const int tid = threadIdx.x, lane = tid & 63;
+    const int wave = __builtin_amdgcn_readfirstlane(tid >> 6);
+    const int frow = lane & 15, fchunk = lane >> 4;
+    const int G = gridDim.x;
+    const unsigned char* zsrc = reinterpret_cast<const unsigned char*>(&g_zero16);
+    const unsigned char* y2g = reinterpret_cast<const unsigned char*>(p.y2);
+    const unsigned char* resg = reinterpret_cast<const unsigned char*>(p.res);
+
+    uint4 w3f[4][4], w1f[2][16];
+#pragma unroll
+    for (int a = 0; a < 4; ++a)
+#pragma unroll
+        for (int kk = 0; kk < 4; ++kk)
+            w3f[a][kk] = *reinterpret_cast<const uint4*>(reinterpret_cast<const unsigned char*>(p.w3) +
+                                                         ((size_t)(wave * 64 + a * 16 + frow) * L2K1 + kk * 32 + fchunk * 8) * 2);
+#pragma unroll
+    for (int a = 0; a < 2; ++a)
+#pragma unroll
+        for (int ks = 0; ks < 16; ++ks)
+            w1f[a][ks] = *reinterpret_cast<const uint4*>(reinterpret_cast<const unsigned char*>(p.w1n) +
+                                                         ((size_t)(wave * 32 + a * 16 + frow) * L2K2 + ks * 32 + fchunk * 8) * 2);
+    float b3l = p.b3[wave * 64 + lane];
+    float b1l = p.b1n[wave * 32 + (lane & 31)];
+    asm volatile("" : "+v"(b3l), "+v"(b1l));
+    auto lane_bias = [&](float held, int src_lane) {
+        return __int_as_float(__builtin_amdgcn_ds_bpermute(src_lane << 2, __float_as_int(held)));
+    };
+#pragma unroll
+    for (int a = 0; a < 4; ++a)
+#pragma unroll
+        for (int kk = 0; kk < 4; ++kk)
+            asm volatile("" : "+v"(w3f[a][kk].x), "+v"(w3f[a][kk].y), "+v"(w3f[a][kk].z), "+v"(w3f[a][kk].w));
+#pragma unroll
+    for (int a = 0; a < 2; ++a)
+#pragma unroll
+        for (int ks = 0; ks < 16; ++ks)
+            asm volatile("" : "+v"(w1f[a][ks].x), "+v"(w1f[a][ks].y), "+v"(w1f[a][ks].z), "+v"(w1f[a][ks].w));
+
+    auto stage_tile = [&](int T, int slot) {
+        const int m0 = T * TBM;
+        int ln = lane;
+        asm volatile("" : "+v"(ln));
+        {
+            const int row = wave * 8 + (ln >> 3);
+            const int gm = m0 + row;
+#pragma unroll
+            for (int kt = 0; kt < 2; ++kt)
+                dma16(gm < p.M ? y2g + (size_t)gm * (L2K1 * 2) + kt * 128 + (((ln & 7) ^ ((row >> 1) & 7)) << 4) : zsrc,
+                      s_a + slot * A_BYTES + kt * (TBM * 128) + wave * 1024);
+        }
+#pragma unroll
+        for (int j = 0; j < 8; ++j) {
+            const int row = wave * 8 + j;
+            const int gm = m0 + row;
+            dma16(gm < p.M ? resg + (size_t)gm * (L2N1 * 2) + ((ln ^ (row & 31)) << 4) : zsrc, s_r + slot * R_BYTES + row * 1024);
+        }
+    };
+
+    const int HW = H * W, Ho = ((H - 1) >> 1) + 1, Wo = ((W - 1) >> 1) + 1;
+    int T = blockIdx.x;
+    if (T < ntiles) stage_tile(T, 0);
+    wait_vmcnt<0>();
+    wg_barrier();
+    int slot = 0;
+    for (; T < ntiles; T += G, slot ^= 1) {
+        const int m0 = T * TBM;
+        if (T + G < ntiles) stage_tile(T + G, slot ^ 1);
+        const unsigned char* sa = s_a + slot * A_BYTES;
+        unsigned char* sr = s_r + slot * R_BYTES;
+#pragma unroll
+        for (int a = 0; a < 4; ++a) {
+            int fr = frow, fc = fchunk;
+            asm volatile("" : "+v"(fr), "+v"(fc));
+            f32x4_t acc[4];
+#pragma unroll
+            for (int b = 0; b < 4; ++b) acc[b] = f32x4_t{0.f, 0.f, 0.f, 0.f};
+            uint4 xp[2][2];
+            auto ld1 = [&](int st, int b) {
+                const int kk = st >> 1;
+                return *reinterpret_cast<const uint4*>(sa + (kk >> 1) * (TBM * 128) + lds_off(((st & 1) * 2 + b) * 16 + fr, (kk & 1) * 4 + fc));
+            };
+#pragma unroll
+            for (int b = 0; b < 2; ++b) xp[0][b] = ld1(0, b);
+#pragma unroll
+            for (int st = 0; st < 8; ++st) {
+                if (st + 1 < 8) {
+#pragma unroll
+                    for (int b = 0; b < 2; ++b) xp[(st + 1) & 1][b] = ld1(st + 1, b);
+                }
+#pragma unroll
+                for (int b = 0; b < 2; ++b) acc[(st & 1) * 2 + b] = Frag<lp16_t>::mma(w3f[a][st >> 1], xp[st & 1][b], acc[(st & 1) * 2 + b]);
+                __builtin_amdgcn_sched_barrier(0);
+            }
+            float bv[4];
+#pragma unroll
+            for (int r = 0; r < 4; ++r) bv[r] = lane_bias(b3l, a * 16 + fc * 4 + r);
+            const int c = wave * 64 + a * 16 + fc * 4;
+            uint2 rcell[4];
+#pragma unroll
+            for (int b = 0; b < 4; ++b) {
+                const int px = b * 16 + fr;
+                rcell[b] = *reinterpret_cast<const uint2*>(sr + px * 1024 + (((c >> 3) ^ (px & 31)) << 4) + ((c & 4) << 1));
+            }
+#pragma unroll
+            for (int b = 0; b < 4; ++b) {
+                const int px = b * 16 + fr;
+                unsigned char* cell = sr + px * 1024 + (((c >> 3) ^ (px & 31)) << 4) + ((c & 4) << 1);
+                float rr[4];
+                unpack_lp16x2(rcell[b].x, rr[0], rr[1]);
+                unpack_lp16x2(rcell[b].y, rr[2], rr[3]);
+                float v[4];
+#pragma unroll
+                for (int r = 0; r < 4; ++r) v[r] = relu_nan(acc[b][r] + bv[r] + rr[r]);
+                store4<lp16_t>(reinterpret_cast<lp16_t*>(cell), v);
+            }
+            __builtin_amdgcn_sched_barrier(0);
+        }
+        wg_barrier();
+        int ld = lane, td = tid;
+        asm volatile("" : "+v"(ld), "+v"(td));
+#pragma unroll
+        for (int i = 0; i < 8; ++i) {
+            const int row = wave + 8 * i;
+            const int gm = m0 + row;
+            if (gm < p.M) {
+                const int n = gm / HW, rem = gm - n * HW;
+                const int h = rem / W, w = rem - h * W;
+                if (((h | w) & 1) == 0) {
+                    const size_t opix = ((size_t)n * Ho + (h >> 1)) * Wo + (w >> 1);
+                    const uint4 v = *reinterpret_cast<const uint4*>(sr + row * 1024 + (ld << 4));
+                    *reinterpret_cast<uint4*>(reinterpret_cast<unsigned char*>(p.out) + (opix * L2N1 + (ld ^ (row & 31)) * 8) * 2) = v;
+                }
+            }
+        }
+        unsigned char* sz0 = s_a + slot * A_BYTES;
+#pragma unroll
+        for (int bh = 0; bh < 2; ++bh) {
+            int fr = frow, fc = fchunk;
+            asm volatile("" : "+v"(fr), "+v"(fc));
+            f32x4_t acc2[2][2];
+#pragma unroll
+            for (int a = 0; a < 2; ++a)
+#pragma unroll
+                for (int b = 0; b < 2; ++b) acc2[a][b] = f32x4_t{0.f, 0.f, 0.f, 0.f};
+            uint4 xq[2][2];
+            auto ld2 = [&](int ks, int b) {
+                const int px = (bh * 2 + b) * 16 + fr;
+                return *reinterpret_cast<const uint4*>(sr + px * 1024 + (((ks * 4 + fc) ^ (px & 31)) << 4));
+            };
+#pragma unroll
+            for (int b = 0; b < 2; ++b) xq[0][b] = ld2(0, b);
+#pragma unroll
+            for (int ks = 0; ks < 16; ++ks) {
+                if (ks + 1 < 16) {
+#pragma unroll
+                    for (int b = 0; b < 2; ++b) xq[(ks + 1) & 1][b] = ld2(ks + 1, b);
+                }
+#pragma unroll
+                for (int a = 0; a < 2; ++a)
+#pragma unroll
+                    for (int b = 0; b < 2; ++b) acc2[a][b] = Frag<lp16_t>::mma(w1f[a][ks], xq[ks & 1][b], acc2[a][b]);
+                __builtin_amdgcn_sched_barrier(0);
+            }
+            if (bh == 1) wg_barrier();
+            unsigned char* sz = bh == 0 ? sz0 : sr;
+#pragma unroll
+            for (int b = 0; b < 2; ++b) {
+                const int pl = b * 16 + fr;
+#pragma unroll
+                for (int a = 0; a < 2; ++a) {
+                    const int c = wave * 32 + a * 16 + fc * 4;
+                    float v[4];
+#pragma unroll
+                    for (int r = 0; r < 4; ++r) v[r] = relu_nan(acc2[a][b][r] + lane_bias(b1l, a * 16 + fc * 4 + r));
+                    store4<lp16_t>(reinterpret_cast<lp16_t*>(sz + pl * 512 + (((c >> 3) ^ (pl & 31)) << 4) + ((c & 4) << 1)), v);
+                }
+            }
+        }
+        wg_barrier();
+#pragma unroll
+        for (int hf = 0; hf < 2; ++hf)
+#pragma unroll
+            for (int i = 0; i < 2; ++i) {
+                const int row = (td >> 5) + 16 * i, pch = td & 31;
+                const int gm = m0 + hf * 32 + row;
+                if (gm < p.M) {
+                    const uint4 v = *reinterpret_cast<const uint4*>((hf == 0 ? sz0 : sr) + row * 512 + (pch << 4));
+                    *reinterpret_cast<uint4*>(reinterpret_cast<unsigned char*>(p.z) + ((size_t)gm * L2XN2 + (pch ^ (row & 31)) * 8) * 2) = v;
+                }
+            }
+        wait_vmcnt<4>();
         wg_barrier();
     }
 }
@@ -568,3 +773,29 @@
     AGRL_CHECK_LAUNCH("agrl_bottleneck_tail");
     return 0;
 }
+
+
+extern "C" int agrl_bottleneck_tail_strided_out(const void* y2, const void* w3, const float* b3, const void* residual,
+                                                const void* x_short, const void* w_short, const float* b_short, void* out,
+                                                const void* w1_next, const float* b1_next, void* z, int M, int Cmid, int Cout,
+                                                int Cnext, int Cshort, int H, int W, int out_stride, agrl_stream_t stream) {
+    AGRL_CHECK_ARG(y2 && w3 && b3 && residual && out && w1_next && b1_next && z, "agrl_bottleneck_tail_strided_out: null pointer");
+    AGRL_CHECK_ARG(!x_short && !w_short && !b_short && Cshort == 0,
+                   "agrl_bottleneck_tail_strided_out: built for the identity shortcut only (no downsample conv)");
+    AGRL_CHECK_ARG(out_stride == 2, "agrl_bottleneck_tail_strided_out: built for out_stride=2 (got %d)", out_stride);
+    AGRL_CHECK_ARG(Cmid == L2K1 && Cout == L2N1 && Cnext == L2XN2,
+                   "agrl_bottleneck_tail_strided_out: built for Cmid=128, Cout=512, Cnext=256, got %d/%d/%d", Cmid, Cout, Cnext);
+    AGRL_CHECK_ARG(M > 0 && H > 0 && W > 0 && (long long)H * W <= M && M % (H * W) == 0,
+                   "agrl_bottleneck_tail_strided_out: M = %d is not a whole number of %d x %d maps", M, H, W);
+    const uintptr_t al = (uintptr_t)y2 | (uintptr_t)w3 | (uintptr_t)b3 | (uintptr_t)residual | (uintptr_t)out |
+                         (uintptr_t)w1_next | (uintptr_t)b1_next | (uintptr_t)z;
+    AGRL_CHECK_ARG((al & 15) == 0, "agrl_bottleneck_tail_strided_out: pointers must be 16-byte aligned");
+    TailParams p;
+    p.y2 = y2; p.w3 = w3; p.b3 = b3; p.res = residual; p.out = out; p.w1n = w1_next; p.b1n = b1_next; p.z = z; p.M = M;
+    p.xs = nullptr; p.ws = nullptr; p.bs = nullptr;
+    const int ntiles = cdiv(M, TBM);
+    const int grid = ntiles < 256 ? ntiles : 256;
+    hipLaunchKernelGGL(bottleneck_tail_l2_exit_kernel, dim3(grid), dim3(512), 0, (hipStream_t)stream, p, ntiles, H, W);
+    AGRL_CHECK_LAUNCH("agrl_bottleneck_tail_strided_out");
+    return 0;
+}
diff --git a/agrl.pytorch_amd/torchreid/_hip.py b/agrl.pytorch_amd/torchreid/_hip.py
--- a/agrl.pytorch_amd/torchreid/_hip.py
+++ b/agrl.pytorch_amd/torchreid/_hip.py
@@ -60,6 +60,7 @@
     "agrl_conv3x3_packed_split16": [_p, _p, _p, _p, _i, _i, _i, _i, _i, _i, _f, _p],
     "agrl_conv2d_bn_act_split16": [_p, _p, _p, _p, _p] + [_i] * 10 + [_f, _i, _i, _p],
     "agrl_bottleneck_tail": [_p, _p, _p, _p, _p, _p, _p, _p, _p, _p, _p, _i, _i, _i, _i, _i, _p],
+    "agrl_bottleneck_tail_strided_out": [_p, _p, _p, _p, _p, _p, _p, _p, _p, _p, _p, _i, _i, _i, _i, _i, _i, _i, _i, _p],
     "agrl_bottleneck_seam_packed_bytes": [_i, _i, _i],
     "agrl_bottleneck_seam_pack": [_p, _p, _p, _i, _i, _i, _p],
     "agrl_bottleneck_seam": [_p, _p, _p, _p, _p, _p, _p, _i, _i, _i, _i, _p],
@@ -74,6 +75,7 @@
     "agrl_conv3x3_pack": [_p, _p, _i, _i, _p],
     "agrl_conv3x3_packed_bn_act": [_p, _p, _p, _p, _i, _i, _i, _i, _i, _i, _p],
     "agrl_bottleneck_block": [_p, _p, _p, _p, _p, _p, _p, _p, _p, _p, _p, _p, _p, _i, _i, _i, _i, _i, _i, _p],
+    "agrl_bottleneck_block_strided_out": [_p, _p, _p, _p, _p, _p, _p, _p, _p, _p, _p, _p, _p, _i, _i, _i, _i, _i, _i, _i, _p],
     "agrl_conv1x1_dual_bn_act": [_p, _p, _p, _p, _p, _i, _i, _i, _i, _i, _p],
     "agrl_conv1x1_bn_act_pool": [_p, _p, _p, _p, _p, _p, _p, _i, _i, _i, _i, _i, _i, C.POINTER(_i), _i, _i, _p],
     "agrl_linear_nobias": [_p, _p, _p, _i, _i, _i, _i, _p],
@@ -227,7 +229,7 @@
 PROFILE_TAG = None
 
 
-def call(name, *args):
+def call(name, *args, profile_as=None):
     fn = getattr(lib(), name)
     if PROFILE is None:
         _check(name, fn(*args))
@@ -238,5 +240,5 @@
     _check(name, fn(*args))
     end.record(stream)
     global PROFILE_TAG
-    PROFILE.append((name, start, end, PROFILE_TAG))
+    PROFILE.append((profile_as or name, start, end, PROFILE_TAG))
     PROFILE_TAG = None
diff --git a/agrl.pytorch_amd/torchreid/hip_ops.py b/agrl.pytorch_amd/torchreid/hip_ops.py
--- a/agrl.pytorch_amd/torchreid/hip_ops.py
+++ b/agrl.pytorch_amd/torchreid/hip_ops.py
@@ -634,7 +634,12 @@
     return ok
 
 
-def bottleneck_tail(y2, w3, b3, residual, w1_next, b1_next, shortcut=None):
+def bottleneck_tail_strided_supported(y2, w3, w1_next, out_stride):
+    return (y2.dtype == LP_DTYPE and out_stride == 2 and tuple(w3.shape) == (512, 1, 1, 128)
+            and tuple(w1_next.shape) == (256, 1, 1, 512))
+
+
+def bottleneck_tail(y2, w3, b3, residual, w1_next, b1_next, shortcut=None, out_stride=1):
     N, H, W, Cmid = y2.shape
     Cout, Cnext = w3.shape[0], w1_next.shape[0]
     assert y2.dtype == LP_DTYPE and (residual is None) != (shortcut is None)
@@ -646,7 +651,8 @@
         Cshort = xs.shape[3]
     else:
         assert residual.shape == (N, H, W, Cout) and residual.dtype == y2.dtype
-    out = torch.empty((N, H, W, Cout), dtype=y2.dtype, device=y2.device)
+    assert out_stride == 1 or shortcut is None
+    out = torch.empty((N, (H - 1) // out_stride + 1, (W - 1) // out_stride + 1, Cout), dtype=y2.dtype, device=y2.device)
     z = torch.empty((N, H, W, Cnext), dtype=y2.dtype, device=y2.device)
     M = N * H * W
     if _hip.PROFILE is not None:
@@ -654,8 +660,13 @@
         _hip.PROFILE_TAG = {"flops": 2.0 * M * ((Cmid + Cshort) * Cout + Cout * Cnext),
                             "bytes": 2.0 * (y2.numel() + rd + out.numel() + z.numel() + w3.numel() + w1_next.numel())}
     with _dev(y2):
-        call("agrl_bottleneck_tail", ptr(y2), ptr(w3), ptr(b3), ptr(residual), ptr(xs), ptr(ws), ptr(bs), ptr(out),
-             ptr(w1_next), ptr(b1_next), ptr(z), M, Cmid, Cout, Cnext, Cshort, _stream(y2))
+        if out_stride != 1:
+            call("agrl_bottleneck_tail_strided_out", ptr(y2), ptr(w3), ptr(b3), ptr(residual), ptr(xs), ptr(ws), ptr(bs), ptr(out),
+                 ptr(w1_next), ptr(b1_next), ptr(z), M, Cmid, Cout, Cnext, Cshort, H, W, out_stride, _stream(y2),
+                 profile_as="agrl_bottleneck_tail")
+        else:
+            call("agrl_bottleneck_tail", ptr(y2), ptr(w3), ptr(b3), ptr(residual), ptr(xs), ptr(ws), ptr(bs), ptr(out),
+                 ptr(w1_next), ptr(b1_next), ptr(z), M, Cmid, Cout, Cnext, Cshort, _stream(y2))
     return out, z
 
 
@@ -667,7 +678,15 @@
     return ok
 
 
-def bottleneck_block(z, w2, b2, w3, b3, residual, w1_next, b1_next, shortcut=None):
+def strided_exits_enabled():
+    return switch('AGRL_HIP_STRIDED_EXITS') != '0'
+
+
+def bottleneck_block_strided_supported(z, w3, w1_next, out_stride):
+    return z.dtype == LP_DTYPE and out_stride == 2 and tuple(w3.shape) == (256, 1, 1, 64) and tuple(w1_next.shape) == (128, 1, 1, 256)
+
+
+def bottleneck_block(z, w2, b2, w3, b3, residual, w1_next, b1_next, shortcut=None, out_stride=1):
     N, H, W, Cmid = z.shape
     Cout, Cnext = w3.shape[0], w1_next.shape[0]
     assert z.dtype == LP_DTYPE and (residual is None) != (shortcut is None)
@@ -677,7 +696,8 @@
         assert tuple(xs.shape) == (N, H, W, 64) and xs.dtype == z.dtype
     else:
         assert tuple(residual.shape) == (N, H, W, Cout) and residual.dtype == z.dtype
-    out = torch.empty((N, H, W, Cout), dtype=z.dtype, device=z.device)
+    assert out_stride == 1 or shortcut is None
+    out = torch.empty((N, H // out_stride, W // out_stride, Cout), dtype=z.dtype, device=z.device)
     zn = torch.empty((N, H, W, Cnext), dtype=z.dtype, device=z.device)
     M = N * H * W
     if _hip.PROFILE is not None:
@@ -685,8 +705,13 @@
         _hip.PROFILE_TAG = {"flops": 2.0 * M * (9 * Cmid * Cmid + (Cmid + (64 if shortcut is not None else 0)) * Cout + Cout * Cnext),
                             "bytes": 2.0 * (z.numel() + rd + out.numel() + zn.numel() + w2.numel() + w3.numel() + w1_next.numel())}
     with _dev(z):
-        call("agrl_bottleneck_block", ptr(z), ptr(w2), ptr(b2), ptr(w3), ptr(b3), ptr(residual), ptr(xs), ptr(ws), ptr(bs),
-             ptr(out), ptr(w1_next), ptr(b1_next), ptr(zn), N, H, W, Cmid, Cout, Cnext, _stream(z))
+        if out_stride != 1:
+            call("agrl_bottleneck_block_strided_out", ptr(z), ptr(w2), ptr(b2), ptr(w3), ptr(b3), ptr(residual), ptr(xs), ptr(ws), ptr(bs),
+                 ptr(out), ptr(w1_next), ptr(b1_next), ptr(zn), N, H, W, Cmid, Cout, Cnext, out_stride, _stream(z),
+                 profile_as="agrl_bottleneck_block")
+        else:
+            call("agrl_bottleneck_block", ptr(z), ptr(w2), ptr(b2), ptr(w3), ptr(b3), ptr(residual), ptr(xs), ptr(ws), ptr(bs),
+                 ptr(out), ptr(w1_next), ptr(b1_next), ptr(zn), N, H, W, Cmid, Cout, Cnext, _stream(z))
     return out, zn
 
 
diff --git a/agrl.pytorch_amd/torchreid/models/_ganet_hip.py b/agrl.pytorch_amd/torchreid/models/_ganet_hip.py
--- a/agrl.pytorch_amd/torchreid/models/_ganet_hip.py
+++ b/agrl.pytorch_amd/torchreid/models/_ganet_hip.py
@@ -4,7 +4,7 @@
 
 from torchreid import hip_ops as ops
 from torchreid import _hip
-from torchreid.models._vmgn_hip import (_PRECISIONS, eval_frames, run_stem, _fingerprint, _fold_bn1d, _fold_conv_bn, _pack_stage, _run_block, _run_trunk,
+from torchreid.models._vmgn_hip import (_PRECISIONS, eval_frames, run_stem, _fingerprint, _fold_bn1d, _fold_conv_bn, _pack_stage, _run_block, _run_trunk, _strided_exits,
                                          check_packed_range)
 
 
@@ -64,7 +64,7 @@
     splits = list(model.total_split_list)
     with torch.no_grad(), ops.f32_split(model.hip_precision == 'bf16x3'):
         a = run_stem(frames, pack, norm)
-        a = _run_trunk(a, pack['trunk'])
+        a = _run_trunk(a, pack['trunk'], _strided_exits(model))
         for blk in pack['l4']:
             a = _run_block(a, blk)
         C = a.shape[-1]
diff --git a/agrl.pytorch_amd/torchreid/models/_vmgn_hip.py b/agrl.pytorch_amd/torchreid/models/_vmgn_hip.py
--- a/agrl.pytorch_amd/torchreid/models/_vmgn_hip.py
+++ b/agrl.pytorch_amd/torchreid/models/_vmgn_hip.py
@@ -103,6 +103,7 @@
     key = (device.index if device.index is not None else torch.cuda.current_device(), precision)
     cached = model._hip_packs.get(key)
     if cached is not None and (model.hip_static_weights or cached['fingerprint'] == _fingerprint(model)):
+        cached['strided_exits'] = _strided_exits(model)
         return cached
     first = next(model.parameters())
     if first.device != device:
@@ -160,6 +161,7 @@
     if dtype == ops.LP_DTYPE:
         check_packed_range(pack)
     pack['fingerprint'] = _fingerprint(model)
+    pack['strided_exits'] = _strided_exits(model)
     model._hip_packs[key] = pack
     return pack
 
@@ -234,8 +236,13 @@
     return getattr(blk['c1'][0], 'agrl_presplit', False)
 
 
-def _run_trunk(a, blocks):
+def _strided_exits(model):
+    return bool(getattr(model, 'hip_strided_exits', True)) and ops.strided_exits_enabled()
+
+
+def _run_trunk(a, blocks, strided_exits=False):
     z = None
+    a_stride = 1
     for i, blk in enumerate(blocks):
         if _is_inloop(blk):
             a = _run_block_inloop(a, blk)
@@ -247,13 +254,22 @@
             if ops.bottleneck_block_supported(y, blk['c2'][0], blk['stride'], blk['c3'][0], nxt['c1'][0], ds) and (
                     ds is None or a.shape[3] == 64):
                 if ds is None:
+                    a_stride = 1
+                    if (strided_exits and 'dualps' in nxt and nxt['stride'] == 2 and nxt['ds_stride'] == 2
+                            and ops.bottleneck_block_strided_supported(y, blk['c3'][0], nxt['c1'][0], 2)):
+                        a_stride = 2
                     a, z = ops.bottleneck_block(y, blk['c2'][0], blk['c2'][1], blk['c3'][0], blk['c3'][1], a,
-                                                nxt['c1'][0], nxt['c1'][1])
+                                                nxt['c1'][0], nxt['c1'][1], out_stride=a_stride)
                 else:
                     a, z = ops.bottleneck_block(y, blk['c2'][0], blk['c2'][1], blk['c3'][0], blk['c3'][1], None,
                                                 nxt['c1'][0], nxt['c1'][1], shortcut=(a, blk['ds'][0], blk['ds'][1]))
                 continue
         y = _conv2(y, blk)
+        if a_stride != 1:
+            assert 'dualps' in blk and a_stride == blk['stride'] and a.shape[:3] == y.shape[:3] and a.dtype == y.dtype
+            a = ops.conv1x1_packed_dual_strided(a, y, blk['dualps'], blk['dualps_bias'], blk['c3'][0].shape[0], 1, True)
+            a_stride, z = 1, None
+            continue
         fusable = nxt is not None and ops.bottleneck_tail_supported(y, blk['c3'][0], nxt['c1'][0])
         if fusable and blk['ds'] is not None and ops.bottleneck_tail_supported(
                 y, blk['c3'][0], nxt['c1'][0], (blk['ds'][0], blk['ds_stride'])) and a.shape[3] == 64:
@@ -264,6 +280,12 @@
                 and tuple(y.shape[1:3]) == tuple((d - 1) // blk['stride'] + 1 for d in a.shape[1:3])):
             a = ops.conv1x1_packed_dual_strided(a, y, blk['dualps'], blk['dualps_bias'], blk['c3'][0].shape[0], blk['stride'], True)
             z = None
+            continue
+        if (strided_exits and nxt is not None and blk['ds'] is None and 'dualps' in nxt and nxt['stride'] == 2 and nxt['ds_stride'] == 2
+                and ops.bottleneck_tail_strided_supported(y, blk['c3'][0], nxt['c1'][0], 2)
+                and a.is_contiguous() and a.dtype == y.dtype and tuple(a.shape) == tuple(y.shape[:3]) + (blk['c3'][0].shape[0],)):
+            a, z = ops.bottleneck_tail(y, blk['c3'][0], blk['c3'][1], a, nxt['c1'][0], nxt['c1'][1], out_stride=2)
+            a_stride = 2
             continue
         shortcut = a if blk['ds'] is None else ops.conv_bn_act(a, blk['ds'][0], blk['ds'][1], blk['ds_stride'], 0, False)
         if nxt is not None and 'seam' in blk and (y.numel() // y.shape[-1]) % 128 == 0:
@@ -327,7 +349,7 @@
 
 def hip_featuremaps(frames, pack, norm=None):
     a = run_stem(frames, pack, norm)
-    a = _run_trunk(a, pack['trunk'])
+    a = _run_trunk(a, pack['trunk'], pack['strided_exits'])
     x4_1 = a
     for blk in pack['l4_1']:
         x4_1 = _run_block(x4_1, blk)
@@ -350,10 +372,10 @@
     a = run_stem(frames, pack, norm)
     if first is None:
         run_block = _run_block
-        a = _run_trunk(a, pack['trunk'])
+        a = _run_trunk(a, pack['trunk'], pack['strided_exits'])
     else:
         run_block = _run_block_planes
-        a = _run_trunk(a, pack['trunk'][:first - 1])
+        a = _run_trunk(a, pack['trunk'][:first - 1], pack['strided_exits'])
         a = _run_block_inloop(a, pack['trunk'][first - 1], out_planes=2)
         for blk in pack['trunk'][first:]:
             a = run_block(a, blk)
@@ -447,7 +469,7 @@
     splits = list(model.total_split_list)
     with torch.no_grad(), ops.f32_split(model.hip_precision == 'bf16x3'):
         a = run_stem(frames, pack, norm)
-        a = _run_trunk(a, pack['trunk'])
+        a = _run_trunk(a, pack['trunk'], pack['strided_exits'])
         if lp and a.shape[1] * a.shape[2] == 128 and pack['l4'][0]['stride'] == 1:
             for blk in pack['l4'][:-1]:
                 a = _run_block(a, blk)
diff --git a/agrl.pytorch_amd/torchreid/models/ganet.py b/agrl.pytorch_amd/torchreid/models/ganet.py
--- a/agrl.pytorch_amd/torchreid/models/ganet.py
+++ b/agrl.pytorch_amd/torchreid/models/ganet.py
@@ -130,6 +130,7 @@
         from torchreid import hip_ops as _ops
         _ops.check_precision(self.hip_precision)
         self.hip_static_weights = False
+        self.hip_strided_exits = True
         self._hip_packs = {}
         self.pixel_mean = (0.485, 0.456, 0.406)
         self.pixel_std = (0.229, 0.224, 0.225)
diff --git a/agrl.pytorch_amd/torchreid/models/gsta.py b/agrl.pytorch_amd/torchreid/models/gsta.py
--- a/agrl.pytorch_amd/torchreid/models/gsta.py
+++ b/agrl.pytorch_amd/torchreid/models/gsta.py
@@ -50,6 +50,7 @@
         from torchreid import hip_ops as _ops
         _ops.check_precision(self.hip_precision)
         self.hip_static_weights = False
+        self.hip_strided_exits = True
         self.hip_train = os.environ.get('AGRL_HIP_TRAIN', '1') != '0'
         self.hip_train_precision = os.environ.get('AGRL_HIP_TRAIN_PRECISION', 'fp32')
         self._hip_packs = {}
diff --git a/agrl.pytorch_amd/torchreid/models/vmgn.py b/agrl.pytorch_amd/torchreid/models/vmgn.py
--- a/agrl.pytorch_amd/torchreid/models/vmgn.py
+++ b/agrl.pytorch_amd/torchreid/models/vmgn.py
@@ -145,6 +145,7 @@
         from torchreid import hip_ops as _ops
         _ops.check_precision(self.hip_precision)
         self.hip_static_weights = False
+        self.hip_strided_exits = True
         self.hip_train = os.environ.get('AGRL_HIP_TRAIN', '1') != '0'
         self.hip_train_precision = os.environ.get('AGRL_HIP_TRAIN_PRECISION', 'fp32')
         self.hip_train_tail = os.environ.get('AGRL_HIP_TRAIN_TAIL', '1') != '0'
diff --git a/include/agrl_hip.h b/include/agrl_hip.h
--- a/include/agrl_hip.h
+++ b/include/agrl_hip.h
@@ -88,6 +88,10 @@
                          const void* x_short, const void* w_short, const float* b_short, void* out,
                          const void* w1_next, const float* b1_next, void* z, int M, int Cmid, int Cout,
                          int Cnext, int Cshort, agrl_stream_t stream);
+int agrl_bottleneck_tail_strided_out(const void* y2, const void* w3, const float* b3, const void* residual,
+                                     const void* x_short, const void* w_short, const float* b_short, void* out,
+                                     const void* w1_next, const float* b1_next, void* z, int M, int Cmid, int Cout,
+                                     int Cnext, int Cshort, int H, int W, int out_stride, agrl_stream_t stream);
 
 long long agrl_bottleneck_seam_packed_bytes(int Cmid, int Cout, int Cnext);
 int agrl_bottleneck_seam_pack(const void* w3, const void* w1_next, void* packed, int Cmid, int Cout, int Cnext,
@@ -119,6 +123,10 @@
                           const void* residual, const void* x_short, const void* w_short, const float* b_short,
                           void* out, const void* w1_next, const float* b1_next, void* z_next, int F, int H, int W,
                           int Cmid, int Cout, int Cnext, agrl_stream_t stream);
+int agrl_bottleneck_block_strided_out(const void* z, const void* w2, const float* b2, const void* w3, const float* b3,
+                                      const void* residual, const void* x_short, const void* w_short, const float* b_short,
+                                      void* out, const void* w1_next, const float* b1_next, void* z_next, int F, int H, int W,
+                                      int Cmid, int Cout, int Cnext, int out_stride, agrl_stream_t stream);
 
 int agrl_linear_nobias(const void* x, const void* w, float* y, int M, int K, int Nout,
                        int in_dtype, agrl_stream_t stream);
```

Result: no change. 74670 frames/s, median of 6 (+1.0%).
